# srinidhiPY/SSL_CR_Histo

Hardware: AMD Instinct MI355X
Metric: images/sec (ResNet18 SSL_CR step, 256x256 bf16 synthetic patches; whole job) (higher is better)
Workload: dtype bf16

## Files before the change

include/sslcr.h:

```cpp
#ifndef SSLCR_H_
#define SSLCR_H_
#include <stddef.h>
#include <stdint.h>

#ifdef __cplusplus
extern "C" {
#endif
#if defined(__GNUC__) || defined(__clang__)
#pragma GCC visibility push(default)
#endif

#define SSLCR_F32 0
#define SSLCR_BF16 1
#define SSLCR_FP8 2

int sslcr_version(void);
const char* sslcr_last_error(void);

typedef struct sslcr_conv_desc {
  const void* x;
  const void* w;
  void* y;
  const float* in_scale;
  const float* in_shift;
  const float* bias;
  const void* residual;
  float* stats;
  int N, H, W, C, K, R, S, stride, pad;
  int PH, PW;
  int OH, OW, osh;
  int transposed;
  int in_relu, relu, accumulate;
  int pix_mul, pix_off_h, pix_off_w;
  unsigned tap_mask;
  const void* mask_x; const float* mask_scale; const float* mask_shift; const float* mask_mean;
  int par4;
  int seg_images, seg_stride;
  const float* out_scale;
} sslcr_conv_desc;
int sslcr_conv2d(int dtype, const sslcr_conv_desc* d, void* stream);
int sslcr_conv2d_partial_rows(const sslcr_conv_desc* d);
int sslcr_conv2d_segments_ok(int dtype, const sslcr_conv_desc* d);
const char* sslcr_conv2d_kernel_name(int dtype, const sslcr_conv_desc* d);
int sslcr_conv2d_s2_pair(int dtype, const sslcr_conv_desc* c1, const sslcr_conv_desc* ds, void* stream);
int sslcr_conv2d_s2_pair_ok(int dtype, const sslcr_conv_desc* c1, const sslcr_conv_desc* ds);

typedef struct sslcr_fp8_desc {
  const uint8_t* w8;
  const float* w_dequant;
  float x_scale;
  const float* x_scale_dev;
  float* amax_out;
} sslcr_fp8_desc;
int sslcr_conv2d_fp8(const sslcr_conv_desc* d, const sslcr_fp8_desc* q, void* stream);
int sslcr_conv2d_fp8_partial_rows(const sslcr_conv_desc* d);
typedef struct sslcr_pack_fp8_desc {
  const float* w;
  uint8_t* w8;
  float* w_dequant;
  const float* gamma; const float* beta; const float* rmean; const float* rvar; float eps; float* bias_out;
  int K, C;
} sslcr_pack_fp8_desc;
int sslcr_pack_conv_fp8(const sslcr_pack_fp8_desc* d, void* stream);

typedef struct sslcr_wgrad_desc {
  const void* x;
  const void* dy;
  float* dw;
  const float* in_scale;
  const float* in_shift;
  int in_relu;
  int N, H, W, C, K, R, S, stride, pad, OH, OW;
  int seg_images;
  int seg_stride;
} sslcr_wgrad_desc;
int sslcr_conv2d_wgrad(int dtype, const sslcr_wgrad_desc* d, void* stream);
const char* sslcr_conv2d_wgrad_kernel_name(int dtype, const sslcr_wgrad_desc* d);

int sslcr_probe_tr16(const uint16_t* in, const int* byte_addr, uint16_t* out, void* stream);

typedef struct sslcr_stem_desc {
  const void* x;
  const void* w;
  void* y;
  const float* bias;
  float* stats;
  int N, H, W, OH, OW, in_f32, relu;
  const void* x2;
  int n_split;
  const float* out_scale;
} sslcr_stem_desc;
int sslcr_stem_conv(int dtype, const sslcr_stem_desc* d, void* stream);
int sslcr_stem_partial_rows(const sslcr_stem_desc* d);
int sslcr_stem_conv_pool(int dtype, const sslcr_stem_desc* d, int POH, int POW, void* stream);
typedef struct sslcr_stem_wgrad_desc {
  const void* x; const void* dy;
  float* dw;
  int N, H, W, OH, OW, in_f32;
  const void* x2; int n_split;
} sslcr_stem_wgrad_desc;
int sslcr_stem_wgrad(int dtype, const sslcr_stem_wgrad_desc* d, void* stream);

typedef struct sslcr_bn_finalize_desc {
  const float* partials;
  int rows, C;
  double count;
  const float* gamma; const float* beta;
  float* scale; float* shift; float* mean; float* invstd;
  float* running_mean; float* running_var; int64_t* num_batches_tracked;
  float momentum, eps; int replay;
  double* sums_out;
  const double* sums_in;
  double* stage;
  int nseg, seg_stride;
  int* tickets;
} sslcr_bn_finalize_desc;
int sslcr_bn_finalize(const sslcr_bn_finalize_desc* d, void* stream);

typedef struct sslcr_bn_act_desc {
  const void* x; const float* scale; const float* shift;
  const void* res; const float* rscale; const float* rshift;
  void* y; size_t pixels; int C; int relu;
  int nseg, seg_stride;
  uint8_t* ybits;
} sslcr_bn_act_desc;
int sslcr_bn_act(int dtype, const sslcr_bn_act_desc* d, void* stream);

typedef struct sslcr_pool_fwd_desc {
  const void* x; const float* scale; const float* shift; void* y; uint8_t* argmax; int N, H, W, C, OH, OW;
} sslcr_pool_fwd_desc;
int sslcr_bn_relu_maxpool(int dtype, const sslcr_pool_fwd_desc* d, void* stream);
typedef struct sslcr_pool_bwd_desc {
  const void* dy; const uint8_t* argmax; const void* x; const float* scale; const float* shift; void* dx; int N, H, W, C, OH, OW;
} sslcr_pool_bwd_desc;
int sslcr_maxpool_relu_bwd(int dtype, const sslcr_pool_bwd_desc* d, void* stream);

int sslcr_avgpool_fwd(int dtype, const void* x, float* y, int N, int HW, int C, void* stream);
int sslcr_avgpool_bwd(int dtype, const float* dy, void* dx, int N, int HW, int C, void* stream);

typedef struct sslcr_bn_bwd_desc {
  const void* dy; const void* x; const void* yact;
  const float* scale; const float* shift; const float* mean; const float* invstd;
  double* sums;
  void* dx; void* gout;
  size_t pixels; int C; int relu_from_x; double count;
  const void* pool_dy;
  const uint8_t* pool_argmax;
  int pH, pW, pOH, pOW;
  const void* pool_y;
  int g_in_reduce;
  float* dgamma; float* dbeta;
  float pg_scale;
  int nseg, seg_stride, sums_stride;
  const uint8_t* yact_bits;
} sslcr_bn_bwd_desc;
int sslcr_bn_bwd_reduce(int dtype, const sslcr_bn_bwd_desc* d, void* stream);
int sslcr_bn_bwd_apply(int dtype, const sslcr_bn_bwd_desc* d, void* stream);
int sslcr_bn_param_grads(const double* sums, const float* invstd, float* dgamma, float* dbeta, int C, void* stream);
int sslcr_stem_wgrad_pool(int dtype, const sslcr_stem_wgrad_desc* w, const sslcr_bn_bwd_desc* bn, void* stream);

int sslcr_linear_fwd(const float* x, const float* w, const float* b, float* y, int M, int N, int K, int relu, void* stream);
int sslcr_linear_bwd(const float* x, const float* w, const float* dy, const float* yact, float* dx, float* dw, float* db,
                     int M, int N, int K, int dx_accumulate, float* scratch, void* stream);
typedef struct sslcr_loss_desc {
  int kind;
  const float* logits; const float* logits_t;
  const float* target_f; const int64_t* target_i;
  float* dlogits;
  float* out;
  int nx, nu, C; float lambda_u;
  float inv_nx_global, inv_nu_global;
} sslcr_loss_desc;
int sslcr_loss(const sslcr_loss_desc* d, void* stream);
int sslcr_softmax_col(const float* logits, float* out, int n, int C, int col, void* stream);

typedef struct sslcr_tensor_desc {
  float* p; float* g; float* s1; float* s2;
  int n;
  int K, C, RS;
  void* w_fwd;
  void* w_dgrad;
  int pack_dtype;
  int dgrad_flip;
} sslcr_tensor_desc;
typedef struct sslcr_opt_desc {
  int kind;
  float lr, beta1, beta2, eps, wd, momentum;
  float bc1, bc2;
  int first_step;
  float grad_scale;
} sslcr_opt_desc;
// ... 126 lines not shown
```

ssl_cr_histo_amd/_lib.py:

```python
import ctypes as C
import os

import torch

HERE = os.path.dirname(os.path.abspath(__file__))
LIB_PATH = os.path.join(HERE, "libsslcr.so")

vp, i32, f32, f64, sz = C.c_void_p, C.c_int, C.c_float, C.c_double, C.c_size_t


class SslcrError(RuntimeError):
    pass


def _S(name, fields):
    return type(name, (C.Structure,), {"_fields_": fields})


ConvDesc = _S("ConvDesc", [("x", vp), ("w", vp), ("y", vp), ("in_scale", vp), ("in_shift", vp), ("bias", vp),
                           ("residual", vp), ("stats", vp)] +
              [(k, i32) for k in ("N", "H", "W", "C", "K", "R", "S", "stride", "pad", "PH", "PW", "OH", "OW", "osh",
                                  "transposed", "in_relu", "relu", "accumulate", "pix_mul", "pix_off_h", "pix_off_w")] +
              [("tap_mask", C.c_uint), ("mask_x", vp), ("mask_scale", vp), ("mask_shift", vp), ("mask_mean", vp),
               ("par4", i32), ("seg_images", i32), ("seg_stride", i32), ("out_scale", vp)])
WgradDesc = _S("WgradDesc", [("x", vp), ("dy", vp), ("dw", vp), ("in_scale", vp), ("in_shift", vp), ("in_relu", i32)] +
               [(k, i32) for k in ("N", "H", "W", "C", "K", "R", "S", "stride", "pad", "OH", "OW", "seg_images", "seg_stride")])
StemDesc = _S("StemDesc", [("x", vp), ("w", vp), ("y", vp), ("bias", vp), ("stats", vp)] +
              [(k, i32) for k in ("N", "H", "W", "OH", "OW", "in_f32", "relu")] + [("x2", vp), ("n_split", i32), ("out_scale", vp)])
StemWgradDesc = _S("StemWgradDesc", [("x", vp), ("dy", vp), ("dw", vp)] +
                   [(k, i32) for k in ("N", "H", "W", "OH", "OW", "in_f32")] + [("x2", vp), ("n_split", i32)])
BnFinalizeDesc = _S("BnFinalizeDesc", [("partials", vp), ("rows", i32), ("C", i32), ("count", f64), ("gamma", vp),
                                       ("beta", vp), ("scale", vp), ("shift", vp), ("mean", vp), ("invstd", vp),
                                       ("running_mean", vp), ("running_var", vp), ("num_batches_tracked", vp),
                                       ("momentum", f32), ("eps", f32), ("replay", i32), ("sums_out", vp),
                                       ("sums_in", vp), ("stage", vp), ("nseg", i32), ("seg_stride", i32), ("tickets", vp)])
BnActDesc = _S("BnActDesc", [("x", vp), ("scale", vp), ("shift", vp), ("res", vp), ("rscale", vp), ("rshift", vp),
                             ("y", vp), ("pixels", sz), ("C", i32), ("relu", i32), ("nseg", i32), ("seg_stride", i32), ("ybits", vp)])
PoolFwdDesc = _S("PoolFwdDesc", [("x", vp), ("scale", vp), ("shift", vp), ("y", vp), ("argmax", vp)] +
                 [(k, i32) for k in ("N", "H", "W", "C", "OH", "OW")])
PoolBwdDesc = _S("PoolBwdDesc", [("dy", vp), ("argmax", vp), ("x", vp), ("scale", vp), ("shift", vp), ("dx", vp)] +
                 [(k, i32) for k in ("N", "H", "W", "C", "OH", "OW")])
BnBwdDesc = _S("BnBwdDesc", [("dy", vp), ("x", vp), ("yact", vp), ("scale", vp), ("shift", vp), ("mean", vp),
                             ("invstd", vp), ("sums", vp), ("dx", vp), ("gout", vp), ("pixels", sz), ("C", i32),
                             ("relu_from_x", i32), ("count", f64), ("pool_dy", vp), ("pool_argmax", vp), ("pH", i32),
                             ("pW", i32), ("pOH", i32), ("pOW", i32), ("pool_y", vp), ("g_in_reduce", i32), ("dgamma", vp), ("dbeta", vp),
                             ("pg_scale", f32), ("nseg", i32), ("seg_stride", i32), ("sums_stride", i32), ("yact_bits", vp)])
LossDesc = _S("LossDesc", [("kind", i32), ("logits", vp), ("logits_t", vp), ("target_f", vp), ("target_i", vp),
                           ("dlogits", vp), ("out", vp), ("nx", i32), ("nu", i32), ("C", i32), ("lambda_u", f32),
                           ("inv_nx_global", f32), ("inv_nu_global", f32)])
TensorDesc = _S("TensorDesc", [("p", vp), ("g", vp), ("s1", vp), ("s2", vp), ("n", i32), ("K", i32), ("C", i32),
                               ("RS", i32), ("w_fwd", vp), ("w_dgrad", vp), ("pack_dtype", i32), ("dgrad_flip", i32)])
OptDesc = _S("OptDesc", [("kind", i32), ("lr", f32), ("beta1", f32), ("beta2", f32), ("eps", f32), ("wd", f32),
                         ("momentum", f32), ("bc1", f32), ("bc2", f32), ("first_step", i32), ("grad_scale", f32)])
WeakAugDesc = _S("WeakAugDesc", [("src", vp), ("dst", vp), ("params", vp)] +
                 [(k, i32) for k in ("N", "SH", "SW", "OH", "OW", "src_hwc")])
ColourAugDesc = _S("ColourAugDesc", [("src", vp), ("dst", vp), ("shift", vp), ("apply", vp), ("hed_from_rgb", f64 * 9),
                                     ("rgb_from_hed", f64 * 9), ("N", i32), ("H", i32), ("W", i32), ("hwc", i32)])
BrightnessContrastDesc = _S("BrightnessContrastDesc", [("src", vp), ("dst", vp), ("alpha_beta", vp), ("apply", vp), ("stats", vp),
                                                       ("N", i32), ("H", i32), ("W", i32)])
PackDesc = _S("PackDesc", [("w", vp), ("w_fwd", vp), ("w_dgrad", vp), ("gamma", vp), ("beta", vp), ("rmean", vp),
                           ("rvar", vp), ("eps", f32), ("bias_out", vp)] + [(k, i32) for k in ("K", "C", "R", "S", "dgrad_flip")] + [("scale_out", vp)])

Fp8Desc = _S("Fp8Desc", [("w8", vp), ("w_dequant", vp), ("x_scale", f32), ("x_scale_dev", vp), ("amax_out", vp)])
PackFp8Desc = _S("PackFp8Desc", [("w", vp), ("w8", vp), ("w_dequant", vp), ("gamma", vp), ("beta", vp), ("rmean", vp), ("rvar", vp),
                                 ("eps", f32), ("bias_out", vp), ("K", i32), ("C", i32)])

P = C.POINTER
SIGNATURES = {
    "sslcr_version": (i32, []),
    "sslcr_last_error": (C.c_char_p, []),
    "sslcr_conv2d": (i32, [i32, P(ConvDesc), vp]),
    "sslcr_conv2d_partial_rows": (i32, [P(ConvDesc)]),
    "sslcr_conv2d_segments_ok": (i32, [i32, P(ConvDesc)]),
    "sslcr_conv2d_kernel_name": (C.c_char_p, [i32, P(ConvDesc)]),
    "sslcr_conv2d_s2_pair": (i32, [i32, P(ConvDesc), P(ConvDesc), vp]),
    "sslcr_conv2d_s2_pair_ok": (i32, [i32, P(ConvDesc), P(ConvDesc)]),
    "sslcr_conv2d_fp8": (i32, [P(ConvDesc), P(Fp8Desc), vp]),
    "sslcr_conv2d_fp8_partial_rows": (i32, [P(ConvDesc)]),
    "sslcr_pack_conv_fp8": (i32, [P(PackFp8Desc), vp]),
    "sslcr_conv2d_wgrad": (i32, [i32, P(WgradDesc), vp]),
    "sslcr_conv2d_wgrad_kernel_name": (C.c_char_p, [i32, P(WgradDesc)]),
    "sslcr_probe_tr16": (i32, [vp, vp, vp, vp]),
    "sslcr_stem_conv": (i32, [i32, P(StemDesc), vp]),
    "sslcr_stem_partial_rows": (i32, [P(StemDesc)]),
    "sslcr_stem_conv_pool": (i32, [i32, P(StemDesc), i32, i32, vp]),
    "sslcr_stem_wgrad": (i32, [i32, P(StemWgradDesc), vp]),
    "sslcr_stem_wgrad_pool": (i32, [i32, P(StemWgradDesc), P(BnBwdDesc), vp]),
    "sslcr_bn_finalize": (i32, [P(BnFinalizeDesc), vp]),
    "sslcr_bn_act": (i32, [i32, P(BnActDesc), vp]),
    "sslcr_bn_relu_maxpool": (i32, [i32, P(PoolFwdDesc), vp]),
    "sslcr_maxpool_relu_bwd": (i32, [i32, P(PoolBwdDesc), vp]),
    "sslcr_avgpool_fwd": (i32, [i32, vp, vp, i32, i32, i32, vp]),
    "sslcr_avgpool_bwd": (i32, [i32, vp, vp, i32, i32, i32, vp]),
    "sslcr_bn_bwd_reduce": (i32, [i32, P(BnBwdDesc), vp]),
    "sslcr_bn_bwd_apply": (i32, [i32, P(BnBwdDesc), vp]),
    "sslcr_bn_param_grads": (i32, [vp, vp, vp, vp, i32, vp]),
    "sslcr_linear_fwd": (i32, [vp, vp, vp, vp, i32, i32, i32, i32, vp]),
    "sslcr_linear_bwd": (i32, [vp, vp, vp, vp, vp, vp, vp, i32, i32, i32, i32, vp, vp]),
    "sslcr_loss": (i32, [P(LossDesc), vp]),
    "sslcr_softmax_col": (i32, [vp, vp, i32, i32, i32, vp]),
    "sslcr_optimizer_step": (i32, [vp, i32, i32, P(OptDesc), vp]),
    "sslcr_axpby": (i32, [vp, vp, sz, f32, i32, vp]),
    "sslcr_fill": (i32, [vp, sz, f32, vp]),
    "sslcr_pack_conv": (i32, [i32, P(PackDesc), vp]),
    "sslcr_pack_stem": (i32, [i32, P(PackDesc), vp]),
    "sslcr_weak_augment": (i32, [P(WeakAugDesc), vp]),
    "sslcr_hed_colour_augment": (i32, [P(ColourAugDesc), vp]),
    "sslcr_brightness_contrast": (i32, [P(BrightnessContrastDesc), vp]),
}

_lib = None


def lib():
    global _lib
    if _lib is None:
        if not os.path.exists(LIB_PATH):
            raise SslcrError(f"{LIB_PATH} not built: run `python -m ssl_cr_histo_amd.build` "
                             "(or __graft_entry__.build()); there is no CPU/PyTorch fallback")
        L = C.CDLL(LIB_PATH, mode=C.RTLD_GLOBAL)
        for name, (res, args) in SIGNATURES.items():
            fn = getattr(L, name)
            fn.restype = res
            fn.argtypes = args
        _lib = L
    return _lib


def check(rc):
    if rc != 0:
        raise SslcrError(lib().sslcr_last_error().decode())


def stream_ptr():
    return C.c_void_p(torch.cuda.current_stream().cuda_stream)


def ptr(t):
    return None if t is None else C.c_void_p(t.data_ptr())
```

ssl_cr_histo_amd/csrc/bn_eltwise.hip:

```cpp
#include <stdlib.h>

#include "kernels.hpp"

namespace sslcr {

__global__ __launch_bounds__(256) void bn_reduce_rows_kernel(const float* __restrict__ part, int rows, int C, double* __restrict__ out, int splits) {
  __shared__ double sm[2][8][32];
  const int c = blockIdx.x * 32 + (threadIdx.x & 31);
  const int rl = threadIdx.x >> 5;
  const int per = (rows + splits - 1) / splits;
  const int r0 = blockIdx.y * per, r1 = min(rows, r0 + per);
  part += (size_t)blockIdx.z * rows * 2 * C;
  out += (size_t)blockIdx.z * splits * 2 * C;
  double s = 0.0, ss = 0.0;
  if (c < C) {
    int r = r0 + rl;
    for (; r + 8 < r1; r += 16) {
      const float* p = part + (size_t)r * 2 * C;
      const float* q = p + (size_t)16 * C;
      const float a0 = p[c], a1 = p[C + c], b0 = q[c], b1 = q[C + c];
      s += (double)a0 + (double)b0;
      ss += (double)a1 + (double)b1;
    }
    for (; r < r1; r += 8) {
// ... 481 lines not shown
template <typename T>
__global__ __launch_bounds__(256) void avgpool_fwd_kernel(const void* xv, float* y, int N, int HW, int C) {
  constexpr int EPC = Elem<T>::EPC;
  __shared__ float sm[3][64][EPC + 1];
  const int cols = C / EPC;
  const int cl = threadIdx.x & 63, q = threadIdx.x >> 6;
  const int i = blockIdx.x * 64 + cl;
  const bool ok = i < N * cols;
  const int n = ok ? i / cols : 0, col = ok ? i - n * cols : 0;
  const char* x = reinterpret_cast<const char*>(xv) + ((size_t)n * HW * C) * sizeof(T) + (size_t)col * 16;
  float acc[EPC];
#pragma unroll
  for (int e = 0; e < EPC; ++e) acc[e] = 0.f;
  if (ok) {
#pragma unroll 4
    for (int p = q; p < HW; p += 4) {
      float f[EPC];
      Elem<T>::unpack(ld16(x + (size_t)p * C * sizeof(T)), f);
#pragma unroll
      for (int e = 0; e < EPC; ++e) acc[e] += f[e];
    }
  }
  if (q > 0) {
#pragma unroll
    for (int e = 0; e < EPC; ++e) sm[q - 1][cl][e] = acc[e];
  }
  __syncthreads();
  if (q > 0 || !ok) return;
#pragma unroll
  for (int w = 0; w < 3; ++w)
#pragma unroll
    for (int e = 0; e < EPC; ++e) acc[e] += sm[w][cl][e];
  const float inv = 1.f / (float)HW;
#pragma unroll
  for (int e = 0; e < EPC; ++e) y[(size_t)n * C + col * EPC + e] = acc[e] * inv;
}

template <typename T>
__global__ __launch_bounds__(256) void avgpool_bwd_kernel(const float* dy, void* dxv, int N, int HW, int C) {
  constexpr int EPC = Elem<T>::EPC;
  const int cols = C / EPC;
  const size_t total = (size_t)N * HW * cols;
  char* dx = reinterpret_cast<char*>(dxv);
  const float inv = 1.f / (float)HW;
  for (size_t i = (size_t)blockIdx.x * 256 + threadIdx.x; i < total; i += (size_t)gridDim.x * 256) {
    const int col = (int)(i % cols);
    const int n = (int)(i / ((size_t)HW * cols));
    float f[EPC];
#pragma unroll
    for (int e = 0; e < EPC; ++e) f[e] = dy[(size_t)n * C + col * EPC + e] * inv;
    st16_nt(dx + i * 16, Elem<T>::pack(f));
  }
}

hipError_t launch_avgpool_fwd(int dtype, const void* x, float* y, int N, int HW, int C, hipStream_t st) {
  if (dtype == DT_BF16) {
    hipLaunchKernelGGL(avgpool_fwd_kernel<bf16_t>, dim3(cdiv(N * (C / 8), 64)), dim3(256), 0, st, x, y, N, HW, C);
  } else {
    hipLaunchKernelGGL(avgpool_fwd_kernel<float>, dim3(cdiv(N * (C / 4), 64)), dim3(256), 0, st, x, y, N, HW, C);
  }
  return hipGetLastError();
}
hipError_t launch_avgpool_bwd(int dtype, const float* dy, void* dx, int N, int HW, int C, hipStream_t st) {
  if (dtype == DT_BF16) {
    hipLaunchKernelGGL(avgpool_bwd_kernel<bf16_t>, dim3(ew_grid((size_t)N * HW * (C / 8))), dim3(256), 0, st, dy, dx, N, HW, C);
  } else {
    hipLaunchKernelGGL(avgpool_bwd_kernel<float>, dim3(ew_grid((size_t)N * HW * (C / 4))), dim3(256), 0, st, dy, dx, N, HW, C);
  }
  return hipGetLastError();
}

template <typename T>
__device__ __forceinline__ void bn_bwd_g(const BnBwdArgs& a, size_t i, const float* rsc, const float* rsh, float* g, float* xf) {
  constexpr int EPC = Elem<T>::EPC;
  Elem<T>::unpack(ld16_nt(reinterpret_cast<const char*>(a.x) + i * 16), xf);
  if (a.pool_dy) {
    const int cols = a.C / EPC, col = (int)(i % cols);
    size_t pix = i / cols;
    const int w = (int)(pix % a.pW);
    pix /= a.pW;
    const int h = (int)(pix % a.pH), n = (int)(pix / a.pH);
#pragma unroll
    for (int e = 0; e < EPC; ++e) g[e] = 0.f;
    u32x4_t dv[4];
    uint32_t am[4][2];
    bool ok[4];
    int code[4];
#pragma unroll
    for (int k = 0; k < 4; ++k) {
      const int dh = k >> 1, dw = k & 1;
      const int oh = (h >> 1) + dh, ow = (w >> 1) + dw;
      ok[k] = (dh == 0 || (h & 1)) && (dw == 0 || (w & 1)) && oh < a.pOH && ow < a.pOW;
      code[k] = (h - (2 * oh - 1)) * 3 + (w - (2 * ow - 1));
      const int ohc = oh < a.pOH ? oh : a.pOH - 1, owc = ow < a.pOW ? ow : a.pOW - 1;
      const size_t o = (((size_t)n * a.pOH + ohc) * a.pOW + owc) * cols + col;
      dv[k] = ld16(reinterpret_cast<const char*>(a.pool_dy) + o * 16);
      if (EPC == 8) { const u32x2_t v = *reinterpret_cast<const u32x2_t*>(a.pool_argmax + o * EPC); am[k][0] = v[0]; am[k][1] = v[1]; }
      else { am[k][0] = *reinterpret_cast<const uint32_t*>(a.pool_argmax + o * EPC); am[k][1] = 0; }
    }
#pragma unroll
    for (int k = 0; k < 4; ++k) {
      float d[EPC];
      Elem<T>::unpack(dv[k], d);
#pragma unroll
      for (int e = 0; e < EPC; ++e)
        if (ok[k] && ((am[k][e >> 2] >> (8 * (e & 3))) & 0xffu) == (uint32_t)code[k]) g[e] += d[e];
    }
  } else {
    Elem<T>::unpack(ld16_nt(reinterpret_cast<const char*>(a.dy) + i * 16), g);
  }
  if (EPC == 8 && a.yact_bits) {
    const unsigned b = a.yact_bits[i];
#pragma unroll
    for (int e = 0; e < EPC; ++e)
      if (!((b >> e) & 1u)) g[e] = 0.f;
  } else if (a.yact) {
// ... 356 lines not shown

hipError_t launch_bn_bwd_reduce(int dtype, const BnBwdArgs& a, hipStream_t st) {
  const int epc = dtype == DT_BF16 ? 8 : 4;
  const int cols = a.C / epc;
  if (cols > 256 || (256 % cols) != 0) return hipErrorInvalidValue;
  const int nseg = a.nseg > 1 ? a.nseg : 1;
  if (nseg > 1 && (a.pool_dy || a.pixels % nseg != 0)) return hipErrorInvalidValue;
  const size_t pixels = a.pixels / nseg;
  const int rpp = 256 / cols;
  size_t blocks = (pixels + rpp - 1) / rpp;
  blocks = (blocks + 7) / 8;
  if (blocks > 1024) blocks = 1024;
  if (blocks < 1) blocks = 1;
  const bool big = blocks >= 512 && !(a.pool_dy && a.pool_y);
  size_t b4 = 0;
  if (big) {
    b4 = ((pixels + 1024 / cols - 1) / (1024 / cols) + 7) / 8;
    if (b4 > 256) b4 = 256;
  }
  const int nrows = (int)(big ? b4 : blocks);
  double* rows = reinterpret_cast<double*>(stream_scratch(st, (size_t)nseg * nrows * 2 * a.C * sizeof(double)));
  if (!rows) return hipErrorOutOfMemory;
  auto fold = [&]() {
    hipLaunchKernelGGL(bn_bwd_sums_kernel, dim3(cdiv(2 * a.C, 64), nseg), dim3(64, 16), 0, st, rows, nrows, 2 * a.C, a.sums, nseg > 1 ? a.sums_stride : 0);
    return hipGetLastError();
  };
  if (a.pool_dy && a.pool_y) {
    if (dtype == DT_BF16) hipLaunchKernelGGL(bn_bwd_reduce_pool_kernel<bf16_t>, dim3((int)blocks), dim3(256), 0, st, a, rows);
    else hipLaunchKernelGGL(bn_bwd_reduce_pool_kernel<float>, dim3((int)blocks), dim3(256), 0, st, a, rows);
    return fold();
  }
  if (big) {
    constexpr int NB = 1024;
    const size_t lds = (size_t)NB * (2 * epc + 1) * sizeof(float);
    static std::atomic<bool> attr_done{false};
    if (!attr_done) {
      (void)hipFuncSetAttribute(reinterpret_cast<const void*>(bn_bwd_reduce_kernel<bf16_t, 1024>), hipFuncAttributeMaxDynamicSharedMemorySize, 96 * 1024);
      (void)hipFuncSetAttribute(reinterpret_cast<const void*>(bn_bwd_reduce_kernel<float, 1024>), hipFuncAttributeMaxDynamicSharedMemorySize, 96 * 1024);
      attr_done = true;
    }
    if (dtype == DT_BF16) hipLaunchKernelGGL((bn_bwd_reduce_kernel<bf16_t, 1024>), dim3((int)b4, nseg), dim3(NB), lds, st, a, rows);
    else hipLaunchKernelGGL((bn_bwd_reduce_kernel<float, 1024>), dim3((int)b4, nseg), dim3(NB), lds, st, a, rows);
    return fold();
  }
  const size_t lds = (size_t)256 * (2 * epc + 1) * sizeof(float);
  if (dtype == DT_BF16) {
    hipLaunchKernelGGL((bn_bwd_reduce_kernel<bf16_t, 256>), dim3((int)blocks, nseg), dim3(256), lds, st, a, rows);
  } else {
    hipLaunchKernelGGL((bn_bwd_reduce_kernel<float, 256>), dim3((int)blocks, nseg), dim3(256), lds, st, a, rows);
  }
  return fold();
}

bool bn_bwd_pair_ok(const BnBwdArgs& a, const BnBwdArgs& b) {
  static const bool on = [] { const char* e = getenv("SSLCR_BN_PAIR"); return !e || atoi(e) != 0; }();
  return on && a.g_in_reduce && a.gout && b.dy == a.gout && !b.yact && !b.yact_bits && !b.relu_from_x && !b.gout && !a.pool_dy && !b.pool_dy &&
         a.nseg <= 1 && b.nseg <= 1 && a.C == b.C && a.pixels == b.pixels && b.sums == a.sums + 2 * a.C && a.dx && b.dx && b.x && a.x;
}
hipError_t launch_bn_bwd_reduce_pair(int dtype, const BnBwdArgs& a, const BnBwdArgs& b, int keep_g, hipStream_t st) {
  const int epc = dtype == DT_BF16 ? 8 : 4;
  const int cols = a.C / epc;
  if (cols > 256 || (256 % cols) != 0 || !bn_bwd_pair_ok(a, b)) return hipErrorInvalidValue;
  const int rpp = 256 / cols;
  size_t blocks = (a.pixels + rpp - 1) / rpp;
  blocks = (blocks + 7) / 8;
  if (blocks > 1024) blocks = 1024;
  if (blocks < 1) blocks = 1;
  const bool big = blocks >= 512;
  size_t b4 = 0;
  if (big) {
    b4 = ((a.pixels + 1024 / cols - 1) / (1024 / cols) + 7) / 8;
    if (b4 > 256) b4 = 256;
  }
  const int nrows = (int)(big ? b4 : blocks);
  double* rows = reinterpret_cast<double*>(stream_scratch(st, (size_t)2 * nrows * 2 * a.C * sizeof(double)));
  if (!rows) return hipErrorOutOfMemory;
  static std::atomic<bool> attr_done{false};
  if (!attr_done) {
    (void)hipFuncSetAttribute(reinterpret_cast<const void*>(bn_bwd_reduce_pair_kernel<bf16_t, 1024>), hipFuncAttributeMaxDynamicSharedMemorySize, 128 * 1024);
    (void)hipFuncSetAttribute(reinterpret_cast<const void*>(bn_bwd_reduce_pair_kernel<float, 1024>), hipFuncAttributeMaxDynamicSharedMemorySize, 128 * 1024);
    attr_done = true;
  }
  const int NB = big ? 1024 : 256;
  const size_t lds = (size_t)NB * (3 * epc + 1) * sizeof(float);
  if (big) {
    if (dtype == DT_BF16) hipLaunchKernelGGL((bn_bwd_reduce_pair_kernel<bf16_t, 1024>), dim3(nrows), dim3(1024), lds, st, a, b, rows, keep_g);
    else hipLaunchKernelGGL((bn_bwd_reduce_pair_kernel<float, 1024>), dim3(nrows), dim3(1024), lds, st, a, b, rows, keep_g);
  } else {
    if (dtype == DT_BF16) hipLaunchKernelGGL((bn_bwd_reduce_pair_kernel<bf16_t, 256>), dim3(nrows), dim3(256), lds, st, a, b, rows, keep_g);
    else hipLaunchKernelGGL((bn_bwd_reduce_pair_kernel<float, 256>), dim3(nrows), dim3(256), lds, st, a, b, rows, keep_g);
  }
  hipLaunchKernelGGL(bn_bwd_sums_kernel, dim3(cdiv(2 * a.C, 64), 2), dim3(64, 16), 0, st, rows, nrows, 2 * a.C, a.sums, 2 * a.C);
  return hipGetLastError();
}
hipError_t launch_bn_bwd_apply_pair(int dtype, const BnBwdArgs& a, const BnBwdArgs& b, int from_g, hipStream_t st) {
  if (!bn_bwd_pair_ok(a, b)) return hipErrorInvalidValue;
  if (dtype == DT_BF16) hipLaunchKernelGGL(bn_bwd_apply_pair_kernel<bf16_t>, dim3(ew_grid(a.pixels * (a.C / 8))), dim3(256), 0, st, a, b, from_g);
  else hipLaunchKernelGGL(bn_bwd_apply_pair_kernel<float>, dim3(ew_grid(a.pixels * (a.C / 4))), dim3(256), 0, st, a, b, from_g);
  return hipGetLastError();
}

hipError_t launch_bn_bwd_apply(int dtype, const BnBwdArgs& a0, hipStream_t st) {
  BnBwdArgs a = a0;
  if (a.g_in_reduce) {
    a.dy = a.gout; a.yact = nullptr; a.yact_bits = nullptr; a.relu_from_x = 0; a.gout = nullptr; a.g_in_reduce = 0;
  }
  if (a.pool_dy && a.nseg > 1) return hipErrorInvalidValue;
  if (a.pool_dy) {
    const int epc = dtype == DT_BF16 ? 8 : 4;
    const size_t items = (a.pixels / ((size_t)a.pH * a.pW)) * ((a.pH + 1) / 2) * ((a.pW + 1) / 2) * (a.C / epc);
    if (dtype == DT_BF16) hipLaunchKernelGGL(bn_bwd_apply_pool_kernel<bf16_t>, dim3(ew_grid(items)), dim3(256), 0, st, a);
    else hipLaunchKernelGGL(bn_bwd_apply_pool_kernel<float>, dim3(ew_grid(items)), dim3(256), 0, st, a);
    return hipGetLastError();
  }
  const int nseg = a.nseg > 1 ? a.nseg : 1;
  if (a.pixels % nseg != 0) return hipErrorInvalidValue;
  const size_t per = a.pixels / nseg;
  if (dtype == DT_BF16) {
    hipLaunchKernelGGL(bn_bwd_apply_kernel<bf16_t>, dim3(ew_grid(per * (a.C / 8)), nseg), dim3(256), 0, st, a);
  } else {
    hipLaunchKernelGGL(bn_bwd_apply_kernel<float>, dim3(ew_grid(per * (a.C / 4)), nseg), dim3(256), 0, st, a);
  }
  return hipGetLastError();
}

__global__ void bn_param_grads_kernel(const double* sums, const float* invstd, float* dgamma, float* dbeta, int C, float scale) {
  const int c = blockIdx.x * blockDim.x + threadIdx.x;
  if (c >= C) return;
  dgamma[c] += (float)(sums[C + c] * (double)invstd[c] * (double)scale);
  dbeta[c] += (float)(sums[c] * (double)scale);
}
hipError_t launch_bn_param_grads_scaled(const double* sums, const float* invstd, float* dgamma, float* dbeta, int C, float scale, hipStream_t st) {
  hipLaunchKernelGGL(bn_param_grads_kernel, dim3(cdiv(C, 64)), dim3(64), 0, st, sums, invstd, dgamma, dbeta, C, scale);
  return hipGetLastError();
}
hipError_t launch_bn_param_grads(const double* sums, const float* invstd, float* dgamma, float* dbeta, int C, hipStream_t st) {
  return launch_bn_param_grads_scaled(sums, invstd, dgamma, dbeta, C, 1.f, st);
}

}
```

ssl_cr_histo_amd/csrc/capi.cpp:

```cpp
#include <stdarg.h>
#include <stdio.h>
#include <string.h>

#include "kernels.hpp"

namespace sslcr {
thread_local char g_err[512] = "";
int fail(const char* fmt, ...) {
  va_list ap;
  va_start(ap, fmt);
  vsnprintf(g_err, sizeof(g_err), fmt, ap);
  va_end(ap);
  return -1;
}
int check(hipError_t e, const char* what) {
  if (e == hipSuccess) return 0;
  return fail("%s: %s", what, hipGetErrorString(e));
}
}

using namespace sslcr;

#define NEED(cond, what) \
  do {                   \
    if (!(cond)) return fail("%s: invalid argument (%s)", __func__, what); \
  } while (0)
#define DT_OK(dt) NEED((dt) == SSLCR_F32 || (dt) == SSLCR_BF16, "dtype")

extern "C" {

int sslcr_version(void) { return 6; }
const char* sslcr_last_error(void) { return g_err; }

int sslcr_conv2d(int dtype, const sslcr_conv_desc* d, void* stream) {
  DT_OK(dtype);
  NEED(d && d->x && d->w && d->y, "null tensor");
  NEED(d->N > 0 && d->C > 0 && d->K > 0 && d->R > 0 && d->S > 0 && d->stride > 0, "shape");
  NEED(d->C % (dtype == SSLCR_BF16 ? 64 : 32) == 0, "C must be a multiple of the 128-byte channel slab");
  NEED(d->K % 64 == 0, "K % 64");
  NEED(d->osh >= 1 && d->PH > 0 && d->PW > 0, "pixel space");
  NEED(conv_segments_ok(dtype, *d), "seg_images: no segment form for this shape / dtype (sslcr_conv2d_segments_ok)");
  return check(launch_conv(dtype, *d, (hipStream_t)stream), "conv2d");
}
int sslcr_conv2d_partial_rows(const sslcr_conv_desc* d) { return d ? conv_partials_rows(*d) : -1; }
int sslcr_conv2d_segments_ok(int dtype, const sslcr_conv_desc* d) { return (d && (dtype == DT_F32 || dtype == DT_BF16) && conv_segments_ok(dtype, *d)) ? 1 : 0; }
const char* sslcr_conv2d_kernel_name(int dtype, const sslcr_conv_desc* d) { return d ? conv_kernel_name(dtype, *d) : ""; }
int sslcr_conv2d_s2_pair_ok(int dtype, const sslcr_conv_desc* c1, const sslcr_conv_desc* ds) {
  return (c1 && ds && conv_s2_pair_ok(dtype, *c1, *ds)) ? 1 : 0;
}
int sslcr_conv2d_s2_pair(int dtype, const sslcr_conv_desc* c1, const sslcr_conv_desc* ds, void* stream) {
  DT_OK(dtype);
  NEED(c1 && ds && c1->x && c1->w && c1->y && ds->w && ds->y, "null tensor");
  NEED(conv_s2_pair_ok(dtype, *c1, *ds), "pair not served (sslcr_conv2d_s2_pair_ok)");
  return check(launch_conv_s2(*c1, ds, (hipStream_t)stream), "conv2d_s2_pair");
}

int sslcr_conv2d_fp8(const sslcr_conv_desc* d, const sslcr_fp8_desc* q, void* stream) {
  NEED(d && q && d->x && d->y && q->w8 && q->w_dequant, "null tensor");
  NEED(q->x_scale > 0.f, "x_scale must be positive");
  NEED(conv_fp8_mode(*d) != 0, "shape not served by the fp8 kernel (3x3/1, C % 128, K % 128, 16x16-tileable or 8x8 with N % 4)");
  return check(launch_conv_fp8(*d, *q, (hipStream_t)stream), "conv2d_fp8");
}
int sslcr_conv2d_fp8_partial_rows(const sslcr_conv_desc* d) { return (d && conv_fp8_mode(*d)) ? conv_fp8_rows(*d) : 0; }
int sslcr_pack_conv_fp8(const sslcr_pack_fp8_desc* d, void* stream) {
  NEED(d && d->w && d->w8 && d->w_dequant && d->K > 0 && d->C > 0, "args");
  NEED(!d->gamma || (d->beta && d->rmean && d->rvar), "BatchNorm fold needs gamma, beta, running mean and var");
  return check(launch_pack_fp8(*d, (hipStream_t)stream), "pack_conv_fp8");
}

const char* sslcr_conv2d_wgrad_kernel_name(int dtype, const sslcr_wgrad_desc* d) { return d ? wgrad_kernel_name(dtype, *d) : ""; }
int sslcr_conv2d_wgrad(int dtype, const sslcr_wgrad_desc* d, void* stream) {
  DT_OK(dtype);
  NEED(d && d->x && d->dy && d->dw, "null tensor");
  NEED(d->C % 64 == 0 && d->K % 64 == 0, "C,K % 64");
  NEED((d->R == 3 && d->S == 3) || (d->R == 1 && d->S == 1), "3x3 or 1x1");
  return check(launch_wgrad(dtype, *d, (hipStream_t)stream), "conv2d_wgrad");
}

int sslcr_probe_tr16(const uint16_t* in, const int* byte_addr, uint16_t* out, void* stream) {
  NEED(in && byte_addr && out, "null");
  return check(launch_probe_tr16(in, byte_addr, out, (hipStream_t)stream), "probe_tr16");
}

int sslcr_stem_conv(int dtype, const sslcr_stem_desc* d, void* stream) {
  DT_OK(dtype);
  NEED(d && d->x && d->w && d->y, "null tensor");
  NEED(d->OH == (d->H + 6 - 7) / 2 + 1 && d->OW == (d->W + 6 - 7) / 2 + 1, "7x7/2 pad 3 output dims");
  NEED(!d->x2 || (d->n_split >= 0 && d->n_split <= d->N), "n_split outside the batch");
  return check(launch_stem(dtype, *d, (hipStream_t)stream), "stem_conv");
}
int sslcr_stem_conv_pool(int dtype, const sslcr_stem_desc* d, int POH, int POW, void* stream) {
  DT_OK(dtype);
  NEED(d && d->x && d->w && d->y, "null");
  NEED(stem_pool_ok(dtype, *d, POH, POW), "shape / mode not served by the fused stem + max-pool kernel");
// ... 2 lines not shown
int sslcr_stem_partial_rows(const sslcr_stem_desc* d) { return d ? stem_partials_rows(*d) : -1; }
int sslcr_stem_wgrad(int dtype, const sslcr_stem_wgrad_desc* d, void* stream) {
  DT_OK(dtype);
  NEED(d && d->x && d->dy && d->dw, "null tensor");
  NEED(!d->x2 || (d->n_split >= 0 && d->n_split <= d->N), "n_split outside the batch");
  return check(launch_stem_wgrad(dtype, *d, (hipStream_t)stream), "stem_wgrad");
}
int sslcr_stem_wgrad_pool(int dtype, const sslcr_stem_wgrad_desc* w, const sslcr_bn_bwd_desc* bn, void* stream) {
  DT_OK(dtype);
  NEED(w && w->x && w->dw && bn && bn->pool_dy && bn->pool_argmax && bn->x && bn->sums && bn->mean && bn->invstd && bn->scale && bn->shift, "null tensor");
  NEED(!w->x2 || (w->n_split >= 0 && w->n_split <= w->N), "n_split outside the batch");
  NEED(bn->C == 64 && bn->pH == w->OH && bn->pW == w->OW && bn->pixels == (size_t)w->N * w->OH * w->OW, "bn descriptor is not this stem's");
  NEED(!bn->g_in_reduce && !bn->gout, "pool form has no g output");
  return check(launch_stem_wgrad_pool(dtype, *w, *bn, (hipStream_t)stream), "stem_wgrad_pool");
}

int sslcr_bn_finalize(const sslcr_bn_finalize_desc* d, void* stream) {
  NEED(d && d->C > 0, "desc");
  NEED(d->sums_in || (d->partials && d->stage && d->rows > 0), "partials/stage");
  NEED(d->sums_out || (d->gamma && d->beta && d->scale && d->shift && d->count > 0), "finalize outputs");
  return check(launch_bn_finalize(*d, (hipStream_t)stream), "bn_finalize");
}
int sslcr_bn_act(int dtype, const sslcr_bn_act_desc* d, void* stream) {
  DT_OK(dtype);
  NEED(d && d->x && d->y && d->scale && d->shift, "null");
  NEED(d->C % 8 == 0, "C % 8");
  return check(launch_bn_act(dtype, *d, (hipStream_t)stream), "bn_act");
}
int sslcr_bn_relu_maxpool(int dtype, const sslcr_pool_fwd_desc* d, void* stream) {
  DT_OK(dtype);
  NEED(d && d->x && d->y, "null");
  if (!d->scale || !d->shift) {
    const int cols = d->C / (dtype == SSLCR_BF16 ? 8 : 4);
    NEED(!d->scale && !d->shift && !d->argmax, "plain max-pool (scale = shift = NULL) records no argmax");
    NEED(cols >= 1 && cols <= 256 && 256 % cols == 0 && d->C % (dtype == SSLCR_BF16 ? 8 : 4) == 0, "plain max-pool: unsupported channel count");
  }
  return check(launch_bn_relu_maxpool(dtype, *d, (hipStream_t)stream), "bn_relu_maxpool");
}
int sslcr_maxpool_relu_bwd(int dtype, const sslcr_pool_bwd_desc* d, void* stream) {
  DT_OK(dtype);
  NEED(d && d->x && d->dy && d->dx && d->argmax, "null");
  return check(launch_maxpool_relu_bwd(dtype, *d, (hipStream_t)stream), "maxpool_relu_bwd");
}
int sslcr_avgpool_fwd(int dtype, const void* x, float* y, int N, int HW, int C, void* stream) {
  DT_OK(dtype);
  NEED(x && y && N > 0 && HW > 0 && C % 8 == 0, "args");
  return check(launch_avgpool_fwd(dtype, x, y, N, HW, C, (hipStream_t)stream), "avgpool_fwd");
}
int sslcr_avgpool_bwd(int dtype, const float* dy, void* dx, int N, int HW, int C, void* stream) {
  DT_OK(dtype);
  NEED(dy && dx && N > 0 && HW > 0 && C % 8 == 0, "args");
  return check(launch_avgpool_bwd(dtype, dy, dx, N, HW, C, (hipStream_t)stream), "avgpool_bwd");
}
int sslcr_bn_bwd_reduce(int dtype, const sslcr_bn_bwd_desc* d, void* stream) {
  DT_OK(dtype);
  NEED(d && (d->dy || (d->pool_dy && d->pool_argmax)) && d->x && d->sums && d->mean, "null");
  NEED(!d->g_in_reduce || (d->yact && d->gout && d->dy && !d->pool_dy), "g_in_reduce needs dy, yact and gout");
  return check(launch_bn_bwd_reduce(dtype, *d, (hipStream_t)stream), "bn_bwd_reduce");
}
int sslcr_bn_bwd_apply(int dtype, const sslcr_bn_bwd_desc* d, void* stream) {
  DT_OK(dtype);
  NEED(d && (d->dy || (d->pool_dy && d->pool_argmax)) && d->x && d->sums && d->dx && d->mean && d->invstd && d->scale, "null");
  NEED(!d->g_in_reduce || (d->yact && d->gout && d->dy && !d->pool_dy), "g_in_reduce needs dy, yact and gout");
  return check(launch_bn_bwd_apply(dtype, *d, (hipStream_t)stream), "bn_bwd_apply");
}
int sslcr_bn_param_grads(const double* sums, const float* invstd, float* dgamma, float* dbeta, int C, void* stream) {
  NEED(sums && invstd && dgamma && dbeta, "null");
  return check(launch_bn_param_grads(sums, invstd, dgamma, dbeta, C, (hipStream_t)stream), "bn_param_grads");
}

int sslcr_linear_fwd(const float* x, const float* w, const float* b, float* y, int M, int N, int K, int relu, void* stream) {
  NEED(x && w && y && M > 0 && N > 0 && K > 0, "args");
  return check(launch_linear_fwd(x, w, b, y, M, N, K, relu, (hipStream_t)stream), "linear_fwd");
}
int sslcr_linear_bwd(const float* x, const float* w, const float* dy, const float* yact, float* dx, float* dw, float* db,
                     int M, int N, int K, int dx_accumulate, float* scratch, void* stream) {
  NEED(x && w && dy && scratch && M > 0 && N > 0 && K > 0, "args");
  return check(launch_linear_bwd(x, w, dy, yact, dx, dw, db, M, N, K, dx_accumulate, scratch, (hipStream_t)stream), "linear_bwd");
}
int sslcr_loss(const sslcr_loss_desc* d, void* stream) {
  NEED(d && d->logits && d->out && d->nx > 0 && d->C > 0 && d->C <= 64, "args");
  return check(launch_loss(*d, (hipStream_t)stream), "loss");
}

int sslcr_softmax_col(const float* logits, float* out, int n, int C, int col, void* stream) {
  NEED(logits && out && n > 0 && C > 0 && C <= 64 && col >= 0 && col < C, "args");
  return check(launch_softmax_col(logits, out, n, C, col, (hipStream_t)stream), "softmax_col");
}

int sslcr_optimizer_step(const sslcr_tensor_desc* device_descs, int ntensors, int max_n, const sslcr_opt_desc* o, void* stream) {
  NEED(device_descs && o && ntensors > 0 && max_n > 0, "args");
  return check(launch_optimizer(device_descs, ntensors, max_n, *o, (hipStream_t)stream), "optimizer_step");
}
int sslcr_axpby(float* p, float* q, size_t n, float alpha, int copy_back, void* stream) {
  NEED(p && q, "null");
  return check(launch_axpby(p, q, n, alpha, copy_back, (hipStream_t)stream), "axpby");
}
int sslcr_fill(float* p, size_t n, float v, void* stream) {
  NEED(p, "null");
  return check(launch_fill(p, n, v, (hipStream_t)stream), "fill");
}
int sslcr_pack_conv(int dtype, const sslcr_pack_desc* d, void* stream) {
  DT_OK(dtype);
  NEED(d && d->w && (d->w_fwd || d->w_dgrad), "null");
  return check(launch_pack_conv(dtype, *d, (hipStream_t)stream), "pack_conv");
}
// ... 23 lines not shown
```

ssl_cr_histo_amd/csrc/conv_h16.hip:

```cpp
#include "kernels.hpp"

namespace sslcr {

template <typename T> struct MmaH;
template <> struct MmaH<bf16_t> {
  __device__ static __forceinline__ void run(const u32x4_t& a, const u32x4_t& b, f32x4_t& c) {
    c = __builtin_amdgcn_mfma_f32_16x16x32_bf16(__builtin_bit_cast(bf16x8_t, a), __builtin_bit_cast(bf16x8_t, b), c, 0, 0, 0);
  }
};
template <> struct MmaH<float> {
  __device__ static __forceinline__ void run(const u32x4_t& a, const u32x4_t& b, f32x4_t& c) {
#pragma unroll
    for (int e = 0; e < 4; ++e)
      c = __builtin_amdgcn_mfma_f32_16x16x4f32(__uint_as_float(a[e]), __uint_as_float(b[e]), c, 0, 0, 0);
  }
};

template <int TK>
__device__ __forceinline__ int wperm_inv(int rr) {
  constexpr int B = 16 * TK;
  const int blk = rr / B, x = rr - blk * B;
  const int t = x >> 4, q = (x >> 2) & 3, j = x & 3;
  return blk * B + q * (4 * TK) + t * 4 + j;
}

#define SSLCR_WAIT_VM0() __builtin_amdgcn_s_waitcnt(0x0f70)
#define SSLCR_BARE_BARRIER() asm volatile("s_barrier" ::: "memory")

#ifdef SSLCR_H16_PROF
__device__ unsigned long long g_h16_prof[16][8];
#define H16_T(v) const unsigned long long v = __builtin_readcyclecounter()
#define H16_ACC(i, d) h16_t[i] += (d)
#else
#define H16_T(v)
#define H16_ACC(i, d)
#endif

template <typename T, int BKO, int WK, bool XF, bool WR, bool RAW = false, int TW = 16>
__global__ __launch_bounds__(256 * WK, WK == 1 ? 1 : 2) void conv3x3_h16_kernel(const ConvArgs a, const int tiles_total, const int n_items, const int kshift,
                                                                                const int row0) {
  constexpr bool OSC = false;
#include "conv_h16_body.hpp"
}
template <typename T, int BKO, int WK, bool WR, int TW>
__global__ __launch_bounds__(256 * WK, WK == 1 ? 1 : 2) void conv3x3_h16s_kernel(const ConvArgs a, const int tiles_total, const int n_items, const int kshift,
                                                                                 const int row0) {
  constexpr bool OSC = true, XF = false, RAW = false;
#include "conv_h16_body.hpp"
}

static int h16_mode(int dtype, const ConvArgs& a) {
  const int q = conv_halo256_mode(dtype, a);
  if (q == 16 && conv_halo256_mode(DT_BF16, a) == 16) return 16;
  static const bool on8 = [] { const char* e = getenv("SSLCR_H16_TW8"); return !e || atoi(e) != 0; }();
  if (q == 8 && on8 && conv_halo256_mode(DT_BF16, a) == 8 && a.K % 128 == 0 && !a.mask_x && (a.seg_images <= 0 || a.seg_images % 4 == 0)) return 8;
  return 0;
}
bool conv_h16_ok(int dtype, const ConvArgs& a) {
  if (a.in_scale && a.residual) return false;
  if (a.mask_x) {
    if (!a.mask_scale || !a.mask_shift || !a.mask_mean || a.in_scale || a.bias || a.residual || a.relu || a.out_scale) return false;
    if (18 * 24 * 128 + 2 * 3 * (a.K % 128 == 0 ? 128 : 64) * 128 + 2 * a.C * 4 + 8 * 128 * 4 + 3 * a.K * 4 > 160 * 1024) return false;
  }
  if (a.out_scale) {
    if (a.in_scale || a.stats || !a.bias) return false;
    const int mode = h16_mode(dtype, a);
    if (mode == 0) return false;
    const int bko = a.K % 128 == 0 ? 128 : 64;
    if (!(a.C == 64 && a.K == 64) &&
        (mode == 16 ? 18 * 24 : 4 * 10 * 10) * 128 + 2 * 3 * bko * 128 + 2 * a.C * 4 + 8 * bko * 4 + 2 * a.K * 4 > 160 * 1024) return false;
  }
  return h16_mode(dtype, a) != 0;
}
static int h16_tiles(const ConvArgs& a, int nseg) {
  return a.H == 8 ? (a.N / nseg) / 4 : (a.N / nseg) * (a.H / 16) * (a.W / 16);
}
static int h16_grid(const ConvArgs& a, int bko) {
  const int nseg = a.seg_images > 0 ? a.N / a.seg_images : 1;
  const int n_items = h16_tiles(a, nseg) * (a.K / bko);
  const int per = device_cus() / nseg;
  return (n_items < per ? n_items : per) * nseg;
}
static int h16_tail8(const ConvArgs& a) {
  if (a.H != 8 || a.seg_images > 0) return 0;
  const int cus = device_cus(), tiles = a.N / 4, kb = a.K / 128, rem = (tiles * kb) % cus;
  if (rem == 0 || 2 * rem > cus || rem % kb != 0 || tiles <= rem / kb) return 0;
  return rem / kb;
}
static ConvArgs h16_head8(const ConvArgs& a, int tail) { ConvArgs h = a; h.N = a.N - 4 * tail; return h; }
static ConvArgs h16_tailargs8(const ConvArgs& a, int tail, int dtype) {
  ConvArgs t = a;
  const int n0 = a.N - 4 * tail;
  const size_t es = dtype == DT_BF16 ? 2 : 4, px = (size_t)n0 * a.H * a.W;
  t.N = 4 * tail;
  t.x = reinterpret_cast<const char*>(a.x) + px * a.C * es;
  t.y = reinterpret_cast<char*>(a.y) + px * a.K * es;
  if (a.residual) t.residual = reinterpret_cast<const char*>(a.residual) + px * a.K * es;
  return t;
}
int conv_h16_rows(const ConvArgs& a) {
  if (a.seg_images > 0 && conv_pp64_ok(DT_BF16, a)) return conv_pp64_rows(a);
  const int tail = h16_tail8(a);
  if (tail) return (h16_grid(h16_head8(a, tail), 128) + h16_grid(h16_tailargs8(a, tail, DT_BF16), 64)) * 4;
  return h16_grid(a, a.K % 128 == 0 ? 128 : 64) * 4;
}

static bool h16_resident(const ConvArgs& a) { return a.C == 64 && a.K == 64; }
static bool h16_raw(const ConvArgs& a) {
  static const bool on = [] { const char* e = getenv("SSLCR_H16_RAW"); return !e || atoi(e) != 0; }();
  return on && a.stats && !a.bias && !a.relu && !a.residual && !a.mask_x;
}

template <typename T, int BKO, int WK, bool XF, bool WR = false, bool RAW = false, int TW = 16, bool OSC = false>
static hipError_t launch_h(const ConvArgs& a, hipStream_t st, int row0 = 0) {
  const size_t lds = (TW == 16 ? 18 * 24 : 4 * 10 * 10) * 128 + (WR ? 3 : 2) * 3 * BKO * 128 + 2 * a.C * sizeof(float) + 8 * BKO * sizeof(float) +
                     (a.mask_x ? 3 : (a.out_scale ? 2 : 1)) * a.K * sizeof(float);
  if (lds > 160 * 1024) return hipErrorInvalidValue;
  static_assert(!OSC || (!XF && !RAW), "output scale: eval forms only");
  void (*kern)(const ConvArgs, const int, const int, const int, const int);
  if constexpr (OSC) kern = conv3x3_h16s_kernel<T, BKO, WK, WR, TW>;
  else kern = conv3x3_h16_kernel<T, BKO, WK, XF, WR, RAW, TW>;
  if (OSC != (a.out_scale != nullptr)) return hipErrorInvalidValue;
  static std::atomic<bool> attr_done{false};
  if (!attr_done) {
    hipError_t e = hipFuncSetAttribute(reinterpret_cast<const void*>(kern), hipFuncAttributeMaxDynamicSharedMemorySize, 160 * 1024);
    if (e != hipSuccess) return e;
    attr_done = true;
  }
  const int nseg = a.seg_images > 0 ? a.N / a.seg_images : 1;
  const int tiles = h16_tiles(a, nseg);
  const int n_items = tiles * (a.K / BKO);
  const int grid = h16_grid(a, BKO);
  const int kbn = a.K / BKO, gseg = grid / nseg;
  const int kshift = (kbn > 1 && (kbn & (kbn - 1)) == 0 && (gseg & (kbn - 1)) == 0) ? __builtin_ctz(kbn) : -1;
  hipLaunchKernelGGL(kern, dim3(grid), dim3(256 * WK), lds, st, a, tiles, n_items, kshift, row0);
  return hipGetLastError();
}

template <typename T>
static hipError_t launch_ht8(const ConvArgs& a, hipStream_t st) {
  const bool xf = a.in_scale != nullptr;
  auto wide = [&](const ConvArgs& q) {
    if (q.out_scale) return launch_h<T, 128, 2, false, false, false, 8, true>(q, st);
    if constexpr (sizeof(T) == 2)
      if (h16_raw(q)) return xf ? launch_h<T, 128, 2, true, false, true, 8>(q, st) : launch_h<T, 128, 2, false, false, true, 8>(q, st);
    return xf ? launch_h<T, 128, 2, true, false, false, 8>(q, st) : launch_h<T, 128, 2, false, false, false, 8>(q, st);
  };
  const int tail = h16_tail8(a);
  if (!tail) return wide(a);
  const ConvArgs head = h16_head8(a, tail), tl = h16_tailargs8(a, tail, Elem<T>::DT);
  hipError_t e = wide(head);
  if (e != hipSuccess) return e;
  const int row0 = h16_grid(head, 128) * 4;
  if (tl.out_scale) return launch_h<T, 64, 2, false, false, false, 8, true>(tl, st, row0);
  return xf ? launch_h<T, 64, 2, true, false, false, 8>(tl, st, row0) : launch_h<T, 64, 2, false, false, false, 8>(tl, st, row0);
}

template <typename T>
static hipError_t launch_ht(const ConvArgs& a, hipStream_t st) {
  const bool xf = a.in_scale != nullptr;
  if (h16_mode(Elem<T>::DT, a) == 8) return launch_ht8<T>(a, st);
  if (a.K % 128 == 0) {
    if (a.out_scale) return launch_h<T, 128, 2, false, false, false, 16, true>(a, st);
    if constexpr (sizeof(T) == 2)
      if (h16_raw(a)) return xf ? launch_h<T, 128, 2, true, false, true>(a, st) : launch_h<T, 128, 2, false, false, true>(a, st);
    return xf ? launch_h<T, 128, 2, true>(a, st) : launch_h<T, 128, 2, false>(a, st);
  }
  if constexpr (sizeof(T) == 2)
    if (h16_resident(a)) {
      if (conv_pp64_ok(DT_BF16, a)) return launch_conv_pp64(a, st);
      if (a.out_scale) return launch_h<T, 64, 2, false, true, false, 16, true>(a, st);
      return xf ? launch_h<T, 64, 2, true, true>(a, st) : launch_h<T, 64, 2, false, true>(a, st);
    }
  if (a.out_scale) return launch_h<T, 64, 2, false, false, false, 16, true>(a, st);
  return xf ? launch_h<T, 64, 2, true>(a, st) : launch_h<T, 64, 2, false>(a, st);
}

hipError_t launch_conv_h16(int dtype, const ConvArgs& a, hipStream_t st) {
  if (a.mask_x && !a.stats) return hipErrorInvalidValue;
  return dtype == DT_BF16 ? launch_ht<bf16_t>(a, st) : launch_ht<float>(a, st);
}

const char* conv_h16_name(int dtype, const ConvArgs& a) {
  const bool bf = dtype == DT_BF16, xf = a.in_scale != nullptr;
  if (a.out_scale) {
    if (h16_mode(dtype, a) == 8) return bf ? "sslcr::conv3x3_h16s_kernel<unsigned short, 128, 2, false, 8>" : "sslcr::conv3x3_h16s_kernel<float, 128, 2, false, 8>";
    if (a.K % 128 == 0) return bf ? "sslcr::conv3x3_h16s_kernel<unsigned short, 128, 2, false, 16>" : "sslcr::conv3x3_h16s_kernel<float, 128, 2, false, 16>";
    if (bf && h16_resident(a) && conv_pp64_ok(DT_BF16, a)) return conv_pp64_name(a);
    if (bf && h16_resident(a)) return "sslcr::conv3x3_h16s_kernel<unsigned short, 64, 2, true, 16>";
    return bf ? "sslcr::conv3x3_h16s_kernel<unsigned short, 64, 2, false, 16>" : "sslcr::conv3x3_h16s_kernel<float, 64, 2, false, 16>";
  }
  if (h16_mode(dtype, a) == 8) {
    if (!bf) return xf ? "sslcr::conv3x3_h16_kernel<float, 128, 2, true, false, false, 8>" : "sslcr::conv3x3_h16_kernel<float, 128, 2, false, false, false, 8>";
    if (h16_raw(a))
      return xf ? "sslcr::conv3x3_h16_kernel<unsigned short, 128, 2, true, false, true, 8>" : "sslcr::conv3x3_h16_kernel<unsigned short, 128, 2, false, false, true, 8>";
    return xf ? "sslcr::conv3x3_h16_kernel<unsigned short, 128, 2, true, false, false, 8>" : "sslcr::conv3x3_h16_kernel<unsigned short, 128, 2, false, false, false, 8>";
  }
  if (a.K % 128 == 0) {
    if (bf && h16_raw(a))
      return xf ? "sslcr::conv3x3_h16_kernel<unsigned short, 128, 2, true, false, true, 16>" : "sslcr::conv3x3_h16_kernel<unsigned short, 128, 2, false, false, true, 16>";
    if (bf) return xf ? "sslcr::conv3x3_h16_kernel<unsigned short, 128, 2, true, false, false, 16>" : "sslcr::conv3x3_h16_kernel<unsigned short, 128, 2, false, false, false, 16>";
    return xf ? "sslcr::conv3x3_h16_kernel<float, 128, 2, true, false, false, 16>" : "sslcr::conv3x3_h16_kernel<float, 128, 2, false, false, false, 16>";
  }
  if (bf && h16_resident(a) && conv_pp64_ok(DT_BF16, a)) return conv_pp64_name(a);
  if (bf && h16_resident(a))
    return xf ? "sslcr::conv3x3_h16_kernel<unsigned short, 64, 2, true, true, false, 16>" : "sslcr::conv3x3_h16_kernel<unsigned short, 64, 2, false, true, false, 16>";
  if (bf) return xf ? "sslcr::conv3x3_h16_kernel<unsigned short, 64, 2, true, false, false, 16>" : "sslcr::conv3x3_h16_kernel<unsigned short, 64, 2, false, false, false, 16>";
  return xf ? "sslcr::conv3x3_h16_kernel<float, 64, 2, true, false, false, 16>" : "sslcr::conv3x3_h16_kernel<float, 64, 2, false, false, false, 16>";
}

}
```

ssl_cr_histo_amd/csrc/conv_h16_body.hpp:

```cpp
  constexpr int NT = 256 * WK;
  constexpr int EPC = Elem<T>::EPC;
  constexpr int CE = 8 * EPC;
  static_assert(TW == 16 || (TW == 8 && !WR), "tile forms");
  constexpr int TH = TW, NI = 256 / (TW * TH), HH = TH + 2, HWD = TW + 2, PITCH = TW == 16 ? 24 : 10;
  constexpr int HP = TW == 16 ? HH * HWD : 256;
  constexpr int NLD = (HP * 8 + NT - 1) / NT;
  constexpr int TK = BKO / (16 * WK), TP = 4;
  constexpr int HBUF = NI * HH * PITCH * 128, WBUF = BKO * 128, TPB = 3;
  static_assert(NLD <= 16, "staging shape");
  extern __shared__ __attribute__((aligned(16))) char smem[];
  char* s_halo = smem;
  constexpr int NRING = WR ? 3 : 2;
  char* s_w = smem + HBUF;
  float* s_scale = reinterpret_cast<float*>(smem + HBUF + NRING * TPB * WBUF);
  float* s_shift = s_scale + a.C;
  float* s_stat = s_shift + a.C;

  const int tid = threadIdx.x, lane = tid & 63;
  const int wave = __builtin_amdgcn_readfirstlane(tid >> 6);
  const int g = lane >> 4, li = lane & 15;
  const int wp = wave & 3, wk = wave >> 2;
  const int tiles_w = TW == 16 ? a.W / TW : 1, tiles_h = TW == 16 ? a.H / TH : 1;
  const int nseg = a.seg_images > 0 ? a.N / a.seg_images : 1;
  const int G = gridDim.x / nseg;
  const int seg = nseg > 1 ? (int)blockIdx.x / G : 0, lb = (int)blockIdx.x - seg * G;
  const int seg_n0 = seg * a.seg_images;
  if (XF) {
    const float* isc = a.in_scale + (size_t)seg * a.seg_stride;
    const float* ish = a.in_shift + (size_t)seg * a.seg_stride;
    for (int c = tid; c < a.C; c += NT) { s_scale[c] = isc[c]; s_shift[c] = ish[c]; }
  }
  for (int i = tid; i < 8 * BKO; i += NT) s_stat[i] = 0.f;
  float* s_bias = s_stat + 8 * BKO;
  const bool mk = !OSC && !XF && !RAW && a.mask_x != nullptr;
  float* s_msh = s_bias + a.K;
  float* s_mmu = s_msh + a.K;
  float* s_osc = s_msh;
  for (int i = tid; i < a.K; i += NT) {
    const size_t mo = (size_t)seg * a.seg_stride + i;
    s_bias[i] = mk ? a.mask_scale[mo] : (a.bias ? a.bias[i] : 0.f);
    if (mk) { s_msh[i] = a.mask_shift[mo]; s_mmu[i] = a.mask_mean[mo]; }
    if constexpr (OSC) s_osc[i] = a.out_scale[i];
  }
  const float relu_lo = a.in_relu ? 0.f : -__builtin_inff();
  const float out_lo = a.relu ? 0.f : -__builtin_inff();

  const int first = (G & 7) ? lb : (lb & 7) * (G >> 3) + (lb >> 3);
  if (first >= n_items) return;

  const int chunk = tid & 7;
  int rel[NLD], st_off[NLD];
  unsigned long long edge = 0;
  unsigned hvalid = 0;
#pragma unroll
  for (int i = 0; i < NLD; ++i) {
    const int sp = (tid >> 3) + (NT / 8) * i;
    rel[i] = 0; st_off[i] = 0;
    if (TW == 8) {
      rel[i] = sp;
      const int hc = (sp & 7) + 1;
      const int hp = ((sp >> 6) * HH + ((sp >> 3) & 7) + 1) * PITCH + hc;
      st_off[i] = hp * 128 + ((chunk ^ (hc & 7)) << 4);
      hvalid |= 1u << i;
    } else if (sp < HP) {
      const int hr = sp / HWD, hc = sp - hr * HWD;
      rel[i] = (hr - 1) * a.W + hc - 1;
      const int hp = hr * PITCH + hc;
      st_off[i] = hp * 128 + ((chunk ^ (hp & 7)) << 4);
      hvalid |= 1u << i;
      edge |= (unsigned long long)((hr == 0) | ((hr == HH - 1) << 1) | ((hc == 0) << 2) | ((hc == HWD - 1) << 3)) << (4 * i);
    }
  }
  const bool loader = WK == 1 || wave >= 4;
  constexpr int WLI = BKO / 32;
  const int lw = wave & 3;
  constexpr int WROWS = BKO / WLI;
  int wsrc0;
  {
    const int rr = lw * 8 + (lane >> 3);
    const int krow = wperm_inv<TK>(rr);
    const int c16 = (lane & 7) ^ (rr & 7);
    wsrc0 = (int)(((size_t)krow * 9 * a.C + c16 * EPC) * sizeof(T));
  }
  int Bb[3][2], Ab[2];
#pragma unroll
  for (int kk = 0; kk < 2; ++kk) {
    const int ci = kk * 4 + g;
#pragma unroll
    for (int s = 0; s < 3; ++s)
      Bb[s][kk] = TW == 16 ? ((wp * 4) * PITCH + li + s) * 128 + ((ci ^ ((li + s) & 7)) << 4)
                           : ((wp * HH + (li >> 3)) * PITCH + (li & 7) + s) * 128 + ((ci ^ (((li & 7) + s) & 7)) << 4);
    Ab[kk] = (wk * (BKO / WK) + li) * 128 + ((ci ^ (li & 7)) << 4);
  }
  const char* xg = reinterpret_cast<const char*>(a.x) + (size_t)chunk * EPC * sizeof(T);
  const char* wg = reinterpret_cast<const char*>(a.w);
  const int nslabs = a.C / CE;

  const bool kfast = kshift >= 0;
  struct Geo { int origin, k0, tile, n0, h0, w0; unsigned long long out; };
  auto geom = [&](int item) {
    Geo q;
    const int kbi = kfast ? item & ((1 << kshift) - 1) : item / tiles_total;
    q.tile = kfast ? item >> kshift : item - kbi * tiles_total;
    q.k0 = kbi * BKO;
    int t = q.tile;
    const int tw_i = t % tiles_w; t /= tiles_w;
    const int th_i = t % tiles_h;
    q.n0 = (t / tiles_h) * NI + seg_n0;
    q.h0 = th_i * TH; q.w0 = tw_i * TW;
    q.origin = (q.n0 * a.H + q.h0) * a.W + q.w0;
    q.out = TW == 8 ? 0ull : (unsigned long long)((q.h0 == 0) | ((q.h0 + TH >= a.H) << 1) | ((q.w0 == 0) << 2) | ((q.w0 + TW >= a.W) << 3)) *
                             0x1111111111111111ull;
    return q;
  };

  u32x4_t hreg[NLD];
  unsigned hin = 0;
  auto load_halo = [&](const Geo& q, int slab) {
    const unsigned long long bad = edge & q.out;
    hin = 0;
#pragma unroll
    for (int i = 0; i < NLD; ++i) {
      const bool ok = ((hvalid >> i) & 1u) && !((bad >> (4 * i)) & 0xfull);
      const int idx = q.origin + (ok ? rel[i] : 0);
      hreg[i] = ld16_nt(xg + ((size_t)idx * a.C + slab * CE) * sizeof(T));
      hin |= (ok ? 1u : 0u) << i;
    }
  };
  float sc[EPC], sh[EPC];
  auto load_affine = [&](int slab) {
    if (XF) {
      const int cb = slab * CE + chunk * EPC;
#pragma unroll
      for (int e = 0; e < EPC; ++e) { sc[e] = s_scale[cb + e]; sh[e] = s_shift[cb + e]; }
    }
  };
  auto xform_one = [&](int i) {
    u32x4_t v = hreg[i];
    if (XF) {
      float f[EPC];
      Elem<T>::unpack(v, f);
#pragma unroll
      for (int e = 0; e < EPC; ++e) f[e] = clamp_lo(fmaf(f[e], sc[e], sh[e]), relu_lo);
      v = PackH<T>::run(f);
    }
    const bool ok = (hin >> i) & 1u;
#pragma unroll
    for (int e = 0; e < 4; ++e) v[e] = ok ? v[e] : 0u;
    hreg[i] = v;
  };
  auto store_halo = [&]() {
#pragma unroll
    for (int i = 0; i < NLD; ++i)
      if ((hvalid >> i) & 1u) st16(s_halo + st_off[i], hreg[i]);
  };
  LdsDma wdma;
  wdma.init(wg, 0x7fffffffu);
  auto dma_w = [&](int k0, int slab, int tap0, int half) {
    if (!loader) return;
#pragma unroll
    for (int tt = 0; tt < TPB; ++tt) {
      const int soff = (int)(((size_t)k0 * 9 * a.C + (size_t)(tap0 + tt) * a.C + slab * CE) * sizeof(T));
#pragma unroll
      for (int i = 0; i < WLI; ++i) {
        char* dst = s_w + (half * TPB + tt) * WBUF + (i * WROWS + lw * 8) * 128;
        wdma.load16(dst, wsrc0, soff + wperm_inv<TK>(i * WROWS) * 9 * a.C * (int)sizeof(T));
      }
    }
  };

  f32x4_t acc[TK][TP];
#pragma unroll
  for (int t = 0; t < TK; ++t)
#pragma unroll
    for (int p = 0; p < TP; ++p) acc[t][p] = f32x4_t{0.f, 0.f, 0.f, 0.f};

  u32x4_t A[2][TK], B[2][TP];
  auto frags = [&](int buf, int step, const char* ringg) {
    const int tap = step >> 1, kk = step & 1;
    const int r = tap / 3, s = tap - 3 * r;
    A[buf][0] = ld16(ringg + Ab[kk] + s * WBUF);
#pragma unroll
    for (int p = 0; p < TP; ++p) B[buf][p] = ld16(s_halo + Bb[s][kk] + ((TW == 16 ? p : 2 * p) + r) * (PITCH * 128));
#pragma unroll
    for (int t = 1; t < TK; ++t) A[buf][t] = ld16(ringg + Ab[kk] + s * WBUF + t * 2048);
  };

  if (TW == 8) {
    for (int i = tid; i < HBUF / 16; i += NT) st16(s_halo + i * 16, u32x4_t{0u, 0u, 0u, 0u});
    __syncthreads();
  }
  Geo cur = geom(first);
  dma_w(cur.k0, 0, 0, 0);
  if constexpr (WR) { dma_w(cur.k0, 0, 3, 1); dma_w(cur.k0, 0, 6, 2); }
  load_halo(cur, 0);
  if (XF) __syncthreads();
  load_affine(0);
#pragma unroll
  for (int i = 0; i < NLD; ++i) xform_one(i);
  store_halo();
  SSLCR_WAIT_VM0();
  __syncthreads();
  frags(0, 0, s_w);

  char* yg = reinterpret_cast<char*>(a.y);
  const char* rg = (XF || RAW) ? nullptr : reinterpret_cast<const char*>(a.mask_x ? a.mask_x : a.residual);
  constexpr bool RPRE = sizeof(T) == 2 && !XF && !RAW;
  constexpr int RQ = 4 * TK / EPC;
  u32x4_t rres[RPRE ? TP : 1][RPRE ? RQ : 1];
  auto out_off = [&](const Geo& q, int p) {
    const int h = q.h0 + wp * 4 + p, w = q.w0 + li;
    const size_t pix = TW == 16 ? ((size_t)q.n0 * a.H + h) * a.W + w : (size_t)(q.n0 + wp) * 64 + p * 16 + li;
    return (pix * a.K + q.k0 + wk * (BKO / WK) + g * (4 * TK)) * sizeof(T);
  };
  int wb = 0, item = first, slab = 0;
  unsigned pub = 0;
#ifdef SSLCR_H16_PROF
  unsigned long long h16_t[8] = {0, 0, 0, 0, 0, 0, 0, 0};
  const unsigned long long h16_begin = __builtin_readcyclecounter();
#endif
  for (;;) {
    const bool last = slab + 1 == nslabs;
    const bool done = last && item + G >= n_items;
    const int nslab = last ? 0 : slab + 1;
    const Geo nxt = (last && !done) ? geom(item + G) : cur;
    const char* ring0 = s_w + wb * (TPB * WBUF);
    const char* ring1 = s_w + (wb ^ 1) * (TPB * WBUF);

    auto load_res = [&]() {
      if constexpr (RPRE) {
        if (rg && last) {
#pragma unroll
          for (int p = 0; p < TP; ++p)
#pragma unroll
            for (int q = 0; q < RQ; ++q) rres[p][q] = ld16(rg + out_off(cur, p) + q * 16);
        }
      }
    };
    if constexpr (WR) {
      load_res();
      load_halo(nxt, 0);
    } else {
      dma_w(cur.k0, slab, 3, wb ^ 1);
    }
    __builtin_amdgcn_sched_barrier(0);
#pragma unroll
    for (int i = 0; i < 18; ++i) {
      if (i < 17) frags((i + 1) & 1, i + 1, WR ? s_w + ((i + 1) / 6) * (TPB * WBUF) : ((((i + 1) / 6) & 1) ? ring1 : ring0));
      if (sizeof(T) != 2) __builtin_amdgcn_sched_barrier(0);
#pragma unroll
      for (int t = 0; t < TK; ++t)
#pragma unroll
        for (int p = 0; p < TP; ++p) MmaH<T>::run(A[i & 1][t], B[i & 1][p], acc[t][p]);
      if (i < 17 && sizeof(T) == 2) {
#pragma unroll
        for (int q = 0; q < TK + TP; ++q) {
          __builtin_amdgcn_sched_group_barrier(0x100, 1, 0);
          __builtin_amdgcn_sched_group_barrier(0x008, (TK * TP) / (TK + TP), 0);
        }
      }
      if (i >= 15) {
#pragma unroll
        for (int j = (i - 15); j < NLD; j += 3) xform_one(j);
      }
      __builtin_amdgcn_sched_barrier(0);
      if (WR && i == 14) {
        SSLCR_WAIT_VM0();
        __builtin_amdgcn_sched_barrier(0);
      }
      if (!WR && i % 6 == 2) {
        H16_T(tp0);
        SSLCR_WAIT_VM0();
        H16_T(tp1);
        SSLCR_BARE_BARRIER();
        H16_T(tp2);
        H16_ACC(0, tp1 - tp0); H16_ACC(1, tp2 - tp1);
        if (i == 8) {
          load_res();
          load_halo(nxt, nslab);
          load_affine(nslab);
        }
        __builtin_amdgcn_sched_barrier(0);
      }
      if (!WR && (i == 5 || i == 11)) {
        H16_T(tf0);
        SSLCR_BARE_BARRIER();
        H16_T(tf1);
        H16_ACC(2, tf1 - tf0);
        if (i == 5) dma_w(cur.k0, slab, 6, wb); else dma_w(nxt.k0, nslab, 0, wb ^ 1);
// ... 57 lines not shown
          }
        }
      } else if constexpr (OSC) {
#pragma unroll
      for (int q = 0; q < 4 * TK / EPC; ++q) {
        float bq[EPC], sq[EPC];
#pragma unroll
        for (int e = 0; e < EPC; ++e) { bq[e] = s_bias[kb + q * EPC + e]; sq[e] = s_osc[kb + q * EPC + e]; }
#pragma unroll
        for (int p = 0; p < TP; ++p) {
          const size_t off = out_off(cur, p);
          float vq[EPC];
#pragma unroll
          for (int e = 0; e < EPC; ++e) {
            const int idx = q * EPC + e;
            vq[e] = fmaf(acc[idx >> 2][p][idx & 3], sq[e], bq[e]);
          }
          if (rg) {
            float rr[EPC];
            if constexpr (RPRE) Elem<T>::unpack(rres[p][q], rr);
            else Elem<T>::unpack(ld16(rg + off + q * 16), rr);
#pragma unroll
            for (int e = 0; e < EPC; ++e) vq[e] += rr[e];
          }
#pragma unroll
          for (int e = 0; e < EPC; ++e) vq[e] = clamp_lo(vq[e], out_lo);
          st16(yg + off + q * 16, PackH<T>::run(vq));
        }
      }
      } else {
      float bias[4 * TK];
#pragma unroll
      for (int j = 0; j < 4 * TK; ++j) bias[j] = s_bias[kb + j];
#pragma unroll
      for (int p = 0; p < TP; ++p) {
        const size_t off = out_off(cur, p);
        float v[4 * TK];
#pragma unroll
        for (int t = 0; t < TK; ++t)
#pragma unroll
          for (int j = 0; j < 4; ++j) v[t * 4 + j] = acc[t][p][j] + bias[t * 4 + j];
#pragma unroll
        for (int q = 0; q < 4 * TK / EPC; ++q) {
          float* vq = v + q * EPC;
          if (rg) {
            float rr[EPC];
            if constexpr (RPRE) Elem<T>::unpack(rres[p][q], rr);
            else Elem<T>::unpack(ld16(rg + off + q * 16), rr);
#pragma unroll
            for (int e = 0; e < EPC; ++e) vq[e] += rr[e];
          }
#pragma unroll
          for (int e = 0; e < EPC; ++e) vq[e] = clamp_lo(vq[e], out_lo);
          st16(yg + off + q * 16, PackH<T>::run(vq));
        }
      }
      }
      if (a.stats) {
#pragma unroll
        for (int t = 0; t < TK; ++t)
#pragma unroll
          for (int j = 0; j < 4; ++j) {
            float x1 = 0.f, x2 = 0.f;
#pragma unroll
            for (int p = 0; p < TP; ++p) { float q = acc[t][p][j]; x1 += q; x2 = fmaf(q, q, x2); }
            s1[t * 4 + j] = x1;
            s2[t * 4 + j] = x2;
          }
      }
      }
      constexpr bool FOLD = (4 * TK) % 16 == 0;
      if (a.stats) {
        if constexpr (FOLD) {
#pragma unroll
          for (int f = 0; f < 4 * TK / 16; ++f) {
            row16_fold16(*reinterpret_cast<float (*)[16]>(s1 + 16 * f));
            row16_fold16(*reinterpret_cast<float (*)[16]>(s2 + 16 * f));
          }
          if ((li & 3) == 0) {
            float* sp = s_stat + (wp * 2) * BKO + wk * (BKO / WK) + g * (4 * TK) + (li >> 2) * 4;
#pragma unroll
            for (int h = 0; h < 2; ++h) {
#pragma unroll
              for (int f = 0; f < 4 * TK / 16; ++f) {
                const float* sv = (h ? s2 : s1) + 16 * f;
                f32x4_t* slot = reinterpret_cast<f32x4_t*>(sp + h * BKO + 16 * f);
                f32x4_t v = *slot;
#pragma unroll
                for (int e = 0; e < 4; ++e) v[e] += sv[e];
                *slot = v;
              }
            }
          }
        } else {
#pragma unroll
          for (int i = 0; i < 4 * TK; ++i) { s1[i] = row16_sum(s1[i]); s2[i] = row16_sum(s2[i]); }
        }
        if (!FOLD && li == 0) {
          float* sp = s_stat + (wp * 2) * BKO + wk * (BKO / WK) + g * (4 * TK);
#pragma unroll
          for (int h = 0; h < 2; ++h) {
            const float* sv = h ? s2 : s1;
#pragma unroll
            for (int c4 = 0; c4 < TK; ++c4) {
              f32x4_t* slot = reinterpret_cast<f32x4_t*>(sp + h * BKO + c4 * 4);
              f32x4_t v = *slot;
// ... 46 lines not shown
```

ssl_cr_histo_amd/csrc/conv_igemm.hip:

```cpp
#include "kernels.hpp"

namespace sslcr {

template <typename T> struct Mma;
template <> struct Mma<bf16_t> {
  __device__ static __forceinline__ void run(const u32x4_t& a, const u32x4_t& b, f32x4_t& c) {
    c = __builtin_amdgcn_mfma_f32_16x16x32_bf16(__builtin_bit_cast(bf16x8_t, a), __builtin_bit_cast(bf16x8_t, b), c, 0, 0, 0);
  }
};
template <> struct Mma<float> {
  __device__ static __forceinline__ void run(const u32x4_t& a, const u32x4_t& b, f32x4_t& c) {
#pragma unroll
    for (int e = 0; e < 4; ++e)
      c = __builtin_amdgcn_mfma_f32_16x16x4f32(__uint_as_float(a[e]), __uint_as_float(b[e]), c, 0, 0, 0);
  }
};

template <typename T, int BP, int BKO>
__global__ __launch_bounds__(256) void conv_igemm_kernel(const ConvArgs a) {
  constexpr int EPC = Elem<T>::EPC;
  constexpr int CE = 8 * EPC;
  constexpr int TP = BP / 32;
  constexpr int TK = BKO / 32;
  constexpr int PR = BP / 32;
// ... 262 lines not shown
  const bool bf = dtype == DT_BF16;
  const bool wide = a.K % 128 == 0;
  if (conv_h16_ok(dtype, a)) return conv_h16_name(dtype, a);
  const int q = conv_halo256_mode(dtype, a);
  if (q && conv_halo256_mode(DT_BF16, a) == q) {
    const bool one = a.C == (bf ? 64 : 32);
    if (q == 16) {
      if (wide) return bf ? "sslcr::conv3x3_halo256_kernel<unsigned short, 16, 128, 2, false>" : "sslcr::conv3x3_halo256_kernel<float, 16, 128, 2, false>";
      if (one) return bf ? "sslcr::conv3x3_halo256_kernel<unsigned short, 16, 64, 1, true>" : "sslcr::conv3x3_halo256_kernel<float, 16, 64, 1, true>";
      return bf ? "sslcr::conv3x3_halo256_kernel<unsigned short, 16, 64, 2, false>" : "sslcr::conv3x3_halo256_kernel<float, 16, 64, 2, false>";
    }
    if (wide) return bf ? "sslcr::conv3x3_halo256_kernel<unsigned short, 8, 128, 2, false>" : "sslcr::conv3x3_halo256_kernel<float, 8, 128, 2, false>";
    if (one) return bf ? "sslcr::conv3x3_halo256_kernel<unsigned short, 8, 64, 1, true>" : "sslcr::conv3x3_halo256_kernel<float, 8, 64, 1, true>";
    return bf ? "sslcr::conv3x3_halo256_kernel<unsigned short, 8, 64, 2, false>" : "sslcr::conv3x3_halo256_kernel<float, 8, 64, 2, false>";
  }
  const int tw = q ? 0 : conv_halo_tw(dtype, a);
  if (tw && conv_halo_tw(DT_BF16, a) == tw) return bf ? "sslcr::conv3x3_halo_kernel<unsigned short, ...>" : "sslcr::conv3x3_halo_kernel<float, ...>";
  if (!q && !tw && conv_s2_ok(dtype, a)) return conv_s2_name(a, false);
  if (!q && !tw && conv_s2d_ok(dtype, a)) return conv_s2d_name();
  const int dbp = (q || tw) ? 0 : conv_dma_bp(dtype, a);
  if (dbp && conv_dma_bp(DT_BF16, a) == dbp) return conv_dma_name(dtype, dbp);
  const int bp = conv_tile_bp(a);
  if (bp == 128) {
    if (wide) return bf ? "sslcr::conv_igemm_kernel<unsigned short, 128, 128>" : "sslcr::conv_igemm_kernel<float, 128, 128>";
    return bf ? "sslcr::conv_igemm_kernel<unsigned short, 128, 64>" : "sslcr::conv_igemm_kernel<float, 128, 64>";
  }
  return bf ? "sslcr::conv_igemm_kernel<unsigned short, 64, 64>" : "sslcr::conv_igemm_kernel<float, 64, 64>";
}

int device_cus() {
  static const int cus = [] {
    int dev = 0, n = 0;
    if (hipGetDevice(&dev) != hipSuccess || hipDeviceGetAttribute(&n, hipDeviceAttributeMultiprocessorCount, dev) != hipSuccess || n <= 0) n = 256;
    return n;
  }();
  return cus;
}

bool conv_segments_ok(int dtype, const ConvArgs& a) {
  if (a.seg_images <= 0) return true;
  if (dtype != DT_BF16 || a.N % a.seg_images != 0 || a.transposed || a.par4) return false;
  const int nseg = a.N / a.seg_images;
  if (nseg > 8) return false;
  if (conv_h16_ok(dtype, a)) return true;
  if (a.mask_x) return false;
  const int q = conv_halo256_mode(dtype, a);
  if (q) return q == 16 || a.seg_images % 4 == 0;
  if (conv_halo_tw(dtype, a)) return false;
  const int bp = conv_dma_bp(dtype, a);
  if (bp) return !a.in_scale && ((long)a.seg_images * a.PH * a.PW) % bp == 0;
  return false;
}

hipError_t launch_conv(int dtype, const ConvArgs& a, hipStream_t st) {
  if (!conv_segments_ok(dtype, a)) return hipErrorInvalidValue;
  if (a.out_scale && (!a.bias || a.stats || a.mask_x)) return hipErrorInvalidValue;
  if (conv_h16_ok(dtype, a)) return launch_conv_h16(dtype, a, st);
  if (a.mask_x) return hipErrorInvalidValue;
  const int q = conv_halo256_mode(dtype, a);
  if (q && conv_halo256_mode(DT_BF16, a) == q) return launch_conv_halo256(dtype, a, q, st);
  const int tw = q ? 0 : conv_halo_tw(dtype, a);
  if (tw && conv_halo_tw(DT_BF16, a) == tw) return launch_conv_halo(dtype, a, tw, st);
  if (!q && !tw && conv_s2_ok(dtype, a)) return launch_conv_s2(a, nullptr, st);
  if (!q && !tw && conv_s2d_ok(dtype, a)) return launch_conv_s2d(a, st);
  const int dbp = (q || tw) ? 0 : conv_dma_bp(dtype, a);
  if (dbp && conv_dma_bp(DT_BF16, a) == dbp) return launch_conv_dma(dtype, a, dbp, st);
  if (a.par4) return hipErrorInvalidValue;
  return dtype == DT_BF16 ? launch_t<bf16_t>(a, st) : launch_t<float>(a, st);
}

}
```

ssl_cr_histo_amd/csrc/conv_pp64.hip:

```cpp
#include <stdlib.h>

#include "kernels.hpp"

namespace sslcr {

typedef const __attribute__((address_space(1))) void* gptr_pp;
typedef __attribute__((address_space(3))) void* lptr_pp;

#define SSLCR_PP_BAR() asm volatile("s_waitcnt lgkmcnt(0)\n\ts_barrier" ::: "memory")

#ifdef SSLCR_PP_PROF
__device__ unsigned long long g_pp_prof[8][8];
#define PP_T(v) const unsigned long long v = __builtin_readcyclecounter()
#define PP_ACC(i, d) pp_t[i] += (d)
#else
#define PP_T(v)
#define PP_ACC(i, d)
#endif

#define PP_CH(t, g, j) ((((t) >> 1) * 32) + ((g) * 8) + (((t) & 1) * 4) + (j))
__device__ __forceinline__ int pp_row_kout(int rr) {
  const int t = rr >> 4, gq = (rr >> 2) & 3, j = rr & 3;
  return PP_CH(t, gq, j);
}
// ... 3 lines not shown
  typedef bf16_t T;
  constexpr int EPC = 8, BKO = 64, TK = 4, TP = 4;
  constexpr int TW = 16, TH = 16, HH = 18, HWD = 18, PITCH = 18, HP = HH * HWD;
  constexpr int GT = 256;
  constexpr int NLD = (HP * 8 + GT - 1) / GT;
  constexpr int WBUF = BKO * 128, HBUF = HH * PITCH * 128;
  constexpr bool RPRE = OP != 0;
  static_assert(!(XF && OP != 0), "no residual with an input transform");
  constexpr int RQ = 4 * TK / EPC;
  extern __shared__ __attribute__((aligned(16))) char smem[];
  char* s_w = smem;
  const int tid = threadIdx.x, lane = tid & 63;
  const int wave = __builtin_amdgcn_readfirstlane(tid >> 6);
  const int grp = wave >> 2, wq = wave & 3;
  const int gtid = tid & (GT - 1);
  const int g = lane >> 4, li = lane & 15;
  char* s_halo = smem + 9 * WBUF + grp * HBUF;
  float* s_f = reinterpret_cast<float*>(smem + 9 * WBUF + 2 * HBUF);
  float* s_scale = s_f;
  float* s_shift = s_f + 64;
  float* s_bias = s_f + 128;
  float* s_msh = s_f + 192;
  float* s_mmu = s_f + 256;
  float* s_stat = s_f + 320 + grp * 512;

  const int tiles_w = a.W / TW, tiles_h = a.H / TH;
  const int nseg = a.seg_images > 0 ? a.N / a.seg_images : 1;
  const int G = gridDim.x / nseg;
  const int seg = nseg > 1 ? (int)blockIdx.x / G : 0, lb = (int)blockIdx.x - seg * G;
  const int seg_n0 = seg * a.seg_images;
  const int vb = (G & 7) ? lb : (lb & 7) * (G >> 3) + (lb >> 3);
  const int first0 = 2 * vb;
  if (first0 >= tiles_total) return;
  const int nst = (tiles_total - first0 + 2 * G - 1) / (2 * G);
  constexpr bool mk = OP == 2;
  const float relu_lo = a.in_relu ? 0.f : -__builtin_inff();

  {
    const int rr = wave * 8 + (lane >> 3);
    const int krow = pp_row_kout(rr);
    const int c16 = (lane & 7) ^ (rr & 7);
    const char* wg = reinterpret_cast<const char*>(a.w) + ((size_t)krow * 9 * 64 + c16 * EPC) * sizeof(T);
#pragma unroll
    for (int tt = 0; tt < 9; ++tt)
      __builtin_amdgcn_global_load_lds((gptr_pp)(wg + (size_t)tt * 64 * sizeof(T)), (lptr_pp)(s_w + tt * WBUF + (wave * 8) * 128), 16, 0, 0);
  }
  if (tid < 64) {
    if (XF) { s_scale[tid] = a.in_scale[(size_t)seg * a.seg_stride + tid]; s_shift[tid] = a.in_shift[(size_t)seg * a.seg_stride + tid]; }
    const size_t mo = (size_t)seg * a.seg_stride + tid;
    s_bias[tid] = mk ? a.mask_scale[mo] : (a.bias ? a.bias[tid] : 0.f);
    if (mk) { s_msh[tid] = a.mask_shift[mo]; s_mmu[tid] = a.mask_mean[mo]; }
    else if (a.out_scale) s_msh[tid] = a.out_scale[tid];
  }
  const bool osc_on = !mk && !XF && a.out_scale != nullptr;
  for (int i = tid; i < 1024; i += 512) s_f[320 + i] = 0.f;

  const int chunk = gtid & 7;
  int role[NLD];
  const int rel_bias = a.W + 1;
  unsigned long long edge = 0;
  unsigned hvalid = 0;
#pragma unroll
  for (int i = 0; i < NLD; ++i) {
    const int sp = (gtid >> 3) + (GT / 8) * i;
    role[i] = rel_bias;
    if (sp < HP) {
      const int hr = sp / HWD, hc = sp - hr * HWD;
      role[i] = ((hr - 1) * a.W + hc - 1 + rel_bias) | ((((hr * PITCH + hc) * 128 + ((chunk ^ (hc & 7)) << 4)) >> 4) << 16);
      hvalid |= 1u << i;
      edge |= (unsigned long long)((hr == 0) | ((hr == HH - 1) << 1) | ((hc == 0) << 2) | ((hc == HWD - 1) << 3)) << (4 * i);
    }
  }
  int Bb[3][2], Ab[2];
#pragma unroll
  for (int kk = 0; kk < 2; ++kk) {
    const int ci = kk * 4 + g;
#pragma unroll
    for (int s = 0; s < 3; ++s) Bb[s][kk] = ((wq * 4) * PITCH + li + s) * 128 + ((ci ^ ((li + s) & 7)) << 4);
    Ab[kk] = li * 128 + ((ci ^ (li & 7)) << 4);
  }
  const char* xg = reinterpret_cast<const char*>(a.x) + (size_t)chunk * EPC * sizeof(T);

  struct Geo { int origin, n0, h0, w0; unsigned long long out; };
  auto geom = [&](int tile) {
    Geo q;
    int t = tile;
    const int tw_i = t % tiles_w; t /= tiles_w;
    const int th_i = t % tiles_h;
    q.n0 = t / tiles_h + seg_n0;
    q.h0 = th_i * TH; q.w0 = tw_i * TW;
    q.origin = (q.n0 * a.H + q.h0) * a.W + q.w0;
    q.out = (unsigned long long)((q.h0 == 0) | ((q.h0 + TH >= a.H) << 1) | ((q.w0 == 0) << 2) | ((q.w0 + TW >= a.W) << 3)) *
            0x1111111111111111ull;
    return q;
  };
  auto tile_of = [&](int k, bool& live) {
    const int t = first0 + grp + k * 2 * G;
    live = t < tiles_total;
    return live ? t : tiles_total - 1;
  };

  u32x4_t hreg[NLD];
  unsigned hin = 0;
  auto load_halo = [&](const Geo& q) {
    const unsigned long long bad = edge & q.out;
    hin = 0;
#pragma unroll
    for (int i = 0; i < NLD; ++i) {
      const bool ok = ((hvalid >> i) & 1u) && !((bad >> (4 * i)) & 0xfull);
      int rl = role[i];
      asm volatile("" : "+v"(rl));
      const int idx = q.origin + (ok ? (rl & 0xffff) - rel_bias : 0);
      hreg[i] = ld16_nt(xg + (unsigned)idx * (unsigned)(64 * sizeof(T)));
      hin |= (ok ? 1u : 0u) << i;
    }
  };
  auto xform_store = [&]() {
    float sc[EPC], sh[EPC];
    if (XF) {
      const f32x4_t c0 = *reinterpret_cast<const f32x4_t*>(s_scale + chunk * EPC), c1 = *reinterpret_cast<const f32x4_t*>(s_scale + chunk * EPC + 4);
      const f32x4_t h0 = *reinterpret_cast<const f32x4_t*>(s_shift + chunk * EPC), h1 = *reinterpret_cast<const f32x4_t*>(s_shift + chunk * EPC + 4);
#pragma unroll
      for (int e = 0; e < 4; ++e) { sc[e] = c0[e]; sc[4 + e] = c1[e]; sh[e] = h0[e]; sh[4 + e] = h1[e]; }
    }
#pragma unroll
    for (int i = 0; i < NLD; ++i) {
      u32x4_t v = hreg[i];
      if (XF) {
        float f[EPC];
        Elem<T>::unpack(v, f);
#pragma unroll
        for (int e = 0; e < EPC; ++e) f[e] = __builtin_amdgcn_fmed3f(fmaf(f[e], sc[e], sh[e]), relu_lo, __builtin_inff());
        v = PackH<T>::run(f);
      }
      const bool ok = (hin >> i) & 1u;
#pragma unroll
      for (int e = 0; e < 4; ++e) v[e] = ok ? v[e] : 0u;
      int rl = role[i];
      asm volatile("" : "+v"(rl));
      if ((hvalid >> i) & 1u) st16(s_halo + ((rl >> 12) & 0xffff0), v);
    }
  };

  char* yg = reinterpret_cast<char*>(a.y);
  const char* rg = OP == 0 ? nullptr : reinterpret_cast<const char*>(OP == 2 ? a.mask_x : a.residual);
  u32x4_t rres[RPRE ? TP : 1][RPRE ? RQ : 1];
  auto out_off = [&](const Geo& q, int p) {
    const int h = q.h0 + wq * 4 + p, w = q.w0 + li;
    return (unsigned)(((q.n0 * a.H + h) * a.W + w) * 64 + g * 8) * (unsigned)sizeof(T);
  };
  auto load_res = [&](const Geo& q) {
    if constexpr (RPRE) {
#pragma unroll
      for (int p = 0; p < TP; ++p)
#pragma unroll
        for (int qq = 0; qq < RQ; ++qq) rres[p][qq] = ld16(rg + out_off(q, p) + qq * 64);
    }
  };

  f32x4_t acc[TK][TP];
  u32x4_t A[2][TK], B[2][TP];
  auto frags = [&](int buf, int step) {
    const int tap = step >> 1, kk = step & 1;
    const int r = tap / 3, s = tap - 3 * r;
#pragma unroll
    for (int t = 0; t < TK; ++t) A[buf][t] = ld16(s_w + Ab[kk] + tap * WBUF + t * 2048);
#pragma unroll
    for (int p = 0; p < TP; ++p) B[buf][p] = ld16(s_halo + Bb[s][kk] + (p + r) * (PITCH * 128));
  };

  bool live = false, live_n = false;
  Geo cur = geom(tile_of(0, live));
  load_halo(cur);
  __builtin_amdgcn_s_waitcnt(0x0f70);
  SSLCR_PP_BAR();
  xform_store();
  Geo nxt = geom(tile_of(1, live_n));
  load_halo(nxt);
  SSLCR_PP_BAR();
  if (grp == 1) SSLCR_PP_BAR();

#ifdef SSLCR_PP_PROF
  unsigned long long pp_t[8] = {0, 0, 0, 0, 0, 0, 0, 0};
#endif
  for (int st = 0; st < nst; ++st) {
    PP_T(t0);
    frags(0, 0);
    __builtin_amdgcn_sched_barrier(0);
#pragma unroll
    for (int i = 0; i < 18; ++i) {
      if (i < 17) frags((i + 1) & 1, i + 1);
#pragma unroll
      for (int t = 0; t < TK; ++t)
#pragma unroll
        for (int p = 0; p < TP; ++p) {
          const bf16x8_t av = __builtin_bit_cast(bf16x8_t, A[i & 1][t]), bv = __builtin_bit_cast(bf16x8_t, B[i & 1][p]);
          if (i == 0) acc[t][p] = __builtin_amdgcn_mfma_f32_16x16x32_bf16(av, bv, f32x4_t{0.f, 0.f, 0.f, 0.f}, 0, 0, 0);
          else acc[t][p] = __builtin_amdgcn_mfma_f32_16x16x32_bf16(av, bv, acc[t][p], 0, 0, 0);
        }
      if (i < 17) {
#pragma unroll
        for (int q = 0; q < TK + TP; ++q) {
          __builtin_amdgcn_sched_group_barrier(0x100, 1, 0);
          __builtin_amdgcn_sched_group_barrier(0x008, (TK * TP) / (TK + TP), 0);
// ... 20 lines not shown
#pragma unroll
          for (int e = 0; e < EPC; ++e) {
            msc[e] = s_bias[kb + q * 32 + e]; msh[e] = s_msh[kb + q * 32 + e]; mmu[e] = s_mmu[kb + q * 32 + e];
            a1[e] = 0.f; a2[e] = 0.f;
          }
#pragma unroll
          for (int p = 0; p < TP; ++p) {
            float xr[EPC], vq[EPC];
            Elem<T>::unpack(rres[RPRE ? p : 0][RPRE ? q : 0], xr);
#pragma unroll
            for (int e = 0; e < EPC; ++e) {
              const int idx = q * EPC + e;
              const float y = acc[idx >> 2][p][idx & 3];
              const float gv = fmaf(xr[e], msc[e], msh[e]) > 0.f ? y : 0.f;
              vq[e] = gv;
              a1[e] += gv;
              a2[e] = fmaf(gv, xr[e] - mmu[e], a2[e]);
            }
            if (live) st16(yg + out_off(cur, p) + q * 64, PackH<T>::run(vq));
          }
#pragma unroll
          for (int e = 0; e < EPC; ++e) { s1[q * EPC + e] = a1[e]; s2[q * EPC + e] = a2[e]; }
        }
      } else {
        if (live) {
          if (OP == 0 && !a.bias && !a.relu) {
#pragma unroll
            for (int p = 0; p < TP; ++p)
#pragma unroll
              for (int q = 0; q < RQ; ++q) {
                float vq[EPC];
#pragma unroll
                for (int e = 0; e < EPC; ++e) vq[e] = acc[(q * EPC + e) >> 2][p][e & 3];
                st16(yg + out_off(cur, p) + q * 64, PackH<T>::run(vq));
              }
          } else {
            if (osc_on) {
#pragma unroll
              for (int j = 0; j < 4 * TK; ++j) {
                const float sj = s_msh[kb + (j >> 3) * 32 + (j & 7)];
#pragma unroll
                for (int p = 0; p < TP; ++p) acc[j >> 2][p][j & 3] *= sj;
              }
            }
            float bias[4 * TK];
#pragma unroll
            for (int j = 0; j < 4 * TK; ++j) bias[j] = s_bias[kb + (j >> 3) * 32 + (j & 7)];
            const float lo = a.relu ? 0.f : -__builtin_inff();
#pragma unroll
            for (int p = 0; p < TP; ++p)
#pragma unroll
              for (int q = 0; q < RQ; ++q) {
                float vq[EPC], rr[EPC];
                if constexpr (OP == 1) Elem<T>::unpack(rres[RPRE ? p : 0][RPRE ? q : 0], rr);
#pragma unroll
                for (int e = 0; e < EPC; ++e) {
                  float v = acc[(q * EPC + e) >> 2][p][e & 3] + bias[q * EPC + e];
                  if constexpr (OP == 1) v += rr[e];
                  vq[e] = __builtin_amdgcn_fmed3f(v, lo, __builtin_inff());
                }
                st16(yg + out_off(cur, p) + q * 64, PackH<T>::run(vq));
              }
          }
        }
        if (a.stats) {
#pragma unroll
          for (int t = 0; t < TK; ++t)
#pragma unroll
            for (int j = 0; j < 4; ++j) {
              float x1 = 0.f, x2 = 0.f;
#pragma unroll
              for (int p = 0; p < TP; ++p) { float q = acc[t][p][j]; x1 += q; x2 = fmaf(q, q, x2); }
              s1[t * 4 + j] = x1;
              s2[t * 4 + j] = x2;
            }
        }
      }
      if (a.stats) {
        row16_fold16(s1);
        row16_fold16(s2);
        if (live && (li & 3) == 0) {
          const int t = li >> 2;
          float* sp = s_stat + (wq * 2) * BKO + kb + (t >> 1) * 32 + (t & 1) * 4;
#pragma unroll
          for (int h = 0; h < 2; ++h) {
            const float* sv = h ? s2 : s1;
            f32x4_t* slot = reinterpret_cast<f32x4_t*>(sp + h * BKO);
            f32x4_t v = *slot;
#pragma unroll
            for (int e = 0; e < 4; ++e) v[e] += sv[e];
            *slot = v;
          }
        }
      }
    }
    PP_T(tb);
    PP_ACC(5, tb - ta);
    cur = nxt;
    live = live_n;
    nxt = geom(tile_of(st + 2, live_n));
    load_halo(nxt);
    PP_T(t3);
    if (!(grp == 1 && st == nst - 1)) SSLCR_PP_BAR();
    PP_T(t4);
    PP_ACC(2, t3 - t2); PP_ACC(3, t4 - t3);
  }
#ifdef SSLCR_PP_PROF
  if (blockIdx.x == 0 && lane == 0)
    for (int i = 0; i < 8; ++i) g_pp_prof[wave][i] = pp_t[i];
#endif
  SSLCR_PP_BAR();
  if (a.stats) {
    const int rw = tid >> 6, c = tid & 63;
    a.stats[((size_t)((int)blockIdx.x * 4 + (rw >> 1)) * 2 + (rw & 1)) * 64 + c] = s_f[320 + tid] + s_f[320 + 512 + tid];
    const int eb = (int)blockIdx.x + (int)gridDim.x;
    if (eb * 4 < rows_total) a.stats[((size_t)(eb * 4 + (rw >> 1)) * 2 + (rw & 1)) * 64 + c] = 0.f;
  }
}

static int pp64_grid(const ConvArgs& a) {
  const int nseg = a.seg_images > 0 ? a.N / a.seg_images : 1;
  const int tiles = (a.N / nseg) * (a.H / 16) * (a.W / 16);
  const int pairs = (tiles + 1) / 2, per = device_cus() / nseg;
  return (pairs < per ? pairs : per) * nseg;
}

bool conv_pp64_ok(int dtype, const ConvArgs& a) {
  static const bool on = [] { const char* e = getenv("SSLCR_PP64"); return !e || atoi(e) != 0; }();
  if ((size_t)a.N * a.H * a.W * 64 * 2 >= ((size_t)1 << 32)) return false;
  if (a.W > 2048) return false;
  return on && dtype == DT_BF16 && a.C == 64 && a.K == 64 && a.R == 3 && a.S == 3 && a.stride == 1 && a.pad == 1 && !a.transposed &&
         a.H % 16 == 0 && a.W % 16 == 0 && !(a.in_scale && (a.residual || a.mask_x)) &&
         !(a.out_scale && (a.in_scale || a.mask_x || a.stats || !a.bias));
}
int conv_pp64_rows(const ConvArgs& a) {
  if (a.seg_images > 0) return pp64_grid(a) * 4;
  const int tiles = a.N * (a.H / 16) * (a.W / 16);
  return (tiles < device_cus() ? tiles : device_cus()) * 4;
}

hipError_t launch_conv_pp64(const ConvArgs& a, hipStream_t st) {
  constexpr size_t lds = 9 * 64 * 128 + 2 * 18 * 18 * 128 + (320 + 1024) * sizeof(float);
  static std::atomic<bool> attr_done{false};
  if (!attr_done) {
    const void* ks[4] = {reinterpret_cast<const void*>(conv3x3_pp64_kernel<false, 0>), reinterpret_cast<const void*>(conv3x3_pp64_kernel<false, 1>),
                         reinterpret_cast<const void*>(conv3x3_pp64_kernel<false, 2>), reinterpret_cast<const void*>(conv3x3_pp64_kernel<true, 0>)};
    for (const void* k : ks) {
      hipError_t e = hipFuncSetAttribute(k, hipFuncAttributeMaxDynamicSharedMemorySize, 160 * 1024);
      if (e != hipSuccess) return e;
    }
    attr_done = true;
  }
  const int nseg = a.seg_images > 0 ? a.N / a.seg_images : 1;
  const int tiles = (a.N / nseg) * (a.H / 16) * (a.W / 16);
  const int grid = pp64_grid(a);
  if (a.mask_x && !a.stats) return hipErrorInvalidValue;
  const int rows = conv_pp64_rows(a);
  if (a.in_scale) hipLaunchKernelGGL((conv3x3_pp64_kernel<true, 0>), dim3(grid), dim3(512), lds, st, a, tiles, rows);
  else if (a.mask_x) hipLaunchKernelGGL((conv3x3_pp64_kernel<false, 2>), dim3(grid), dim3(512), lds, st, a, tiles, rows);
  else if (a.residual) hipLaunchKernelGGL((conv3x3_pp64_kernel<false, 1>), dim3(grid), dim3(512), lds, st, a, tiles, rows);
  else hipLaunchKernelGGL((conv3x3_pp64_kernel<false, 0>), dim3(grid), dim3(512), lds, st, a, tiles, rows);
  return hipGetLastError();
}

const char* conv_pp64_name(const ConvArgs& a) {
  if (a.in_scale) return "sslcr::conv3x3_pp64_kernel<true, 0>";
  return a.mask_x ? "sslcr::conv3x3_pp64_kernel<false, 2>" : (a.residual ? "sslcr::conv3x3_pp64_kernel<false, 1>" : "sslcr::conv3x3_pp64_kernel<false, 0>");
}

}
```

ssl_cr_histo_amd/csrc/engine.cpp:

```cpp
#include <rccl/rccl.h>
#include <stdio.h>
#include <stdlib.h>
#include <string.h>

#include <atomic>
#include <chrono>
#include <condition_variable>
#include <mutex>
#include <vector>

#include "kernels.hpp"

using namespace sslcr;

#define TRY(expr)                                   \
  do {                                              \
    hipError_t _e = (expr);                         \
    if (_e != hipSuccess) return check(_e, #expr);  \
  } while (0)
#define TRYI(expr)            \
  do {                        \
    int _r = (expr);          \
    if (_r != 0) return _r;   \
  } while (0)
// ... 217 lines not shown
    ch.slot[ph][r] = nullptr; ch.cap[ph][r] = 0;
    TRY(hipMalloc(&ch.slot[ph][r], (bytes + 255) & ~(size_t)255));
    ch.cap[ph][r] = (bytes + 255) & ~(size_t)255;
  }
  if (!ch.ev_in[ph][r]) {
    TRY(hipEventCreateWithFlags(&ch.ev_in[ph][r], hipEventDisableTiming));
    TRY(hipEventCreateWithFlags(&ch.ev_out[ph][r], hipEventDisableTiming));
  }
  TRY(hipMemcpyAsync(ch.slot[ph][r], buf, bytes, hipMemcpyDeviceToDevice, st));
  TRY(hipEventRecord(ch.ev_in[ph][r], st));
  {
    std::unique_lock<std::mutex> lk(ch.m);
    const long g = ch.gen;
    if (++ch.arrived == W) {
      ch.arrived = 0; ++ch.gen;
      ch.cv.notify_all();
    } else if (!ch.cv.wait_for(lk, std::chrono::seconds(120), [&] { return ch.gen != g; })) {
      --ch.arrived;
      c->vcomm->poisoned = true;
      ch.cv.notify_all();
      return fail("virtual all-reduce: rank %d waited 120 s for its peers (channel %d); the communicator is now unusable", r, chan);
    }
  }
  VSrc src;
  for (int q = 0; q < W; ++q) {
    src.p[q] = ch.slot[ph][q];
    if (q != r) TRY(hipStreamWaitEvent(st, ch.ev_in[ph][q], 0));
  }
  const int blocks = (int)((count + 255) / 256 < 1024 ? (count + 255) / 256 : 1024);
  if (f64) hipLaunchKernelGGL(vsum_kernel<double>, dim3(blocks), dim3(256), 0, st, (double*)buf, src, W, count);
  else hipLaunchKernelGGL(vsum_kernel<float>, dim3(blocks), dim3(256), 0, st, (float*)buf, src, W, count);
  TRY(hipGetLastError());
  TRY(hipEventRecord(ch.ev_out[ph][r], st));
  ch.out_set[ph][r] = true;
  return 0;
}

int all_reduce(sslcr_ctx* c, int chan, void* buf, size_t count, bool f64, hipStream_t st) {
  if (c->vcomm) return vcomm_all_reduce(c, chan, buf, count, f64, st);
  TRYN(ncclAllReduce(buf, buf, count, f64 ? ncclDouble : ncclFloat, ncclSum, chan == 0 ? c->comm : c->comm_g, st));
  return 0;
}

hipError_t prof_conv(sslcr_ctx* c, int dt, const ConvArgs& a, hipStream_t st) {
  if (!c->prof.on) return launch_conv(dt, a, st);
  ProfRec r;
  r.e0 = c->prof.get(); r.e1 = c->prof.get();
  const double es = c->esz();
  const double rs = a.tap_mask ? (double)__builtin_popcount(a.tap_mask) : (double)a.R * a.S;
  const double M = (double)a.N * a.PH * a.PW;
  const double src = (double)a.N * a.H * a.W;
  r.flops = a.transposed ? 2.0 * src * a.C * a.K * rs : 2.0 * M * a.K * a.C * rs;
  r.bytes = (src * a.C + (double)a.K * rs * a.C + M * a.K * (a.residual ? 2.0 : 1.0) * (a.accumulate ? 2.0 : 1.0)) * es;
  r.name = conv_kernel_name(dt, a);
  (void)hipEventRecord(r.e0, st);
  hipError_t e = launch_conv(dt, a, st);
  (void)hipEventRecord(r.e1, st);
  c->prof.rec[0].push_back(r);
  return e;
}
hipError_t prof_conv_pair(sslcr_ctx* c, const ConvArgs& a, const ConvArgs& d, hipStream_t st) {
  if (!c->prof.on) return launch_conv_s2(a, &d, st);
  ProfRec r;
  r.e0 = c->prof.get(); r.e1 = c->prof.get();
  const double es = c->esz();
  const double M = (double)a.N * a.PH * a.PW, src = (double)a.N * a.H * a.W;
  r.flops = 2.0 * M * a.K * a.C * 10.0;
  r.bytes = (src * a.C + (double)a.K * 10.0 * a.C + 2.0 * M * a.K) * es;
  r.name = conv_s2_name(a, true);
  (void)hipEventRecord(r.e0, st);
  hipError_t e = launch_conv_s2(a, &d, st);
  (void)hipEventRecord(r.e1, st);
  c->prof.rec[0].push_back(r);
  return e;
}
inline bool fp8_layer(const sslcr_ctx* c, const ConvL& L) {
  return c->fp8 && L.k == 3 && L.stride == 1 && L.cin % 128 == 0 && L.cout % 128 == 0;
}
inline bool use_fp8(const sslcr_ctx* c, const ConvL& L, const ConvArgs& a) { return fp8_layer(c, L) && L.w8_fwd && conv_fp8_mode(a) != 0; }
hipError_t prof_conv_fwd(sslcr_ctx* c, int dt, const ConvArgs& a_in, const ConvL& L, bool folded, hipStream_t st) {
  ConvArgs a = a_in;
  a.out_scale = nullptr;
  if (!use_fp8(c, L, a)) return prof_conv(c, dt, a_in, st);
  Fp8Args q;
  q.w8 = folded ? L.w8_fold : L.w8_fwd;
  q.w_dequant = folded ? L.dq_fold : L.dq_fwd;
  q.x_scale = 1.0f;
  q.x_scale_dev = L.f8s ? L.f8s + (folded ? 2 : 0) : nullptr;
  q.amax_out = L.f8s ? L.f8s + (folded ? 3 : 1) : nullptr;
  if (!c->prof.on) return launch_conv_fp8(a, q, st);
  ProfRec r;
  r.e0 = c->prof.get(); r.e1 = c->prof.get();
  const double M = (double)a.N * a.PH * a.PW;
  r.flops = 2.0 * M * a.K * a.C * 9.0;
  r.bytes = ((double)a.N * a.H * a.W * a.C + M * a.K * (a.residual ? 2.0 : 1.0)) * 2.0 + (double)a.K * 9.0 * a.C;
  r.name = conv_fp8_name(a);
  (void)hipEventRecord(r.e0, st);
  hipError_t e = launch_conv_fp8(a, q, st);
  (void)hipEventRecord(r.e1, st);
  c->prof.rec[0].push_back(r);
  return e;
}
hipError_t prof_wgrad(sslcr_ctx* c, int dt, const WgradArgs& a, hipStream_t st) {
  if (!c->prof.on) return launch_wgrad(dt, a, st);
  ProfRec r;
  r.e0 = c->prof.get(); r.e1 = c->prof.get();
// ... 290 lines not shown
    o_bits[i] = take(s_bits[i]);
    if (s_bits[i] * 8 != (size_t)N * d.lh[i] * d.lw[i] * kBlockCfg[i][1]) bits_ok = false;
  }
  const size_t s_bn = 20 * 4 * 512 * sizeof(float), s_E = (size_t)N * 512 * sizeof(float);
  const size_t o_bn = take(s_bn), o_E = take(s_E);
  TRYI(n->pass[0].mem.ensure(c.off));
  char* b = (char*)n->pass[0].mem.p;
  for (int p = 0; p < npass; ++p) {
    PassState& ps = n->pass[p];
    ps.raw0 = b + o_raw0 + p * s_raw0; ps.pooled = b + o_pool + p * s_pool; ps.argmax = (uint8_t*)(b + o_arg + p * s_arg);
    for (int i = 0; i < 8; ++i) {
      ps.blk[i].raw1 = b + o_blk[i][0] + p * s_blk[i]; ps.blk[i].raw2 = b + o_blk[i][1] + p * s_blk[i];
      ps.blk[i].rawd = n->blocks[i].has_ds ? b + o_blk[i][2] + p * s_blk[i] : nullptr;
      ps.blk[i].y = b + o_blk[i][3] + p * s_blk[i];
      ps.blk[i].ybits = (uint8_t*)(b + o_bits[i] + p * s_bits[i]);
    }
    float* f = (float*)(b + o_bn + p * s_bn);
    for (int i = 0; i < 20; ++i) {
      ps.bn[i] = BnSaved{f, f + 512, f + 1024, f + 1536};
      f += 2048;
    }
    ps.E = (float*)(b + o_E + p * s_E);
    ps.N = N; ps.H = H; ps.W = W;
  }
  n->ybits_ok = bits_ok;
  return 0;
}

int forward_stem(sslcr_net* n, PassState& ps, const void* x, int in_f32, int N, int H, int W, int replay, hipStream_t st) {
  sslcr_ctx* c = n->ctx;
  const int dt = c->dtype;
  const Dims d = make_dims(H, W);
  ps.x = x; ps.in_f32 = in_f32;
  StemArgs a;
  memset(&a, 0, sizeof(a));
  a.x = x; a.x2 = ps.x2; a.n_split = ps.n_split; a.w = n->stem.w_fwd; a.y = ps.raw0;
  a.N = N; a.H = H; a.W = W; a.OH = d.oh0; a.OW = d.ow0; a.in_f32 = in_f32;
  const int rows = stem_partials_rows(a);
  TRYI(c->partials.ensure((size_t)rows * 2 * 64 * sizeof(float)));
  a.stats = (float*)c->partials.p;
  TRY(launch_stem(dt, a, st));
  TRYI(finalize_bn(n, n->bn0, a.stats, rows, (double)N * d.oh0 * d.ow0, ps.bn[0], replay, st));
  PoolFwdArgs p;
  memset(&p, 0, sizeof(p));
  p.x = ps.raw0; p.scale = ps.bn[0].scale; p.shift = ps.bn[0].shift; p.y = ps.pooled; p.argmax = ps.argmax;
  p.N = N; p.H = d.oh0; p.W = d.ow0; p.C = 64; p.OH = d.ph; p.OW = d.pw;
  TRY(launch_bn_relu_maxpool(dt, p, st));
  return 0;
}

bool ybits_on(const sslcr_ctx* c) {
  static const bool on = [] { const char* e = getenv("SSLCR_YBITS"); return !e || atoi(e) != 0; }();
  return on && c->dtype == DT_BF16;
}
const uint8_t* ybits_of(const sslcr_net* n, const void* yact) {
  if (!yact || !n->ybits_ok || !ybits_on(n->ctx)) return nullptr;
  for (int p = 0; p < 3; ++p)
    for (int i = 0; i < 8; ++i)
      if (n->pass[p].blk[i].y == yact) return n->pass[p].blk[i].ybits;
  return nullptr;
}

int forward_blocks(sslcr_net* n, PassState& ps, int N, int H, int W, int replay, int nseg, hipStream_t st) {
  sslcr_ctx* c = n->ctx;
  const int dt = c->dtype;
  const Dims d = make_dims(H, W);
  const bool segs = nseg > 1;
  const int NT = nseg * N;
  const int seg_stride = segs ? (int)(n->pass[1].bn[0].scale - n->pass[0].bn[0].scale) : 0;
  const char* X = ps.pooled;
  int xh = d.ph, xw = d.pw;
  for (int i = 0; i < 8; ++i) {
    BlockL& B = n->blocks[i];
    const int oh = d.lh[i], ow = d.lw[i];
    const double cnt = (double)N * oh * ow;
    float* part; int rows;
    ConvArgs a1 = conv_args(B.c1, X, B.c1.w_fwd, ps.blk[i].raw1, NT, xh, xw);
    if (segs) a1.seg_images = N;
    ConvArgs ad;
    bool paired = false;
    if (B.has_ds) {
      ad = conv_args(B.ds, X, B.ds.w_fwd, ps.blk[i].rawd, NT, xh, xw);
      if (segs) ad.seg_images = N;
      ConvArgs t1 = a1, td = ad;
      t1.stats = td.stats = c->zeros;
      paired = !use_fp8(c, B.c1, a1) && conv_s2_pair_ok(dt, t1, td);
    }
    if (paired) {
      if (segs && (!conv_segments_ok(dt, a1) || !conv_segments_ok(dt, ad))) return fail("forward_blocks: the paired stride-2 launch has no segment form here");
      rows = conv_partials_rows(a1);
      const size_t rb = (size_t)rows * 2 * a1.K * sizeof(float);
      TRYI(c->partials.ensure(2 * rb));
      part = (float*)c->partials.p;
      a1.stats = part;
      ad.stats = (float*)((char*)c->partials.p + rb);
      TRY(prof_conv_pair(c, a1, ad, st));
      TRYI(finalize_bn_pair(n, B.b1, a1.stats, rows, B.bd, ad.stats, rows, cnt, ps.bn[B.b1.bidx], ps.bn[B.bd.bidx], replay, st, nseg, seg_stride));
    } else if (B.has_ds) {
      const int rows1 = conv_partials_rows(a1), rowsd = conv_partials_rows(ad);
      const size_t rb1 = (((size_t)rows1 * 2 * a1.K * sizeof(float)) + 255) & ~(size_t)255;
      TRYI(c->partials.ensure(rb1 + (size_t)rowsd * 2 * ad.K * sizeof(float)));
      a1.stats = (float*)c->partials.p;
      ad.stats = (float*)((char*)c->partials.p + rb1);
      TRY(prof_conv(c, dt, a1, st));
      TRY(prof_conv(c, dt, ad, st));
      TRYI(finalize_bn_pair(n, B.b1, a1.stats, rows1, B.bd, ad.stats, rowsd, cnt, ps.bn[B.b1.bidx], ps.bn[B.bd.bidx], replay, st, nseg, seg_stride));
// ... 377 lines not shown
  TRY(prof_wgrad(c, c->dtype, a, c->wg_stream));
  TRY(hipEventRecord(c->ev_wg_done[kind], c->wg_stream));
  c->wg_pending[kind] = true;
  c->wg_any = true;
  return 0;
}

int launch_bucket_allreduce(sslcr_net* n, int bucket, size_t lo, size_t hi, hipStream_t st) {
  sslcr_ctx* c = n->ctx;
  if (!sharded(c) || hi <= lo) return 0;
  TRY(hipEventRecord(c->ev_ready[bucket], st));
  TRY(hipStreamWaitEvent(c->comm_stream, c->ev_ready[bucket], 0));
  TRYI(wg_join(c, c->comm_stream));
  float* g = (float*)n->grads.p + lo;
  TRYI(all_reduce(c, 1, g, hi - lo, false, c->comm_stream));
  return 0;
}

int lowest_trainable(const sslcr_net* n) {
  for (int i = 0; i < 60; ++i)
    if (n->rg[i]) return i;
  return 60;
}

int backbone_backward(sslcr_net* n, int npass, hipStream_t st) {
  sslcr_ctx* c = n->ctx;
  const int dt = c->dtype;
  const size_t es = c->esz();
  PassState* P = n->pass;
  const int N = P[0].N;
  const Dims d = make_dims(P[0].H, P[0].W);
  const int low = lowest_trainable(n);
  if (low >= 60) return 0;
  const size_t unit = (((size_t)N * d.ph * d.pw * 64 * es) + 255) & ~(size_t)255;
  const size_t stem_sz = (((size_t)N * d.oh0 * d.ow0 * 64 * es) + 255) & ~(size_t)255;
  TRYI(c->scratch.ensure(7 * npass * unit + stem_sz));
  char* S = (char*)c->scratch.p;
  auto buf = [&](int kind, int p, size_t bytes) { return S + (size_t)kind * npass * unit + (size_t)p * bytes; };
  int kOut = 0, kXin = 5;
  const int kG = 1, kRaw2 = 2, kAct1 = 3, kRaw1 = 4, kRawD = 6;
  char* dRaw0 = S + (size_t)7 * npass * unit;
  auto tap = [&](int blk, int slot, const void* src, int n_, int h_, int w_, int c_) -> int {
    if (!n->tap) return 0;
    const size_t bytes = (size_t)n_ * h_ * w_ * c_ * es;
    TRYI(n->tapbuf[blk][slot].ensure(bytes));
    TRY(hipMemcpyAsync(n->tapbuf[blk][slot].p, src, bytes, hipMemcpyDeviceToDevice, st));
    int* d4 = n->tapdims[blk][slot];
    d4[0] = n_; d4[1] = h_; d4[2] = w_; d4[3] = c_;
    return 0;
  };

  size_t hi_pending = n->goff[60];
  int bucket = 1;
  for (int p = 0; p < npass; ++p)
    TRY(launch_avgpool_bwd(dt, n->dE[p], buf(kOut, p, (size_t)N * d.lh[7] * d.lw[7] * 512 * es), N, d.lh[7] * d.lw[7], 512, st));
  for (int i = 7; i >= 0; --i) {
    BlockL& B = n->blocks[i];
    const int oh = d.lh[i], ow = d.lw[i];
    const int xh = i == 0 ? d.ph : d.lh[i - 1], xw = i == 0 ? d.pw : d.lw[i - 1];
    const size_t opix = (size_t)N * oh * ow;
    const bool need_dx = low < B.pstart;
    const size_t so = opix * B.c2.cout * es, si = (size_t)N * xh * xw * B.c1.cin * es;
    bool c2_batched = false;
    if (npass > 1) {
      WgradArgs q;
      memset(&q, 0, sizeof(q));
      q.N = N * npass; q.H = oh; q.W = ow; q.C = B.c2.cin; q.K = B.c2.cout; q.R = 3; q.S = 3; q.stride = 1; q.pad = 1; q.OH = oh; q.OW = ow;
      c2_batched = wgrad_halo_tw(q) != 0 && (wgrad_halo_tw(q) == 16 || N % 2 == 0);
    }
    ConvArgs seg_m;
    bool seg_dg = false;
    if (npass > 1 && segments_on() && !c->prof.on) {
      seg_m = conv_args(B.c2, nullptr, B.c2.w_dg, nullptr, N * npass, oh, ow);
      seg_m.C = B.c2.cout; seg_m.K = B.c2.cin; seg_m.transposed = 0; seg_m.PH = oh; seg_m.PW = ow; seg_m.OH = oh; seg_m.OW = ow;
      const BnSaved& s1 = P[0].bn[B.b1.bidx];
      seg_m.mask_x = P[0].blk[i].raw1; seg_m.mask_scale = s1.scale; seg_m.mask_shift = s1.shift; seg_m.mask_mean = s1.mean;
      seg_m.seg_images = N; seg_m.seg_stride = (int)(P[1].bn[B.b1.bidx].scale - s1.scale);
      seg_dg = conv_h16_ok(dt, seg_m) && conv_segments_ok(dt, seg_m) && conv_partials_rows(seg_m) % npass == 0;
    }
    const bool seg_bn = npass > 1 && segments_on() && !c->prof.on && !(sharded(c) && c->bn_sync) && c->bn_ring.p &&
                        c->bn_ring_i + 2 * npass <= sslcr_ctx::kBnRing;
    const int bn_stride = npass > 1 ? (int)(P[1].bn[0].scale - P[0].bn[0].scale) : 0;
    if (seg_bn) {
      char *dOut = buf(kOut, 0, so), *G = buf(kG, 0, so), *dRaw2 = buf(kRaw2, 0, so), *dRawD = buf(kRawD, 0, so);
      TRYI(wg_wait(c, 0, st));
      if (B.has_ds) TRYI(wg_wait(c, 2, st));
      const size_t apix = opix * npass;
      if (B.has_ds) {
        BnBwdArgs a2, ad;
        double* sums_2 = take_sums_n(c, npass);
        if (!sums_2) return fail("backbone_backward: ring slots");
        TRYI(bn_bwd_begin(n, B.b2, P[0].bn[B.b2.bidx], dOut, P[0].blk[i].raw2, P[0].blk[i].y, 0, dRaw2, G, apix, (double)opix, st, sums_2, &a2, nullptr, 1,
                          nullptr, 0, true, npass, bn_stride));
        TRYI(bn_bwd_begin(n, B.bd, P[0].bn[B.bd.bidx], G, P[0].blk[i].rawd, nullptr, 0, dRawD, nullptr, apix, (double)opix, st, sums_2 + 2 * B.b2.C, &ad,
                          nullptr, 0, nullptr, 0, true, npass, bn_stride));
        TRYI(bn_bwd_end(c, a2, st));
        TRYI(bn_bwd_end(c, ad, st));
      } else {
        TRYI(bn_backward(n, B.b2, P[0].bn[B.b2.bidx], dOut, P[0].blk[i].raw2, P[0].blk[i].y, 0, dRaw2, G, apix, (double)opix, st, nullptr, 1, nullptr, 0,
                         npass, bn_stride));
      }
      TRYI(tap(i, 0, G, N, oh, ow, B.c2.cout));
      TRYI(tap(i, 1, dRaw2, N, oh, ow, B.c2.cout));
      if (B.has_ds) TRYI(tap(i, 4, dRawD, N, oh, ow, B.ds.cout));
    }
    for (int p = 0; p < npass; ++p) {
      PassState& ps = P[p];
      char *dOut = buf(kOut, p, so), *G = buf(kG, p, so), *dRaw2 = buf(kRaw2, p, so), *dAct1 = buf(kAct1, p, so), *dRaw1 = buf(kRaw1, p, so),
           *dRawD = buf(kRawD, p, so);
      if (!seg_bn) {
      TRYI(wg_wait(c, 0, st));
      if (B.has_ds) TRYI(wg_wait(c, 2, st));
      if (B.has_ds) {
        BnBwdArgs a2, ad;
        double* ring = take_sums(c);
        double* sums_2 = ring ? ring : c->bn_sums;
        double* sums_d = sums_2 + 2 * B.b2.C;
        TRYI(bn_bwd_begin(n, B.b2, ps.bn[B.b2.bidx], dOut, ps.blk[i].raw2, ps.blk[i].y, 0, dRaw2, G, opix, (double)opix, st, sums_2, &a2, nullptr, 1,
                          nullptr, 0, ring != nullptr, 1, 0, true));
        TRYI(bn_bwd_begin(n, B.bd, ps.bn[B.bd.bidx], G, ps.blk[i].rawd, nullptr, 0, dRawD, nullptr, opix, (double)opix, st, sums_d, &ad, nullptr, 0,
                          nullptr, 0, ring != nullptr, 1, 0, true));
        const bool pair = bn_bwd_pair_ok(a2, ad);
        static const bool g_free = [] { const char* e = getenv("SSLCR_BN_PAIR_G"); return e && atoi(e) == 0; }();
        const int keep_g = (n->tap || !a2.yact_bits || !g_free) ? 1 : 0;
        if (pair) {
          TRY(launch_bn_bwd_reduce_pair(dt, a2, ad, keep_g, st));
        } else {
          TRY(launch_bn_bwd_reduce(dt, a2, st));
          TRY(launch_bn_bwd_reduce(dt, ad, st));
        }
        TRYI(bn_bwd_sync(c, sums_2, 4 * (size_t)B.b2.C, st));
        if (pair) {
          if (c->prof.on) {
            ProfRec r;
            r.e0 = c->prof.get(); r.e1 = c->prof.get();
            r.name = dt == DT_BF16 ? "sslcr::bn_bwd_apply_pair_kernel<unsigned short>" : "sslcr::bn_bwd_apply_pair_kernel<float>";
            r.flops = 0.0;
            r.bytes = (keep_g ? 5.0 : 5.0625) * (double)opix * B.b2.C * c->esz();
            (void)hipEventRecord(r.e0, st);
            hipError_t e = launch_bn_bwd_apply_pair(dt, a2, ad, keep_g, st);
            (void)hipEventRecord(r.e1, st);
            c->prof.rec[2].push_back(r);
            TRY(e);
          } else {
            TRY(launch_bn_bwd_apply_pair(dt, a2, ad, keep_g, st));
          }
        } else {
          TRYI(bn_bwd_end(c, a2, st));
          TRYI(bn_bwd_end(c, ad, st));
        }
      } else {
        TRYI(bn_backward(n, B.b2, ps.bn[B.b2.bidx], dOut, ps.blk[i].raw2, ps.blk[i].y, 0, dRaw2, G, opix, (double)opix, st, nullptr, 1));
      }
      if (p == 0) {
        TRYI(tap(i, 0, G, N, oh, ow, B.c2.cout));
        TRYI(tap(i, 1, dRaw2, N, oh, ow, B.c2.cout));
        if (B.has_ds) TRYI(tap(i, 4, dRawD, N, oh, ow, B.ds.cout));
      }
      }
      if (!c2_batched) TRYI(wgrad_call(n, B.c2, ps.blk[i].raw1, dRaw2, &ps.bn[B.b1.bidx], N, oh, ow, oh, ow, st, 0, 0, 0));
      if (seg_dg) continue;
      float* b1_rows = nullptr;
      int b1_nrows = 0;
      {
        ConvArgs a = conv_args(B.c2, dRaw2, B.c2.w_dg, dAct1, N, oh, ow);
        a.C = B.c2.cout; a.K = B.c2.cin; a.transposed = 0; a.PH = oh; a.PW = ow; a.OH = oh; a.OW = ow;
        ConvArgs m = a;
        const BnSaved& s1 = ps.bn[B.b1.bidx];
        m.mask_x = ps.blk[i].raw1; m.mask_scale = s1.scale; m.mask_shift = s1.shift; m.mask_mean = s1.mean;
        if (conv_h16_ok(dt, m)) {
          TRYI(ensure_partials(c, m, &b1_rows, &b1_nrows));
          m.stats = b1_rows;
          a = m;
        }
        TRY(prof_conv(c, dt,a, st));
        if (p == 0) {
          TRYI(tap(i, 2, dAct1, N, oh, ow, B.c2.cin));
          n->tap_flags[i] = b1_rows ? 1 : 0;
        }
      }
      TRYI(wg_wait(c, 1, st));
      TRYI(bn_backward(n, B.b1, ps.bn[B.b1.bidx], dAct1, ps.blk[i].raw1, nullptr, b1_rows ? 0 : 1, dRaw1, nullptr, opix, (double)opix, st,
                       nullptr, 0, b1_rows, b1_nrows));
      if (p == 0) TRYI(tap(i, 3, dRaw1, N, oh, ow, B.c1.cout));
    }
    if (seg_dg) {
      float* rows = nullptr;
      int nrows = 0;
      seg_m.x = buf(kRaw2, 0, so); seg_m.y = buf(kAct1, 0, so);
      TRYI(ensure_partials(c, seg_m, &rows, &nrows));
      seg_m.stats = rows;
      TRY(prof_conv(c, dt, seg_m, st));
      TRYI(tap(i, 2, buf(kAct1, 0, so), N, oh, ow, B.c2.cin));
      n->tap_flags[i] = 1;
      const int per = nrows / npass;
      if (seg_bn) {
        TRYI(wg_wait(c, 1, st));
        TRYI(bn_backward(n, B.b1, P[0].bn[B.b1.bidx], buf(kAct1, 0, so), P[0].blk[i].raw1, nullptr, 0, buf(kRaw1, 0, so), nullptr, opix * npass,
                         (double)opix, st, nullptr, 0, rows, nrows, npass, bn_stride));
        TRYI(tap(i, 3, buf(kRaw1, 0, so), N, oh, ow, B.c1.cout));
      }
      for (int p = 0; p < npass && !seg_bn; ++p) {
        PassState& ps = P[p];
        TRYI(wg_wait(c, 1, st));
        TRYI(bn_backward(n, B.b1, ps.bn[B.b1.bidx], buf(kAct1, p, so), ps.blk[i].raw1, nullptr, 0, buf(kRaw1, p, so), nullptr, opix, (double)opix, st,
                         nullptr, 0, rows + (size_t)p * per * 2 * B.b1.C, per));
        if (p == 0) TRYI(tap(i, 3, buf(kRaw1, 0, so), N, oh, ow, B.c1.cout));
      }
    }
    if (c2_batched)
      TRYI(wgrad_call(n, B.c2, P[0].blk[i].raw1, buf(kRaw2, 0, so), &P[0].bn[B.b1.bidx], N * npass, oh, ow, oh, ow, st, N,
                      (int)(P[1].bn[B.b1.bidx].scale - P[0].bn[B.b1.bidx].scale), 0));
    {
      const char* X0 = i == 0 ? P[0].pooled : P[0].blk[i - 1].y;
      TRYI(wgrad_call(n, B.c1, X0, buf(kRaw1, 0, so), nullptr, N * npass, xh, xw, oh, ow, st, 0, 0, 1));
      if (B.has_ds) TRYI(wgrad_call(n, B.ds, X0, buf(kRawD, 0, so), nullptr, N * npass, xh, xw, oh, ow, st, 0, 0, 2));
    }
    if (need_dx) {
      {
        const int NB = N * npass;
        char *G = buf(kG, 0, so), *dRaw1 = buf(kRaw1, 0, so), *dXin = buf(kXin, 0, si), *dRawD = buf(kRawD, 0, so);
        ConvArgs a = conv_args(B.c1, dRaw1, B.c1.w_dg, dXin, NB, oh, ow);
        a.C = B.c1.cout; a.K = B.c1.cin; a.transposed = (B.c1.stride == 1) ? 0 : 1; a.PH = xh; a.PW = xw; a.OH = xh; a.OW = xw;
        if (!B.has_ds) a.residual = G;
        if (B.c1.stride == 1) {
          TRY(prof_conv(c, dt,a, st));
        } else {
          ConvArgs q4 = a;
          q4.pix_mul = 2; q4.PH = xh / 2; q4.PW = xw / 2; q4.par4 = 1;
          const bool one = xh % 2 == 0 && xw % 2 == 0 && conv_dma_bp(dt, q4) != 0 && conv_dma_bp(DT_BF16, q4) == conv_dma_bp(dt, q4) &&
                           conv_halo_tw(dt, q4) == 0;
          if (one) TRY(prof_conv(c, dt, q4, st));
          for (int par = 0; par < (one ? 0 : 4); ++par) {
            ConvArgs q = a;
            const int ph_ = par >> 1, pw_ = par & 1;
            q.pix_mul = 2; q.pix_off_h = ph_; q.pix_off_w = pw_;
            q.PH = (xh - ph_ + 1) / 2; q.PW = (xw - pw_ + 1) / 2;
            if (q.PH <= 0 || q.PW <= 0) continue;
            unsigned m = 0;
            for (int r = 0; r < 3; ++r)
              for (int s2 = 0; s2 < 3; ++s2)
                if (((ph_ + 1 - r) & 1) == 0 && ((pw_ + 1 - s2) & 1) == 0) m |= 1u << (r * 3 + s2);
            q.tap_mask = m;
            TRY(prof_conv(c, dt,q, st));
          }
        }
        if (B.has_ds) {
          ConvArgs s = conv_args(B.ds, dRawD, B.ds.w_dg, dXin, NB, oh, ow);
          s.C = B.ds.cout; s.K = B.ds.cin; s.stride = 1; s.pad = 0; s.PH = oh; s.PW = ow; s.OH = xh; s.OW = xw; s.osh = B.ds.stride;
          s.accumulate = 1;
          TRY(prof_conv(c, dt,s, st));
        }
        TRYI(tap(i, 5, dXin, N, xh, xw, B.c1.cin));
      }
      const int t = kOut; kOut = kXin; kXin = t;
    }
    if (i == 6 || i == 4 || i == 2) {
      TRYI(launch_bucket_allreduce(n, bucket++, n->goff[B.pstart], hi_pending, st));
      hi_pending = n->goff[B.pstart];
    }
    if (!need_dx) break;
  }
  if (low < 3) {
    for (int p = 0; p < npass; ++p) {
      PassState& ps = P[p];
      PoolSrc pool{buf(kOut, p, (size_t)N * d.ph * d.pw * 64 * es), ps.argmax, d.oh0, d.ow0, d.ph, d.pw, ps.pooled};
      const size_t spix = (size_t)N * d.oh0 * d.ow0;
      StemWgradArgs w;
      memset(&w, 0, sizeof(w));
      w.x = ps.x; w.x2 = ps.x2; w.n_split = ps.n_split; w.dy = dRaw0; w.dw = (float*)n->grads.p + n->goff[0];
      w.N = N; w.H = ps.H; w.W = ps.W; w.OH = d.oh0; w.OW = d.ow0; w.in_f32 = ps.in_f32;
      if (n->rg[0] && c->fuse_stem_bwd) {
        BnBwdArgs a;
        double* ring = take_sums(c);
        double* sums0 = ring ? ring : c->bn_sums;
        TRYI(bn_bwd_begin(n, n->bn0, ps.bn[0], nullptr, ps.raw0, nullptr, 1, nullptr, nullptr, spix, (double)spix, st, sums0, &a, &pool, 0, nullptr, 0,
                          ring != nullptr));
        TRYI(bn_bwd_sync(c, sums0, 2 * 64, st));
        w.dy = nullptr;
        if (c->prof.on) {
          ProfRec r;
          r.e0 = c->prof.get(); r.e1 = c->prof.get();
          r.name = dt == DT_BF16 ? "sslcr::stem_wgrad_kernel<unsigned short, pool>" : "sslcr::stem_wgrad_kernel<float, pool>";
          r.flops = 0.0;
          const double t = (double)spix * 64 * c->esz();
          r.bytes = 0.25 * t + 0.25 * (double)spix * 64 + t + (double)N * 3 * ps.H * ps.W * (ps.in_f32 ? 4 : 1);
          (void)hipEventRecord(r.e0, st);
          hipError_t e = launch_stem_wgrad_pool(dt, w, a, st);
          (void)hipEventRecord(r.e1, st);
          c->prof.rec[2].push_back(r);
          TRY(e);
        } else {
          TRY(launch_stem_wgrad_pool(dt, w, a, st));
        }
        continue;
      }
      TRYI(bn_backward(n, n->bn0, ps.bn[0], nullptr, ps.raw0, nullptr, 1, dRaw0, nullptr, spix, (double)spix, st, &pool));
      if (n->rg[0]) TRY(launch_stem_wgrad(dt, w, st));
    }
  }
  TRYI(launch_bucket_allreduce(n, bucket, 0, hi_pending, st));
  return 0;
}

int net_forward(sslcr_net* n, int train, const void* const* xs, int in_f32, int N, int H, int W, float* feats, float* logits, hipStream_t st) {
  if (!(train ? n->packed_train : n->packed_eval)) TRYI(sslcr_net_pack(n, train ? 1 : 2, st));
  const int npass_ = n->triplet ? 3 : 1;
  if (n->n8 > 0 && !n->f8_cal[train ? 0 : 1]) {
    n->f8_calib_pass = true;
// ... 556 lines not shown
```

ssl_cr_histo_amd/csrc/kernels.hpp:

```cpp
#pragma once
#include "common.hpp"
#include "../../include/sslcr.h"

namespace sslcr {

using ConvArgs = sslcr_conv_desc;
using WgradArgs = sslcr_wgrad_desc;
using StemArgs = sslcr_stem_desc;
using StemWgradArgs = sslcr_stem_wgrad_desc;
using BnFinalizeArgs = sslcr_bn_finalize_desc;
using BnActArgs = sslcr_bn_act_desc;
using PoolFwdArgs = sslcr_pool_fwd_desc;
using PoolBwdArgs = sslcr_pool_bwd_desc;
using BnBwdArgs = sslcr_bn_bwd_desc;
using LossArgs = sslcr_loss_desc;
using TensorDesc = sslcr_tensor_desc;
using OptArgs = sslcr_opt_desc;
using PackArgs = sslcr_pack_desc;
using Fp8Args = sslcr_fp8_desc;
using PackFp8Args = sslcr_pack_fp8_desc;

hipError_t launch_conv(int dtype, const ConvArgs& a, hipStream_t st);
int conv_tile_bp(const ConvArgs& a);
const char* conv_kernel_name(int dtype, const ConvArgs& a);
const char* wgrad_kernel_name(int dtype, const WgradArgs& a);
int conv_partials_rows(const ConvArgs& a);
bool conv_segments_ok(int dtype, const ConvArgs& a);
int device_cus();
int conv_halo_tw(int dtype, const ConvArgs& a);
int conv_halo_tiles(const ConvArgs& a, int tw);
hipError_t launch_conv_halo(int dtype, const ConvArgs& a, int tw, hipStream_t st);
int conv_halo256_mode(int dtype, const ConvArgs& a);
int conv_halo256_tiles(const ConvArgs& a, int mode);
hipError_t launch_conv_halo256(int dtype, const ConvArgs& a, int mode, hipStream_t st);
bool conv_h16_ok(int dtype, const ConvArgs& a);
int conv_h16_rows(const ConvArgs& a);
hipError_t launch_conv_h16(int dtype, const ConvArgs& a, hipStream_t st);
const char* conv_h16_name(int dtype, const ConvArgs& a);
bool conv_pp64_ok(int dtype, const ConvArgs& a);
hipError_t launch_conv_pp64(const ConvArgs& a, hipStream_t st);
const char* conv_pp64_name(const ConvArgs& a);
int conv_pp64_rows(const ConvArgs& a);
int conv_dma_bp(int dtype, const ConvArgs& a);
int conv_dma_rows(const ConvArgs& a, int bp);
hipError_t launch_conv_dma(int dtype, const ConvArgs& a, int bp, hipStream_t st);
const char* conv_dma_name(int dtype, int bp);
bool conv_s2_ok(int dtype, const ConvArgs& a);
bool conv_s2_pair_ok(int dtype, const ConvArgs& a, const ConvArgs& d);
int conv_s2_rows(const ConvArgs& a);
hipError_t launch_conv_s2(const ConvArgs& a, const ConvArgs* d, hipStream_t st);
const char* conv_s2_name(const ConvArgs& a, bool pair);
bool conv_s2d_ok(int dtype, const ConvArgs& a);
hipError_t launch_conv_s2d(const ConvArgs& a, hipStream_t st);
const char* conv_s2d_name();
int conv_fp8_mode(const ConvArgs& a);
int conv_fp8_rows(const ConvArgs& a);
const char* conv_fp8_name(const ConvArgs& a);
hipError_t launch_conv_fp8(const ConvArgs& a, const Fp8Args& q, hipStream_t st);
hipError_t launch_pack_fp8(const PackFp8Args& a, hipStream_t st);
hipError_t launch_fp8_scale_update(float* slots, int n, hipStream_t st);
hipError_t launch_wgrad(int dtype, const WgradArgs& a, hipStream_t st);
int wgrad_halo_tw(const WgradArgs& a);
void* stream_scratch(hipStream_t st, size_t bytes);
void stream_scratch_release();
hipError_t launch_wgrad_fold(const void* slabs, float* dw, int C, int gx, int gy, int splits, int taps, int kh_n, hipStream_t st);
hipError_t launch_stem_wgrad_fold(const void* slabs, float* dw, int nwg, hipStream_t st);
hipError_t launch_wgrad_halo(int dtype, const WgradArgs& a, int tw, hipStream_t st);
bool wgrad_dma_ok(int dtype, const WgradArgs& a, int splits);
bool wgrad_dma_used(int dtype, const WgradArgs& a);
hipError_t launch_wgrad_dma(const WgradArgs& a, int tw, int tps, int ntiles, int splits, void* slabs, hipStream_t st);
hipError_t launch_probe_tr16(const uint16_t* in, const int* byte_addr, uint16_t* out, hipStream_t st);
bool wgrad_s2_ok(int dtype, const WgradArgs& a);
hipError_t launch_wgrad_s2(const WgradArgs& a, hipStream_t st);
hipError_t launch_stem(int dtype, const StemArgs& a, hipStream_t st);
int stem_partials_rows(const StemArgs& a);
hipError_t launch_stem_wgrad(int dtype, const StemWgradArgs& a, hipStream_t st);
hipError_t launch_stem_wgrad_pool(int dtype, const StemWgradArgs& a, const sslcr_bn_bwd_desc& b, hipStream_t st);
bool stem_pool_ok(int dtype, const StemArgs& a, int POH, int POW);
hipError_t launch_stem_pool(int dtype, const StemArgs& a, int POH, int POW, hipStream_t st);
hipError_t launch_bn_finalize(const BnFinalizeArgs& a, hipStream_t st);
hipError_t launch_bn_act(int dtype, const BnActArgs& a, hipStream_t st);
hipError_t launch_bn_relu_maxpool(int dtype, const PoolFwdArgs& a, hipStream_t st);
hipError_t launch_maxpool_relu_bwd(int dtype, const PoolBwdArgs& a, hipStream_t st);
hipError_t launch_avgpool_fwd(int dtype, const void* x, float* y, int N, int HW, int C, hipStream_t st);
hipError_t launch_avgpool_bwd(int dtype, const float* dy, void* dx, int N, int HW, int C, hipStream_t st);
hipError_t launch_bn_bwd_reduce(int dtype, const BnBwdArgs& a, hipStream_t st);
hipError_t launch_bn_bwd_apply(int dtype, const BnBwdArgs& a, hipStream_t st);
bool bn_bwd_pair_ok(const BnBwdArgs& a, const BnBwdArgs& b);
hipError_t launch_bn_bwd_reduce_pair(int dtype, const BnBwdArgs& a, const BnBwdArgs& b, int keep_g, hipStream_t st);
hipError_t launch_bn_bwd_apply_pair(int dtype, const BnBwdArgs& a, const BnBwdArgs& b, int from_g, hipStream_t st);
hipError_t launch_bn_param_grads(const double* sums, const float* invstd, float* dgamma, float* dbeta, int C, hipStream_t st);
hipError_t launch_bn_param_grads_scaled(const double* sums, const float* invstd, float* dgamma, float* dbeta, int C, float scale, hipStream_t st);
hipError_t launch_linear_fwd(const float* x, const float* w, const float* b, float* y, int M, int N, int K, int relu, hipStream_t st);
hipError_t launch_linear_bwd(const float* x, const float* w, const float* dy, const float* yact, float* dx, float* dw, float* db,
                             int M, int N, int K, int dx_accumulate, float* scratch, hipStream_t st);
hipError_t launch_loss(const LossArgs& a, hipStream_t st);
hipError_t launch_softmax_col(const float* logits, float* out, int n, int C, int col, hipStream_t st);
hipError_t launch_weak_augment(const sslcr_weak_aug_desc& a, hipStream_t st);
hipError_t launch_hed_colour(const sslcr_colour_aug_desc& a, hipStream_t st);
hipError_t launch_brightness_contrast(const sslcr_brightness_contrast_desc& a, hipStream_t st);
hipError_t launch_optimizer(const TensorDesc* d_descs, int ntensors, int max_n, const OptArgs& o, hipStream_t st);
constexpr int OPT_CHUNK = 2048;
constexpr int OPT_TILE = 16 * 16 * 9;
hipError_t launch_optimizer_chunks(const TensorDesc* d_descs, const void* d_chunks , int nchunks,
                                   const OptArgs& o, hipStream_t st);
hipError_t launch_axpby(float* p, float* q, size_t n, float alpha, int copy_back, hipStream_t st);
hipError_t launch_fill(float* p, size_t n, float v, hipStream_t st);
hipError_t launch_pack_conv(int dtype, const PackArgs& a, hipStream_t st);
hipError_t launch_pack_stem(int dtype, const PackArgs& a, hipStream_t st);
hipError_t launch_copy2d(float* dst, long ldd, const float* src, long lds, int rows, int w, int accumulate, hipStream_t st);
hipError_t launch_copy2d_multi(float* dst, long ldd, int ndst, long dstep, const float* src, long lds, int nsrc, long sstep, int rows, int w,
                               hipStream_t st);
hipError_t launch_unpack_grad(const float* g, float* out, int K, int C, int RS, hipStream_t st);
int fail(const char* fmt, ...);
int check(hipError_t e, const char* what);

}
```

ssl_cr_histo_amd/kernels.py:

```python
import torch

from . import _lib as L

F32, BF16 = 0, 1


def tdtype(dtype):
    return torch.bfloat16 if dtype == BF16 else torch.float32


def _dt(t):
    if t.dtype == torch.bfloat16:
        return BF16
    if t.dtype == torch.float32:
        return F32
    raise TypeError(f"unsupported activation dtype {t.dtype}")


def _chk(*ts):
    for t in ts:
        if t is not None:
            if not t.is_cuda:
                raise L.SslcrError("sslcr kernels need device tensors (no CPU fallback)")
            if not t.is_contiguous():
                raise L.SslcrError("sslcr kernels need contiguous tensors")


last_conv_kernel = ""
last_wgrad_kernel = ""


def conv2d(x, w, stride, pad, *, in_scale=None, in_shift=None, in_relu=False, bias=None, residual=None, relu=False,
           want_stats=False, out=None, transposed=False, out_hw=None, osh=1, accumulate=False, pixel_hw=None,
           pix_mul=0, pix_off=(0, 0), tap_mask=0, mask=None, par4=False, seg_images=0, out_scale=None):
    _chk(x, w, in_scale, in_shift, bias, residual, out, out_scale)
    dt = _dt(x)
    N, H, W, C = x.shape
    K, R, S, C2 = w.shape
    assert C2 == C and w.dtype == x.dtype
    if transposed:
        PH, PW = pixel_hw
    else:
        PH, PW = (H + 2 * pad - R) // stride + 1, (W + 2 * pad - S) // stride + 1
    OH, OW = out_hw if out_hw is not None else (PH * osh, PW * osh)
    y = out if out is not None else torch.empty((N, OH, OW, K), dtype=x.dtype, device=x.device)
    d = L.ConvDesc(L.ptr(x), L.ptr(w), L.ptr(y), L.ptr(in_scale), L.ptr(in_shift), L.ptr(bias), L.ptr(residual), None,
                   N, H, W, C, K, R, S, stride, pad, PH, PW, OH, OW, osh, int(transposed), int(in_relu), int(relu),
                   int(accumulate), int(pix_mul), int(pix_off[0]), int(pix_off[1]), int(tap_mask))
    d.par4 = int(par4)
    d.out_scale = L.ptr(out_scale)
    if seg_images:
        d.seg_images = int(seg_images)
        d.seg_stride = int(in_scale.stride(0)) if in_scale is not None and in_scale.dim() == 2 else 0
        if not L.lib().sslcr_conv2d_segments_ok(dt, d):
            raise L.SslcrError("conv2d: no segment form for this shape / dtype")
    if mask is not None:
        _chk(*mask)
        d.mask_x, d.mask_scale, d.mask_shift, d.mask_mean = (L.ptr(t) for t in mask)
    stats = None
    if want_stats:
        rows = L.lib().sslcr_conv2d_partial_rows(d)
        stats = torch.full((rows, 2, K), float("nan"), dtype=torch.float32, device=x.device)
        d.stats = L.ptr(stats)
    global last_conv_kernel
    last_conv_kernel = L.lib().sslcr_conv2d_kernel_name(dt, d).decode()
    L.check(L.lib().sslcr_conv2d(dt, d, L.stream_ptr()))
    return (y, stats) if want_stats else y


def conv2d_s2_pair(x, w3, w1, *, bias3=None, bias1=None, relu3=False, want_stats=False, scale3=None, scale1=None):
    _chk(x, w3, w1, bias3, bias1, scale3, scale1)
    dt = _dt(x)
    N, H, W, C = x.shape
    K = w3.shape[0]
    assert w3.shape == (K, 3, 3, C) and w1.shape == (K, 1, 1, C)
    PH, PW = H // 2, W // 2
    y3 = torch.empty((N, PH, PW, K), dtype=x.dtype, device=x.device)
    yd = torch.empty_like(y3)
    d3 = L.ConvDesc(L.ptr(x), L.ptr(w3), L.ptr(y3), None, None, L.ptr(bias3), None, None,
                    N, H, W, C, K, 3, 3, 2, 1, PH, PW, PH, PW, 1, 0, 0, int(relu3), 0, 0, 0, 0, 0)
    d1 = L.ConvDesc(L.ptr(x), L.ptr(w1), L.ptr(yd), None, None, L.ptr(bias1), None, None,
                    N, H, W, C, K, 1, 1, 2, 0, PH, PW, PH, PW, 1, 0, 0, 0, 0, 0, 0, 0, 0)
    d3.out_scale, d1.out_scale = L.ptr(scale3), L.ptr(scale1)
    s3 = sd = None
    if want_stats:
        rows = L.lib().sslcr_conv2d_partial_rows(d3)
        s3 = torch.full((rows, 2, K), float("nan"), dtype=torch.float32, device=x.device)
        sd = torch.full((rows, 2, K), float("nan"), dtype=torch.float32, device=x.device)
        d3.stats, d1.stats = L.ptr(s3), L.ptr(sd)
    if not L.lib().sslcr_conv2d_s2_pair_ok(dt, d3, d1):
        raise L.SslcrError("conv2d_s2_pair: not served")
    L.check(L.lib().sslcr_conv2d_s2_pair(dt, d3, d1, L.stream_ptr()))
    return (y3, yd, s3, sd) if want_stats else (y3, yd)


def pack_conv_fp8(w_kcrs, *, bn=None, eps=1e-5):
    _chk(w_kcrs)
    K, C, R, S = w_kcrs.shape
    assert R == 3 and S == 3
    dev = w_kcrs.device
    w8 = torch.empty((K, 3, 3, C), dtype=torch.uint8, device=dev)
    dq = torch.empty(K, dtype=torch.float32, device=dev)
    bias = torch.empty(K, dtype=torch.float32, device=dev) if bn is not None else None
# ... 147 lines not shown
    scale, shift, mean, invstd = (torch.empty(shape, dtype=torch.float32, device=dev) for _ in range(4))
    stage = torch.empty((max(nseg, 1), 32, 2, Cn), dtype=torch.float64, device=dev)
    tickets = torch.zeros((Cn + 31) // 32, dtype=torch.int32, device=dev) if one_launch else None
    d = L.BnFinalizeDesc(L.ptr(partials), rows, Cn, float(count), L.ptr(gamma), L.ptr(beta), L.ptr(scale), L.ptr(shift),
                         L.ptr(mean), L.ptr(invstd), L.ptr(running_mean), L.ptr(running_var), L.ptr(nbt), momentum, eps,
                         replay, None, None, L.ptr(stage), nseg if nseg > 1 else 0, Cn if nseg > 1 else 0, L.ptr(tickets))
    L.check(L.lib().sslcr_bn_finalize(d, L.stream_ptr()))
    return scale, shift, mean, invstd


def bn_act(x, scale, shift, *, res=None, rscale=None, rshift=None, relu=True, nseg=1, want_bits=False):
    _chk(x, scale, shift, res, rscale, rshift)
    y = torch.empty_like(x)
    Cn = x.shape[-1]
    d = L.BnActDesc(L.ptr(x), L.ptr(scale), L.ptr(shift), L.ptr(res), L.ptr(rscale), L.ptr(rshift), L.ptr(y),
                    x.numel() // Cn, Cn, int(relu), nseg if nseg > 1 else 0, Cn if nseg > 1 else 0)
    bits = None
    if want_bits:
        bits = torch.full((x.numel() // 8,), 0xa5, dtype=torch.uint8, device=x.device)
        d.ybits = L.ptr(bits)
    L.check(L.lib().sslcr_bn_act(_dt(x), d, L.stream_ptr()))
    return (y, bits) if want_bits else y


def bn_relu_maxpool(x, scale, shift):
    _chk(x, scale, shift)
    N, H, W, Cn = x.shape
    OH, OW = (H - 1) // 2 + 1, (W - 1) // 2 + 1
    y = torch.empty((N, OH, OW, Cn), dtype=x.dtype, device=x.device)
    am = torch.empty((N, OH, OW, Cn), dtype=torch.uint8, device=x.device) if scale is not None else None
    d = L.PoolFwdDesc(L.ptr(x), L.ptr(scale), L.ptr(shift), L.ptr(y), L.ptr(am), N, H, W, Cn, OH, OW)
    L.check(L.lib().sslcr_bn_relu_maxpool(_dt(x), d, L.stream_ptr()))
    return y, am


def maxpool_relu_bwd(dy, argmax, x, scale, shift):
    _chk(dy, argmax, x, scale, shift)
    N, H, W, Cn = x.shape
    _, OH, OW, _ = dy.shape
    dx = torch.empty_like(x)
    d = L.PoolBwdDesc(L.ptr(dy), L.ptr(argmax), L.ptr(x), L.ptr(scale), L.ptr(shift), L.ptr(dx), N, H, W, Cn, OH, OW)
    L.check(L.lib().sslcr_maxpool_relu_bwd(_dt(x), d, L.stream_ptr()))
    return dx


def avgpool_fwd(x):
    _chk(x)
    N, H, W, Cn = x.shape
    y = torch.empty((N, Cn), dtype=torch.float32, device=x.device)
    L.check(L.lib().sslcr_avgpool_fwd(_dt(x), L.ptr(x), L.ptr(y), N, H * W, Cn, L.stream_ptr()))
    return y


def avgpool_bwd(dy, shape, dtype):
    _chk(dy)
    N, H, W, Cn = shape
    dx = torch.empty(shape, dtype=tdtype(dtype), device=dy.device)
    L.check(L.lib().sslcr_avgpool_bwd(dtype, L.ptr(dy), L.ptr(dx), N, H * W, Cn, L.stream_ptr()))
    return dx


def bn_bwd(dy, x, scale, shift, mean, invstd, *, yact=None, relu_from_x=False, want_g=False, count=None, pool=None,
           g_in_reduce=False, nseg=1, dgamma=None, dbeta=None, yact_bits=None):
    _chk(x, scale, shift, mean, invstd, yact, dgamma, dbeta)
    if dy is not None:
        _chk(dy)
    Cn = x.shape[-1]
    pixels = x.numel() // Cn
    sums = torch.zeros((nseg, 2, Cn) if nseg > 1 else (2, Cn), dtype=torch.float64, device=x.device)
    dx = torch.empty_like(x)
    g = torch.empty_like(x) if want_g else None
    d = L.BnBwdDesc(L.ptr(dy), L.ptr(x), L.ptr(yact), L.ptr(scale), L.ptr(shift), L.ptr(mean), L.ptr(invstd), L.ptr(sums),
                    L.ptr(dx), L.ptr(g), pixels, Cn, int(relu_from_x), float(count if count is not None else pixels // nseg),
                    None, None, 0, 0, 0, 0, None, int(g_in_reduce))
    if dgamma is not None:
        d.dgamma, d.dbeta, d.pg_scale = L.ptr(dgamma), L.ptr(dbeta), 1.0
    if yact_bits is not None:
        _chk(yact_bits)
        d.yact_bits = L.ptr(yact_bits)
    if nseg > 1:
        d.nseg, d.seg_stride, d.sums_stride = nseg, Cn, 2 * Cn
    if pool is not None:
        pdy, pam = pool[0], pool[1]
        _chk(pdy, pam)
        d.pool_dy, d.pool_argmax = L.ptr(pdy), L.ptr(pam)
        if len(pool) > 2 and pool[2] is not None:
            _chk(pool[2])
            d.pool_y = L.ptr(pool[2])
        d.pH, d.pW, d.pOH, d.pOW = x.shape[1], x.shape[2], pdy.shape[1], pdy.shape[2]
    L.check(L.lib().sslcr_bn_bwd_reduce(_dt(x), d, L.stream_ptr()))
    L.check(L.lib().sslcr_bn_bwd_apply(_dt(x), d, L.stream_ptr()))
    return dx, sums, g


def bn_param_grads(sums, invstd, dgamma, dbeta):
    _chk(sums, invstd, dgamma, dbeta)
    L.check(L.lib().sslcr_bn_param_grads(L.ptr(sums), L.ptr(invstd), L.ptr(dgamma), L.ptr(dbeta), invstd.numel(),
                                         L.stream_ptr()))


def linear_fwd(x, w, b, relu=False):
    _chk(x, w, b)
    M, K = x.shape
    N = w.shape[0]
    y = torch.empty((M, N), dtype=torch.float32, device=x.device)
    L.check(L.lib().sslcr_linear_fwd(L.ptr(x), L.ptr(w), L.ptr(b), L.ptr(y), M, N, K, int(relu), L.stream_ptr()))
    return y


def linear_bwd(x, w, dy, *, yact=None, dw=None, db=None, want_dx=True, dx=None, dx_accumulate=False):
    _chk(x, w, dy, yact, dw, db, dx)
# ... 30 lines not shown
```

Measured before the change: 68260.

## Fuse ReLU gradient masking into dgrad conv epilogue and avgpool backward

Adds an out_bits path. The dgrad conv epilogue and the avgpool backward apply the next block's saved ReLU bitmask directly, producing the masked gradient G in place. BN backward can then treat the incoming gradient as ready and skip reading the activation and writing a separate G buffer. The aim is to cut elementwise memory traffic in the backward pass. It adds a new conv kernel variant with register-packing tricks in the halo loader, which may raise register pressure, and it is gated by SSLCR_GMASK.

```diff
diff --git a/include/sslcr.h b/include/sslcr.h
--- a/include/sslcr.h
+++ b/include/sslcr.h
@@ -37,6 +37,7 @@
   int par4;
   int seg_images, seg_stride;
   const float* out_scale;
+  const uint8_t* out_bits;
 } sslcr_conv_desc;
 int sslcr_conv2d(int dtype, const sslcr_conv_desc* d, void* stream);
 int sslcr_conv2d_partial_rows(const sslcr_conv_desc* d);
@@ -137,6 +138,7 @@
 
 int sslcr_avgpool_fwd(int dtype, const void* x, float* y, int N, int HW, int C, void* stream);
 int sslcr_avgpool_bwd(int dtype, const float* dy, void* dx, int N, int HW, int C, void* stream);
+int sslcr_avgpool_bwd_bits(int dtype, const float* dy, void* dx, const uint8_t* bits, int N, int HW, int C, void* stream);
 
 typedef struct sslcr_bn_bwd_desc {
   const void* dy; const void* x; const void* yact;
diff --git a/ssl_cr_histo_amd/_lib.py b/ssl_cr_histo_amd/_lib.py
--- a/ssl_cr_histo_amd/_lib.py
+++ b/ssl_cr_histo_amd/_lib.py
@@ -22,7 +22,7 @@
               [(k, i32) for k in ("N", "H", "W", "C", "K", "R", "S", "stride", "pad", "PH", "PW", "OH", "OW", "osh",
                                   "transposed", "in_relu", "relu", "accumulate", "pix_mul", "pix_off_h", "pix_off_w")] +
               [("tap_mask", C.c_uint), ("mask_x", vp), ("mask_scale", vp), ("mask_shift", vp), ("mask_mean", vp),
-               ("par4", i32), ("seg_images", i32), ("seg_stride", i32), ("out_scale", vp)])
+               ("par4", i32), ("seg_images", i32), ("seg_stride", i32), ("out_scale", vp), ("out_bits", vp)])
 WgradDesc = _S("WgradDesc", [("x", vp), ("dy", vp), ("dw", vp), ("in_scale", vp), ("in_shift", vp), ("in_relu", i32)] +
                [(k, i32) for k in ("N", "H", "W", "C", "K", "R", "S", "stride", "pad", "OH", "OW", "seg_images", "seg_stride")])
 StemDesc = _S("StemDesc", [("x", vp), ("w", vp), ("y", vp), ("bias", vp), ("stats", vp)] +
@@ -92,6 +92,7 @@
     "sslcr_maxpool_relu_bwd": (i32, [i32, P(PoolBwdDesc), vp]),
     "sslcr_avgpool_fwd": (i32, [i32, vp, vp, i32, i32, i32, vp]),
     "sslcr_avgpool_bwd": (i32, [i32, vp, vp, i32, i32, i32, vp]),
+    "sslcr_avgpool_bwd_bits": (i32, [i32, vp, vp, vp, i32, i32, i32, vp]),
     "sslcr_bn_bwd_reduce": (i32, [i32, P(BnBwdDesc), vp]),
     "sslcr_bn_bwd_apply": (i32, [i32, P(BnBwdDesc), vp]),
     "sslcr_bn_param_grads": (i32, [vp, vp, vp, vp, i32, vp]),
diff --git a/ssl_cr_histo_amd/csrc/bn_eltwise.hip b/ssl_cr_histo_amd/csrc/bn_eltwise.hip
--- a/ssl_cr_histo_amd/csrc/bn_eltwise.hip
+++ b/ssl_cr_histo_amd/csrc/bn_eltwise.hip
@@ -557,6 +557,26 @@
     st16_nt(dx + i * 16, Elem<T>::pack(f));
   }
 }
+__global__ __launch_bounds__(256) void avgpool_bwd_bits_kernel(const float* dy, void* dxv, const uint8_t* __restrict__ bits, int N, int HW, int C) {
+  typedef bf16_t T;
+  constexpr int EPC = Elem<T>::EPC;
+  const int cols = C / EPC;
+  const size_t total = (size_t)N * HW * cols;
+  char* dx = reinterpret_cast<char*>(dxv);
+  const float inv = 1.f / (float)HW;
+  for (size_t i = (size_t)blockIdx.x * 256 + threadIdx.x; i < total; i += (size_t)gridDim.x * 256) {
+    const int col = (int)(i % cols);
+    const int n = (int)(i / ((size_t)HW * cols));
+    const unsigned b = bits[i];
+    float f[EPC];
+#pragma unroll
+    for (int e = 0; e < EPC; ++e) {
+      f[e] = dy[(size_t)n * C + col * EPC + e] * inv;
+      if (!((b >> e) & 1u)) f[e] = 0.f;
+    }
+    st16_nt(dx + i * 16, Elem<T>::pack(f));
+  }
+}
 
 hipError_t launch_avgpool_fwd(int dtype, const void* x, float* y, int N, int HW, int C, hipStream_t st) {
   if (dtype == DT_BF16) {
@@ -566,7 +586,12 @@
   }
   return hipGetLastError();
 }
-hipError_t launch_avgpool_bwd(int dtype, const float* dy, void* dx, int N, int HW, int C, hipStream_t st) {
+hipError_t launch_avgpool_bwd(int dtype, const float* dy, void* dx, int N, int HW, int C, hipStream_t st, const uint8_t* bits) {
+  if (bits) {
+    if (dtype != DT_BF16) return hipErrorInvalidValue;
+    hipLaunchKernelGGL(avgpool_bwd_bits_kernel, dim3(ew_grid((size_t)N * HW * (C / 8))), dim3(256), 0, st, dy, dx, bits, N, HW, C);
+    return hipGetLastError();
+  }
   if (dtype == DT_BF16) {
     hipLaunchKernelGGL(avgpool_bwd_kernel<bf16_t>, dim3(ew_grid((size_t)N * HW * (C / 8))), dim3(256), 0, st, dy, dx, N, HW, C);
   } else {
@@ -1029,15 +1054,19 @@
   return fold();
 }
 
+static bool bn_bwd_pair_g_ready(const BnBwdArgs& a) {
+  return !a.g_in_reduce && a.gout && a.dy == a.gout && !a.yact && !a.yact_bits && !a.relu_from_x;
+}
 bool bn_bwd_pair_ok(const BnBwdArgs& a, const BnBwdArgs& b) {
   static const bool on = [] { const char* e = getenv("SSLCR_BN_PAIR"); return !e || atoi(e) != 0; }();
-  return on && a.g_in_reduce && a.gout && b.dy == a.gout && !b.yact && !b.yact_bits && !b.relu_from_x && !b.gout && !a.pool_dy && !b.pool_dy &&
+  return on && (a.g_in_reduce || bn_bwd_pair_g_ready(a)) && a.gout && b.dy == a.gout && !b.yact && !b.yact_bits && !b.relu_from_x && !b.gout && !a.pool_dy && !b.pool_dy &&
          a.nseg <= 1 && b.nseg <= 1 && a.C == b.C && a.pixels == b.pixels && b.sums == a.sums + 2 * a.C && a.dx && b.dx && b.x && a.x;
 }
 hipError_t launch_bn_bwd_reduce_pair(int dtype, const BnBwdArgs& a, const BnBwdArgs& b, int keep_g, hipStream_t st) {
   const int epc = dtype == DT_BF16 ? 8 : 4;
   const int cols = a.C / epc;
   if (cols > 256 || (256 % cols) != 0 || !bn_bwd_pair_ok(a, b)) return hipErrorInvalidValue;
+  if (bn_bwd_pair_g_ready(a)) keep_g = 0;
   const int rpp = 256 / cols;
   size_t blocks = (a.pixels + rpp - 1) / rpp;
   blocks = (blocks + 7) / 8;
@@ -1072,6 +1101,7 @@
 }
 hipError_t launch_bn_bwd_apply_pair(int dtype, const BnBwdArgs& a, const BnBwdArgs& b, int from_g, hipStream_t st) {
   if (!bn_bwd_pair_ok(a, b)) return hipErrorInvalidValue;
+  if (bn_bwd_pair_g_ready(a)) from_g = 1;
   if (dtype == DT_BF16) hipLaunchKernelGGL(bn_bwd_apply_pair_kernel<bf16_t>, dim3(ew_grid(a.pixels * (a.C / 8))), dim3(256), 0, st, a, b, from_g);
   else hipLaunchKernelGGL(bn_bwd_apply_pair_kernel<float>, dim3(ew_grid(a.pixels * (a.C / 4))), dim3(256), 0, st, a, b, from_g);
   return hipGetLastError();
diff --git a/ssl_cr_histo_amd/csrc/capi.cpp b/ssl_cr_histo_amd/csrc/capi.cpp
--- a/ssl_cr_histo_amd/csrc/capi.cpp
+++ b/ssl_cr_histo_amd/csrc/capi.cpp
@@ -29,7 +29,7 @@
 
 extern "C" {
 
-int sslcr_version(void) { return 6; }
+int sslcr_version(void) { return 7; }
 const char* sslcr_last_error(void) { return g_err; }
 
 int sslcr_conv2d(int dtype, const sslcr_conv_desc* d, void* stream) {
@@ -40,6 +40,7 @@
   NEED(d->K % 64 == 0, "K % 64");
   NEED(d->osh >= 1 && d->PH > 0 && d->PW > 0, "pixel space");
   NEED(conv_segments_ok(dtype, *d), "seg_images: no segment form for this shape / dtype (sslcr_conv2d_segments_ok)");
+  NEED(!d->out_bits || conv_out_bits_ok(dtype, *d), "out_bits: bf16, no stats / mask_x / in_scale / out_scale, and only where the kernel serving the shape has the form");
   return check(launch_conv(dtype, *d, (hipStream_t)stream), "conv2d");
 }
 int sslcr_conv2d_partial_rows(const sslcr_conv_desc* d) { return d ? conv_partials_rows(*d) : -1; }
@@ -148,6 +149,11 @@
   NEED(dy && dx && N > 0 && HW > 0 && C % 8 == 0, "args");
   return check(launch_avgpool_bwd(dtype, dy, dx, N, HW, C, (hipStream_t)stream), "avgpool_bwd");
 }
+int sslcr_avgpool_bwd_bits(int dtype, const float* dy, void* dx, const uint8_t* bits, int N, int HW, int C, void* stream) {
+  NEED(dtype == SSLCR_BF16, "mask bits: bf16 only");
+  NEED(dy && dx && bits && N > 0 && HW > 0 && C % 8 == 0, "args");
+  return check(launch_avgpool_bwd(dtype, dy, dx, N, HW, C, (hipStream_t)stream, bits), "avgpool_bwd_bits");
+}
 int sslcr_bn_bwd_reduce(int dtype, const sslcr_bn_bwd_desc* d, void* stream) {
   DT_OK(dtype);
   NEED(d && (d->dy || (d->pool_dy && d->pool_argmax)) && d->x && d->sums && d->mean, "null");
diff --git a/ssl_cr_histo_amd/csrc/conv_h16.hip b/ssl_cr_histo_amd/csrc/conv_h16.hip
--- a/ssl_cr_histo_amd/csrc/conv_h16.hip
+++ b/ssl_cr_histo_amd/csrc/conv_h16.hip
@@ -39,13 +39,19 @@
 template <typename T, int BKO, int WK, bool XF, bool WR, bool RAW = false, int TW = 16>
 __global__ __launch_bounds__(256 * WK, WK == 1 ? 1 : 2) void conv3x3_h16_kernel(const ConvArgs a, const int tiles_total, const int n_items, const int kshift,
                                                                                 const int row0) {
-  constexpr bool OSC = false;
+  constexpr bool OSC = false, OBITS = false;
 #include "conv_h16_body.hpp"
 }
 template <typename T, int BKO, int WK, bool WR, int TW>
 __global__ __launch_bounds__(256 * WK, WK == 1 ? 1 : 2) void conv3x3_h16s_kernel(const ConvArgs a, const int tiles_total, const int n_items, const int kshift,
                                                                                  const int row0) {
-  constexpr bool OSC = true, XF = false, RAW = false;
+  constexpr bool OSC = true, OBITS = false, XF = false, RAW = false;
+#include "conv_h16_body.hpp"
+}
+template <typename T, int BKO, int WK, int TW>
+__global__ __launch_bounds__(256 * WK, WK == 1 ? 1 : 2) void conv3x3_h16m_kernel(const ConvArgs a, const int tiles_total, const int n_items, const int kshift,
+                                                                                 const int row0) {
+  constexpr bool OSC = false, OBITS = true, XF = false, WR = false, RAW = false;
 #include "conv_h16_body.hpp"
 }
 
@@ -56,8 +62,13 @@
   if (q == 8 && on8 && conv_halo256_mode(DT_BF16, a) == 8 && a.K % 128 == 0 && !a.mask_x && (a.seg_images <= 0 || a.seg_images % 4 == 0)) return 8;
   return 0;
 }
+static bool h16_resident(const ConvArgs& a);
 bool conv_h16_ok(int dtype, const ConvArgs& a) {
   if (a.in_scale && a.residual) return false;
+  if (a.out_bits) {
+    if (dtype != DT_BF16 || a.stats || a.mask_x || a.in_scale || a.out_scale || a.seg_images > 0 || a.W > 2048) return false;
+    if (a.K % 128 != 0 && !(h16_resident(a) && a.residual && conv_pp64_ok(DT_BF16, a))) return false;
+  }
   if (a.mask_x) {
     if (!a.mask_scale || !a.mask_shift || !a.mask_mean || a.in_scale || a.bias || a.residual || a.relu || a.out_scale) return false;
     if (18 * 24 * 128 + 2 * 3 * (a.K % 128 == 0 ? 128 : 64) * 128 + 2 * a.C * 4 + 8 * 128 * 4 + 3 * a.K * 4 > 160 * 1024) return false;
@@ -96,6 +107,7 @@
   t.x = reinterpret_cast<const char*>(a.x) + px * a.C * es;
   t.y = reinterpret_cast<char*>(a.y) + px * a.K * es;
   if (a.residual) t.residual = reinterpret_cast<const char*>(a.residual) + px * a.K * es;
+  if (a.out_bits) t.out_bits = a.out_bits + px * a.K / 8;
   return t;
 }
 int conv_h16_rows(const ConvArgs& a) {
@@ -111,16 +123,19 @@
   return on && a.stats && !a.bias && !a.relu && !a.residual && !a.mask_x;
 }
 
-template <typename T, int BKO, int WK, bool XF, bool WR = false, bool RAW = false, int TW = 16, bool OSC = false>
+template <typename T, int BKO, int WK, bool XF, bool WR = false, bool RAW = false, int TW = 16, bool OSC = false, bool OB = false>
 static hipError_t launch_h(const ConvArgs& a, hipStream_t st, int row0 = 0) {
   const size_t lds = (TW == 16 ? 18 * 24 : 4 * 10 * 10) * 128 + (WR ? 3 : 2) * 3 * BKO * 128 + 2 * a.C * sizeof(float) + 8 * BKO * sizeof(float) +
                      (a.mask_x ? 3 : (a.out_scale ? 2 : 1)) * a.K * sizeof(float);
   if (lds > 160 * 1024) return hipErrorInvalidValue;
   static_assert(!OSC || (!XF && !RAW), "output scale: eval forms only");
   void (*kern)(const ConvArgs, const int, const int, const int, const int);
-  if constexpr (OSC) kern = conv3x3_h16s_kernel<T, BKO, WK, WR, TW>;
+  static_assert(!OB || (sizeof(T) == 2 && !OSC && !XF && !WR && !RAW), "output bits: the plain bf16 forms");
+  if constexpr (OB) kern = conv3x3_h16m_kernel<T, BKO, WK, TW>;
+  else if constexpr (OSC) kern = conv3x3_h16s_kernel<T, BKO, WK, WR, TW>;
   else kern = conv3x3_h16_kernel<T, BKO, WK, XF, WR, RAW, TW>;
-  if (OSC != (a.out_scale != nullptr)) return hipErrorInvalidValue;
+  if (OSC != (a.out_scale != nullptr) || OB != (a.out_bits != nullptr)) return hipErrorInvalidValue;
+  if (OB && (a.stats || a.mask_x || a.in_scale)) return hipErrorInvalidValue;
   static std::atomic<bool> attr_done{false};
   if (!attr_done) {
     hipError_t e = hipFuncSetAttribute(reinterpret_cast<const void*>(kern), hipFuncAttributeMaxDynamicSharedMemorySize, 160 * 1024);
@@ -141,6 +156,8 @@
 static hipError_t launch_ht8(const ConvArgs& a, hipStream_t st) {
   const bool xf = a.in_scale != nullptr;
   auto wide = [&](const ConvArgs& q) {
+    if constexpr (sizeof(T) == 2)
+      if (q.out_bits) return launch_h<T, 128, 2, false, false, false, 8, false, true>(q, st);
     if (q.out_scale) return launch_h<T, 128, 2, false, false, false, 8, true>(q, st);
     if constexpr (sizeof(T) == 2)
       if (h16_raw(q)) return xf ? launch_h<T, 128, 2, true, false, true, 8>(q, st) : launch_h<T, 128, 2, false, false, true, 8>(q, st);
@@ -152,6 +169,8 @@
   hipError_t e = wide(head);
   if (e != hipSuccess) return e;
   const int row0 = h16_grid(head, 128) * 4;
+  if constexpr (sizeof(T) == 2)
+    if (tl.out_bits) return launch_h<T, 64, 2, false, false, false, 8, false, true>(tl, st, row0);
   if (tl.out_scale) return launch_h<T, 64, 2, false, false, false, 8, true>(tl, st, row0);
   return xf ? launch_h<T, 64, 2, true, false, false, 8>(tl, st, row0) : launch_h<T, 64, 2, false, false, false, 8>(tl, st, row0);
 }
@@ -161,6 +180,8 @@
   const bool xf = a.in_scale != nullptr;
   if (h16_mode(Elem<T>::DT, a) == 8) return launch_ht8<T>(a, st);
   if (a.K % 128 == 0) {
+    if constexpr (sizeof(T) == 2)
+      if (a.out_bits) return launch_h<T, 128, 2, false, false, false, 16, false, true>(a, st);
     if (a.out_scale) return launch_h<T, 128, 2, false, false, false, 16, true>(a, st);
     if constexpr (sizeof(T) == 2)
       if (h16_raw(a)) return xf ? launch_h<T, 128, 2, true, false, true>(a, st) : launch_h<T, 128, 2, false, false, true>(a, st);
@@ -169,6 +190,7 @@
   if constexpr (sizeof(T) == 2)
     if (h16_resident(a)) {
       if (conv_pp64_ok(DT_BF16, a)) return launch_conv_pp64(a, st);
+      if (a.out_bits) return hipErrorInvalidValue;
       if (a.out_scale) return launch_h<T, 64, 2, false, true, false, 16, true>(a, st);
       return xf ? launch_h<T, 64, 2, true, true>(a, st) : launch_h<T, 64, 2, false, true>(a, st);
     }
@@ -178,11 +200,17 @@
 
 hipError_t launch_conv_h16(int dtype, const ConvArgs& a, hipStream_t st) {
   if (a.mask_x && !a.stats) return hipErrorInvalidValue;
+  if (a.out_bits && !conv_h16_ok(dtype, a)) return hipErrorInvalidValue;
   return dtype == DT_BF16 ? launch_ht<bf16_t>(a, st) : launch_ht<float>(a, st);
 }
 
 const char* conv_h16_name(int dtype, const ConvArgs& a) {
   const bool bf = dtype == DT_BF16, xf = a.in_scale != nullptr;
+  if (a.out_bits) {
+    if (h16_mode(dtype, a) == 8) return "sslcr::conv3x3_h16m_kernel<unsigned short, 128, 2, 8>";
+    if (a.K % 128 == 0) return "sslcr::conv3x3_h16m_kernel<unsigned short, 128, 2, 16>";
+    return conv_pp64_name(a);
+  }
   if (a.out_scale) {
     if (h16_mode(dtype, a) == 8) return bf ? "sslcr::conv3x3_h16s_kernel<unsigned short, 128, 2, false, 8>" : "sslcr::conv3x3_h16s_kernel<float, 128, 2, false, 8>";
     if (a.K % 128 == 0) return bf ? "sslcr::conv3x3_h16s_kernel<unsigned short, 128, 2, false, 16>" : "sslcr::conv3x3_h16s_kernel<float, 128, 2, false, 16>";
diff --git a/ssl_cr_histo_amd/csrc/conv_h16_body.hpp b/ssl_cr_histo_amd/csrc/conv_h16_body.hpp
--- a/ssl_cr_histo_amd/csrc/conv_h16_body.hpp
+++ b/ssl_cr_histo_amd/csrc/conv_h16_body.hpp
@@ -32,7 +32,7 @@
   }
   for (int i = tid; i < 8 * BKO; i += NT) s_stat[i] = 0.f;
   float* s_bias = s_stat + 8 * BKO;
-  const bool mk = !OSC && !XF && !RAW && a.mask_x != nullptr;
+  const bool mk = !OSC && !OBITS && !XF && !RAW && a.mask_x != nullptr;
   float* s_msh = s_bias + a.K;
   float* s_mmu = s_msh + a.K;
   float* s_osc = s_msh;
@@ -50,6 +50,7 @@
 
   const int chunk = tid & 7;
   int rel[NLD], st_off[NLD];
+  const int rel_bias = a.W + 1;
   unsigned long long edge = 0;
   unsigned hvalid = 0;
 #pragma unroll
@@ -70,6 +71,7 @@
       hvalid |= 1u << i;
       edge |= (unsigned long long)((hr == 0) | ((hr == HH - 1) << 1) | ((hc == 0) << 2) | ((hc == HWD - 1) << 3)) << (4 * i);
     }
+    if constexpr (OBITS) rel[i] = (rel[i] + rel_bias) | ((st_off[i] >> 4) << 16);
   }
   const bool loader = WK == 1 || wave >= 4;
   constexpr int WLI = BKO / 32;
@@ -122,7 +124,12 @@
 #pragma unroll
     for (int i = 0; i < NLD; ++i) {
       const bool ok = ((hvalid >> i) & 1u) && !((bad >> (4 * i)) & 0xfull);
-      const int idx = q.origin + (ok ? rel[i] : 0);
+      int rl = rel[i];
+      if constexpr (OBITS) {
+        asm volatile("" : "+v"(rl));
+        rl = (rl & 0xffff) - rel_bias;
+      }
+      const int idx = q.origin + (ok ? rl : 0);
       hreg[i] = ld16_nt(xg + ((size_t)idx * a.C + slab * CE) * sizeof(T));
       hin |= (ok ? 1u : 0u) << i;
     }
@@ -152,7 +159,15 @@
   auto store_halo = [&]() {
 #pragma unroll
     for (int i = 0; i < NLD; ++i)
-      if ((hvalid >> i) & 1u) st16(s_halo + st_off[i], hreg[i]);
+      if ((hvalid >> i) & 1u) {
+        int so = st_off[i];
+        if constexpr (OBITS) {
+          int rl = rel[i];
+          asm volatile("" : "+v"(rl));
+          so = (rl >> 12) & 0xffff0;
+        }
+        st16(s_halo + so, hreg[i]);
+      }
   };
   LdsDma wdma;
   wdma.init(wg, 0x7fffffffu);
@@ -204,10 +219,12 @@
   frags(0, 0, s_w);
 
   char* yg = reinterpret_cast<char*>(a.y);
-  const char* rg = (XF || RAW) ? nullptr : reinterpret_cast<const char*>(a.mask_x ? a.mask_x : a.residual);
+  const char* rg = (XF || RAW) ? nullptr : reinterpret_cast<const char*>((!OBITS && a.mask_x) ? a.mask_x : a.residual);
   constexpr bool RPRE = sizeof(T) == 2 && !XF && !RAW;
   constexpr int RQ = 4 * TK / EPC;
   u32x4_t rres[RPRE ? TP : 1][RPRE ? RQ : 1];
+  static_assert(!OBITS || (sizeof(T) == 2 && RPRE && (TK == 4 || TK == 2)), "output bits: the bf16 residual forms");
+  unsigned obits[OBITS ? TP : 1];
   auto out_off = [&](const Geo& q, int p) {
     const int h = q.h0 + wp * 4 + p, w = q.w0 + li;
     const size_t pix = TW == 16 ? ((size_t)q.n0 * a.H + h) * a.W + w : (size_t)(q.n0 + wp) * 64 + p * 16 + li;
@@ -235,6 +252,15 @@
 #pragma unroll
             for (int q = 0; q < RQ; ++q) rres[p][q] = ld16(rg + out_off(cur, p) + q * 16);
         }
+        if constexpr (OBITS) {
+          if (last) {
+#pragma unroll
+            for (int p = 0; p < TP; ++p) {
+              const uint8_t* bp = a.out_bits + (out_off(cur, p) >> 4);
+              obits[p] = TK == 4 ? (unsigned)*reinterpret_cast<const unsigned short*>(bp) : (unsigned)*bp;
+            }
+          }
+        }
       }
     };
     if constexpr (WR) {
@@ -398,6 +424,11 @@
           }
 #pragma unroll
           for (int e = 0; e < EPC; ++e) vq[e] = clamp_lo(vq[e], out_lo);
+          if constexpr (OBITS) {
+#pragma unroll
+            for (int e = 0; e < EPC; ++e)
+              vq[e] = __uint_as_float(__float_as_uint(vq[e]) & (unsigned)__builtin_amdgcn_sbfe((int)obits[p], q * EPC + e, 1));
+          }
           st16(yg + off + q * 16, PackH<T>::run(vq));
         }
       }
diff --git a/ssl_cr_histo_amd/csrc/conv_igemm.hip b/ssl_cr_histo_amd/csrc/conv_igemm.hip
--- a/ssl_cr_histo_amd/csrc/conv_igemm.hip
+++ b/ssl_cr_histo_amd/csrc/conv_igemm.hip
@@ -338,8 +338,11 @@
   return false;
 }
 
+bool conv_out_bits_ok(int dtype, const ConvArgs& a) { return a.out_bits && conv_h16_ok(dtype, a); }
+
 hipError_t launch_conv(int dtype, const ConvArgs& a, hipStream_t st) {
   if (!conv_segments_ok(dtype, a)) return hipErrorInvalidValue;
+  if (a.out_bits && !conv_out_bits_ok(dtype, a)) return hipErrorInvalidValue;
   if (a.out_scale && (!a.bias || a.stats || a.mask_x)) return hipErrorInvalidValue;
   if (conv_h16_ok(dtype, a)) return launch_conv_h16(dtype, a, st);
   if (a.mask_x) return hipErrorInvalidValue;
diff --git a/ssl_cr_histo_amd/csrc/conv_pp64.hip b/ssl_cr_histo_amd/csrc/conv_pp64.hip
--- a/ssl_cr_histo_amd/csrc/conv_pp64.hip
+++ b/ssl_cr_histo_amd/csrc/conv_pp64.hip
@@ -79,7 +79,7 @@
     if (mk) { s_msh[tid] = a.mask_shift[mo]; s_mmu[tid] = a.mask_mean[mo]; }
     else if (a.out_scale) s_msh[tid] = a.out_scale[tid];
   }
-  const bool osc_on = !mk && !XF && a.out_scale != nullptr;
+  const bool osc_on = !mk && !XF && OP != 3 && a.out_scale != nullptr;
   for (int i = tid; i < 1024; i += 512) s_f[320 + i] = 0.f;
 
   const int chunk = gtid & 7;
@@ -172,11 +172,19 @@
   char* yg = reinterpret_cast<char*>(a.y);
   const char* rg = OP == 0 ? nullptr : reinterpret_cast<const char*>(OP == 2 ? a.mask_x : a.residual);
   u32x4_t rres[RPRE ? TP : 1][RPRE ? RQ : 1];
+  constexpr bool OB = OP == 3;
+  unsigned obits[OB ? TP : 1][OB ? RQ : 1];
   auto out_off = [&](const Geo& q, int p) {
     const int h = q.h0 + wq * 4 + p, w = q.w0 + li;
     return (unsigned)(((q.n0 * a.H + h) * a.W + w) * 64 + g * 8) * (unsigned)sizeof(T);
   };
   auto load_res = [&](const Geo& q) {
+    if constexpr (OB) {
+#pragma unroll
+      for (int p = 0; p < TP; ++p)
+#pragma unroll
+        for (int qq = 0; qq < RQ; ++qq) obits[p][qq] = a.out_bits[(out_off(q, p) >> 4) + qq * 4];
+    }
     if constexpr (RPRE) {
 #pragma unroll
       for (int p = 0; p < TP; ++p)
@@ -303,12 +311,13 @@
 #pragma unroll
               for (int q = 0; q < RQ; ++q) {
                 float vq[EPC], rr[EPC];
-                if constexpr (OP == 1) Elem<T>::unpack(rres[RPRE ? p : 0][RPRE ? q : 0], rr);
+                if constexpr (OP == 1 || OP == 3) Elem<T>::unpack(rres[RPRE ? p : 0][RPRE ? q : 0], rr);
 #pragma unroll
                 for (int e = 0; e < EPC; ++e) {
                   float v = acc[(q * EPC + e) >> 2][p][e & 3] + bias[q * EPC + e];
-                  if constexpr (OP == 1) v += rr[e];
+                  if constexpr (OP == 1 || OP == 3) v += rr[e];
                   vq[e] = __builtin_amdgcn_fmed3f(v, lo, __builtin_inff());
+                  if constexpr (OB) vq[e] = __uint_as_float(__float_as_uint(vq[e]) & (unsigned)__builtin_amdgcn_sbfe((int)obits[OB ? p : 0][OB ? q : 0], e, 1));
                 }
                 st16(yg + out_off(cur, p) + q * 64, PackH<T>::run(vq));
               }
@@ -394,8 +403,9 @@
   constexpr size_t lds = 9 * 64 * 128 + 2 * 18 * 18 * 128 + (320 + 1024) * sizeof(float);
   static std::atomic<bool> attr_done{false};
   if (!attr_done) {
-    const void* ks[4] = {reinterpret_cast<const void*>(conv3x3_pp64_kernel<false, 0>), reinterpret_cast<const void*>(conv3x3_pp64_kernel<false, 1>),
-                         reinterpret_cast<const void*>(conv3x3_pp64_kernel<false, 2>), reinterpret_cast<const void*>(conv3x3_pp64_kernel<true, 0>)};
+    const void* ks[5] = {reinterpret_cast<const void*>(conv3x3_pp64_kernel<false, 0>), reinterpret_cast<const void*>(conv3x3_pp64_kernel<false, 1>),
+                         reinterpret_cast<const void*>(conv3x3_pp64_kernel<false, 2>), reinterpret_cast<const void*>(conv3x3_pp64_kernel<true, 0>),
+                         reinterpret_cast<const void*>(conv3x3_pp64_kernel<false, 3>)};
     for (const void* k : ks) {
       hipError_t e = hipFuncSetAttribute(k, hipFuncAttributeMaxDynamicSharedMemorySize, 160 * 1024);
       if (e != hipSuccess) return e;
@@ -407,7 +417,10 @@
   const int grid = pp64_grid(a);
   if (a.mask_x && !a.stats) return hipErrorInvalidValue;
   const int rows = conv_pp64_rows(a);
-  if (a.in_scale) hipLaunchKernelGGL((conv3x3_pp64_kernel<true, 0>), dim3(grid), dim3(512), lds, st, a, tiles, rows);
+  if (a.out_bits) {
+    if (!a.residual || a.in_scale || a.mask_x || a.stats || a.out_scale || a.seg_images > 0) return hipErrorInvalidValue;
+    hipLaunchKernelGGL((conv3x3_pp64_kernel<false, 3>), dim3(grid), dim3(512), lds, st, a, tiles, rows);
+  } else if (a.in_scale) hipLaunchKernelGGL((conv3x3_pp64_kernel<true, 0>), dim3(grid), dim3(512), lds, st, a, tiles, rows);
   else if (a.mask_x) hipLaunchKernelGGL((conv3x3_pp64_kernel<false, 2>), dim3(grid), dim3(512), lds, st, a, tiles, rows);
   else if (a.residual) hipLaunchKernelGGL((conv3x3_pp64_kernel<false, 1>), dim3(grid), dim3(512), lds, st, a, tiles, rows);
   else hipLaunchKernelGGL((conv3x3_pp64_kernel<false, 0>), dim3(grid), dim3(512), lds, st, a, tiles, rows);
@@ -415,6 +428,7 @@
 }
 
 const char* conv_pp64_name(const ConvArgs& a) {
+  if (a.out_bits) return "sslcr::conv3x3_pp64_kernel<false, 3>";
   if (a.in_scale) return "sslcr::conv3x3_pp64_kernel<true, 0>";
   return a.mask_x ? "sslcr::conv3x3_pp64_kernel<false, 2>" : (a.residual ? "sslcr::conv3x3_pp64_kernel<false, 1>" : "sslcr::conv3x3_pp64_kernel<false, 0>");
 }
diff --git a/ssl_cr_histo_amd/csrc/engine.cpp b/ssl_cr_histo_amd/csrc/engine.cpp
--- a/ssl_cr_histo_amd/csrc/engine.cpp
+++ b/ssl_cr_histo_amd/csrc/engine.cpp
@@ -293,6 +293,7 @@
   const double src = (double)a.N * a.H * a.W;
   r.flops = a.transposed ? 2.0 * src * a.C * a.K * rs : 2.0 * M * a.K * a.C * rs;
   r.bytes = (src * a.C + (double)a.K * rs * a.C + M * a.K * (a.residual ? 2.0 : 1.0) * (a.accumulate ? 2.0 : 1.0)) * es;
+  if (a.out_bits) r.bytes += M * a.K / 8.0;
   r.name = conv_kernel_name(dt, a);
   (void)hipEventRecord(r.e0, st);
   hipError_t e = launch_conv(dt, a, st);
@@ -689,6 +690,10 @@
 bool ybits_on(const sslcr_ctx* c) {
   static const bool on = [] { const char* e = getenv("SSLCR_YBITS"); return !e || atoi(e) != 0; }();
   return on && c->dtype == DT_BF16;
+}
+bool gmask_on() {
+  static const bool on = [] { const char* e = getenv("SSLCR_GMASK"); return !e || atoi(e) != 0; }();
+  return on;
 }
 const uint8_t* ybits_of(const sslcr_net* n, const void* yact) {
   if (!yact || !n->ybits_ok || !ybits_on(n->ctx)) return nullptr;
@@ -1172,8 +1177,11 @@
 
   size_t hi_pending = n->goff[60];
   int bucket = 1;
+  const bool gm = gmask_on() && dt == DT_BF16 && npass == 1 && !n->tap && n->ybits_ok && ybits_on(c);
+  bool g_ready = gm && P[0].blk[7].ybits != nullptr;
   for (int p = 0; p < npass; ++p)
-    TRY(launch_avgpool_bwd(dt, n->dE[p], buf(kOut, p, (size_t)N * d.lh[7] * d.lw[7] * 512 * es), N, d.lh[7] * d.lw[7], 512, st));
+    TRY(launch_avgpool_bwd(dt, n->dE[p], buf(kOut, p, (size_t)N * d.lh[7] * d.lw[7] * 512 * es), N, d.lh[7] * d.lw[7], 512, st,
+                           g_ready ? P[p].blk[7].ybits : nullptr));
   for (int i = 7; i >= 0; --i) {
     BlockL& B = n->blocks[i];
     const int oh = d.lh[i], ow = d.lw[i];
@@ -1226,8 +1234,8 @@
     }
     for (int p = 0; p < npass; ++p) {
       PassState& ps = P[p];
-      char *dOut = buf(kOut, p, so), *G = buf(kG, p, so), *dRaw2 = buf(kRaw2, p, so), *dAct1 = buf(kAct1, p, so), *dRaw1 = buf(kRaw1, p, so),
-           *dRawD = buf(kRawD, p, so);
+      char *dOut = buf(kOut, p, so), *G = g_ready ? dOut : buf(kG, p, so), *dRaw2 = buf(kRaw2, p, so), *dAct1 = buf(kAct1, p, so),
+           *dRaw1 = buf(kRaw1, p, so), *dRawD = buf(kRawD, p, so);
       if (!seg_bn) {
       TRYI(wg_wait(c, 0, st));
       if (B.has_ds) TRYI(wg_wait(c, 2, st));
@@ -1236,13 +1244,14 @@
         double* ring = take_sums(c);
         double* sums_2 = ring ? ring : c->bn_sums;
         double* sums_d = sums_2 + 2 * B.b2.C;
-        TRYI(bn_bwd_begin(n, B.b2, ps.bn[B.b2.bidx], dOut, ps.blk[i].raw2, ps.blk[i].y, 0, dRaw2, G, opix, (double)opix, st, sums_2, &a2, nullptr, 1,
-                          nullptr, 0, ring != nullptr, 1, 0, true));
+        TRYI(bn_bwd_begin(n, B.b2, ps.bn[B.b2.bidx], dOut, ps.blk[i].raw2, g_ready ? nullptr : ps.blk[i].y, 0, dRaw2, G, opix, (double)opix, st, sums_2,
+                          &a2, nullptr, g_ready ? 0 : 1, nullptr, 0, ring != nullptr, 1, 0, true));
         TRYI(bn_bwd_begin(n, B.bd, ps.bn[B.bd.bidx], G, ps.blk[i].rawd, nullptr, 0, dRawD, nullptr, opix, (double)opix, st, sums_d, &ad, nullptr, 0,
                           nullptr, 0, ring != nullptr, 1, 0, true));
         const bool pair = bn_bwd_pair_ok(a2, ad);
         static const bool g_free = [] { const char* e = getenv("SSLCR_BN_PAIR_G"); return e && atoi(e) == 0; }();
-        const int keep_g = (n->tap || !a2.yact_bits || !g_free) ? 1 : 0;
+        const int keep_g = (g_ready || n->tap || !a2.yact_bits || !g_free) ? 1 : 0;
+        if (!pair && g_ready) a2.gout = nullptr;
         if (pair) {
           TRY(launch_bn_bwd_reduce_pair(dt, a2, ad, keep_g, st));
         } else {
@@ -1270,7 +1279,8 @@
           TRYI(bn_bwd_end(c, ad, st));
         }
       } else {
-        TRYI(bn_backward(n, B.b2, ps.bn[B.b2.bidx], dOut, ps.blk[i].raw2, ps.blk[i].y, 0, dRaw2, G, opix, (double)opix, st, nullptr, 1));
+        if (g_ready) TRYI(bn_backward(n, B.b2, ps.bn[B.b2.bidx], G, ps.blk[i].raw2, nullptr, 0, dRaw2, nullptr, opix, (double)opix, st));
+        else TRYI(bn_backward(n, B.b2, ps.bn[B.b2.bidx], dOut, ps.blk[i].raw2, ps.blk[i].y, 0, dRaw2, G, opix, (double)opix, st, nullptr, 1));
       }
       if (p == 0) {
         TRYI(tap(i, 0, G, N, oh, ow, B.c2.cout));
@@ -1336,14 +1346,20 @@
       TRYI(wgrad_call(n, B.c1, X0, buf(kRaw1, 0, so), nullptr, N * npass, xh, xw, oh, ow, st, 0, 0, 1));
       if (B.has_ds) TRYI(wgrad_call(n, B.ds, X0, buf(kRawD, 0, so), nullptr, N * npass, xh, xw, oh, ow, st, 0, 0, 2));
     }
+    bool next_ready = false;
     if (need_dx) {
       {
         const int NB = N * npass;
-        char *G = buf(kG, 0, so), *dRaw1 = buf(kRaw1, 0, so), *dXin = buf(kXin, 0, si), *dRawD = buf(kRawD, 0, so);
+        char *G = g_ready ? buf(kOut, 0, so) : buf(kG, 0, so), *dRaw1 = buf(kRaw1, 0, so), *dXin = buf(kXin, 0, si), *dRawD = buf(kRawD, 0, so);
         ConvArgs a = conv_args(B.c1, dRaw1, B.c1.w_dg, dXin, NB, oh, ow);
         a.C = B.c1.cout; a.K = B.c1.cin; a.transposed = (B.c1.stride == 1) ? 0 : 1; a.PH = xh; a.PW = xw; a.OH = xh; a.OW = xw;
         if (!B.has_ds) a.residual = G;
         if (B.c1.stride == 1) {
+          if (gm && i > 0 && !B.has_ds && P[0].blk[i - 1].ybits) {
+            a.out_bits = P[0].blk[i - 1].ybits;
+            if (conv_out_bits_ok(dt, a)) next_ready = true;
+            else a.out_bits = nullptr;
+          }
           TRY(prof_conv(c, dt,a, st));
         } else {
           ConvArgs q4 = a;
@@ -1375,6 +1391,7 @@
       }
       const int t = kOut; kOut = kXin; kXin = t;
     }
+    g_ready = next_ready;
     if (i == 6 || i == 4 || i == 2) {
       TRYI(launch_bucket_allreduce(n, bucket++, n->goff[B.pstart], hi_pending, st));
       hi_pending = n->goff[B.pstart];
diff --git a/ssl_cr_histo_amd/csrc/kernels.hpp b/ssl_cr_histo_amd/csrc/kernels.hpp
--- a/ssl_cr_histo_amd/csrc/kernels.hpp
+++ b/ssl_cr_histo_amd/csrc/kernels.hpp
@@ -26,6 +26,7 @@
 const char* wgrad_kernel_name(int dtype, const WgradArgs& a);
 int conv_partials_rows(const ConvArgs& a);
 bool conv_segments_ok(int dtype, const ConvArgs& a);
+bool conv_out_bits_ok(int dtype, const ConvArgs& a);
 int device_cus();
 int conv_halo_tw(int dtype, const ConvArgs& a);
 int conv_halo_tiles(const ConvArgs& a, int tw);
@@ -83,7 +84,7 @@
 hipError_t launch_bn_relu_maxpool(int dtype, const PoolFwdArgs& a, hipStream_t st);
 hipError_t launch_maxpool_relu_bwd(int dtype, const PoolBwdArgs& a, hipStream_t st);
 hipError_t launch_avgpool_fwd(int dtype, const void* x, float* y, int N, int HW, int C, hipStream_t st);
-hipError_t launch_avgpool_bwd(int dtype, const float* dy, void* dx, int N, int HW, int C, hipStream_t st);
+hipError_t launch_avgpool_bwd(int dtype, const float* dy, void* dx, int N, int HW, int C, hipStream_t st, const uint8_t* bits = nullptr);
 hipError_t launch_bn_bwd_reduce(int dtype, const BnBwdArgs& a, hipStream_t st);
 hipError_t launch_bn_bwd_apply(int dtype, const BnBwdArgs& a, hipStream_t st);
 bool bn_bwd_pair_ok(const BnBwdArgs& a, const BnBwdArgs& b);
diff --git a/ssl_cr_histo_amd/kernels.py b/ssl_cr_histo_amd/kernels.py
--- a/ssl_cr_histo_amd/kernels.py
+++ b/ssl_cr_histo_amd/kernels.py
@@ -32,8 +32,8 @@
 
 def conv2d(x, w, stride, pad, *, in_scale=None, in_shift=None, in_relu=False, bias=None, residual=None, relu=False,
            want_stats=False, out=None, transposed=False, out_hw=None, osh=1, accumulate=False, pixel_hw=None,
-           pix_mul=0, pix_off=(0, 0), tap_mask=0, mask=None, par4=False, seg_images=0, out_scale=None):
-    _chk(x, w, in_scale, in_shift, bias, residual, out, out_scale)
+           pix_mul=0, pix_off=(0, 0), tap_mask=0, mask=None, par4=False, seg_images=0, out_scale=None, out_bits=None):
+    _chk(x, w, in_scale, in_shift, bias, residual, out, out_scale, out_bits)
     dt = _dt(x)
     N, H, W, C = x.shape
     K, R, S, C2 = w.shape
@@ -49,6 +49,9 @@
                    int(accumulate), int(pix_mul), int(pix_off[0]), int(pix_off[1]), int(tap_mask))
     d.par4 = int(par4)
     d.out_scale = L.ptr(out_scale)
+    if out_bits is not None:
+        assert out_bits.dtype == torch.uint8 and out_bits.numel() * 8 == y.numel()
+        d.out_bits = L.ptr(out_bits)
     if seg_images:
         d.seg_images = int(seg_images)
         d.seg_stride = int(in_scale.stride(0)) if in_scale is not None and in_scale.dim() == 2 else 0
@@ -302,11 +305,15 @@
     return y
 
 
-def avgpool_bwd(dy, shape, dtype):
-    _chk(dy)
+def avgpool_bwd(dy, shape, dtype, bits=None):
+    _chk(dy, bits)
     N, H, W, Cn = shape
     dx = torch.empty(shape, dtype=tdtype(dtype), device=dy.device)
-    L.check(L.lib().sslcr_avgpool_bwd(dtype, L.ptr(dy), L.ptr(dx), N, H * W, Cn, L.stream_ptr()))
+    if bits is not None:
+        assert bits.dtype == torch.uint8 and bits.numel() * 8 == dx.numel()
+        L.check(L.lib().sslcr_avgpool_bwd_bits(dtype, L.ptr(dy), L.ptr(dx), L.ptr(bits), N, H * W, Cn, L.stream_ptr()))
+    else:
+        L.check(L.lib().sslcr_avgpool_bwd(dtype, L.ptr(dy), L.ptr(dx), N, H * W, Cn, L.stream_ptr()))
     return dx
 
 
```

Result: no change. 68590 (median of 6 runs) (+0.5%).
